# maxim2266/csvplus

Hardware: AMD Instinct MI355X
Metric: joined rows/sec (IndexOn build + chained Join, 1e8-row 3-col orders) (higher is better)
Workload: dtype u32; 1 GPU; BASELINE configs[3]: orders(1e8 x {cust_id,prod_id,qty}).Join(UniqueIndexOn customers.id 1e7).Join(UniqueIndexOn products.prod_id 1e5); rows=100000000, customers=10000000, products=100000, rows_this_rank=100000000, exchange=none (1 GPU), output=sorted positions

## Files before the change

csvplus_amd/csrc/capi.hip:

```cpp
#include <algorithm>
#include <map>
#include <mutex>
#include <new>

#include "cph_internal.hpp"
#include "codec_device.hpp"

namespace cph {

constexpr size_t kGuardBytes = 256;
constexpr uint8_t kGuardByte = 0xA5;

Status DevicePool::alloc(size_t bytes, void** out) {
    std::lock_guard<std::recursive_mutex> lk(mu_);
    const size_t want = (bytes + (guard ? kGuardBytes : 0) + 255) & ~(size_t)255;
    int best = -1;
    for (int i = 0; i < (int)free_.size(); i++) {
        if (free_[i].cap >= want && free_[i].cap <= want * 2 + (1u << 20)) {
            if (best < 0 || free_[i].cap < free_[best].cap) best = i;
        }
    }
    Block b;
    bool from_slab = false;
    for (size_t i = 0; i < slab_free_.size(); i++)
// ... 349 lines not shown
}

Status validate_cols(const cph_strcol* cols, int32_t ncols) {
    if (!cols || ncols <= 0) return {CPH_ERR_INVALID, "no key columns"};
    if (ncols > kMaxKeyCols) return {CPH_ERR_INVALID, "too many key columns"};
    for (int c = 0; c < ncols; c++) {
        if (cols[c].fixed_width == 0 && cols[c].offset_bits != 32 && cols[c].offset_bits != 64)
            return {CPH_ERR_INVALID, "offset_bits must be 32 or 64"};
        if (cols[c].mem != CPH_MEM_HOST && cols[c].mem != CPH_MEM_DEVICE) return {CPH_ERR_INVALID, "bad mem"};
        if (cols[c].nrows != cols[0].nrows) return {CPH_ERR_INVALID, "key columns differ in row count"};
        if (cols[c].nrows && !cols[c].offsets && cols[c].fixed_width == 0) return {CPH_ERR_INVALID, "offsets is NULL"};
        if (cols[c].nrows && cols[c].fixed_width && !cols[c].data) return {CPH_ERR_INVALID, "data is NULL"};
    }
    if (cols[0].nrows > 0xFFFFFFFFull) return {CPH_ERR_TOO_MANY_ROWS, "more than 2^32-1 rows"};
    return {};
}

Status stage_cols(cph_ctx* ctx, const cph_strcol* cols, int32_t ncols, std::vector<DevBuf>* storage,
                         DevCol* out) {
    for (int c = 0; c < ncols; c++) {
        DevCol d;
        d.nrows = cols[c].nrows;
        d.offset_bits = cols[c].offset_bits;
        d.fixed_width = cols[c].fixed_width;
        if (cols[c].mem == CPH_MEM_DEVICE || cols[c].nrows == 0) {
            d.data = cols[c].data;
            d.offsets = cols[c].offsets;
            if (!d.data) {
                if (!ctx->safe_words) {
                    CPH_TRY(ctx->safe_words.alloc(&ctx->pool, 64));
                    CPH_HIP_TRY(hipMemsetAsync(ctx->safe_words.get(), 0, 64, ctx->stream));
                }
                d.data = ctx->safe_words.as<uint8_t>();
            }
        } else if (cols[c].fixed_width) {
            const size_t bytes = (size_t)cols[c].nrows * cols[c].fixed_width;
            DevBuf bd;
            CPH_TRY(bd.alloc(&ctx->pool, bytes + 8));
            CPH_HIP_TRY(hipMemcpyAsync(bd.get(), cols[c].data, bytes, hipMemcpyHostToDevice, ctx->stream));
            d.data = bd.as<uint8_t>();
            d.offsets = nullptr;
            storage->push_back(std::move(bd));
        } else {
            const size_t obytes = (size_t)(cols[c].nrows + 1) * (size_t)(cols[c].offset_bits / 8);
            const uint64_t first = cols[c].offset_bits == 32 ? ((const uint32_t*)cols[c].offsets)[0]
                                                             : ((const uint64_t*)cols[c].offsets)[0];
            const uint64_t last = cols[c].offset_bits == 32 ? ((const uint32_t*)cols[c].offsets)[cols[c].nrows]
                                                            : ((const uint64_t*)cols[c].offsets)[cols[c].nrows];
            if (last < first) return {CPH_ERR_INVALID, "offsets are not monotonic"};
            DevBuf bo, bd;
            CPH_TRY(bo.alloc(&ctx->pool, obytes));
            CPH_TRY(bd.alloc(&ctx->pool, (size_t)last + 8));
            CPH_HIP_TRY(hipMemcpyAsync(bo.get(), cols[c].offsets, obytes, hipMemcpyHostToDevice, ctx->stream));
            if (last) CPH_HIP_TRY(hipMemcpyAsync(bd.get(), cols[c].data, (size_t)last, hipMemcpyHostToDevice, ctx->stream));
            d.data = bd.as<uint8_t>();
            d.offsets = bo.get();
            storage->push_back(std::move(bo));
            storage->push_back(std::move(bd));
        }
        out[c] = d;
    }
    return {};
}

Status check_row_sources(const cph_strcol* cols, const cph_rowsel* sel, int32_t ncols, uint64_t first_row, uint64_t nrows, bool exact) {
    for (int c = 0; c < ncols; c++) {
        CPH_TRY(validate_cols(cols + c, 1));
        const bool ident = !sel || !sel[c].ids;
        if (ident && nrows && (exact ? cols[c].nrows != nrows : cols[c].nrows < first_row + nrows))
            return {CPH_ERR_INVALID, exact ? "a column without row ids must have nrows rows"
                                           : "a column without row ids must have at least first_row + nrows rows"};
        if (!ident && sel[c].bits != 32 && sel[c].bits != 64) return {CPH_ERR_INVALID, "row id bits must be 32 or 64"};
    }
    return {};
}

Status stage_row_sources(cph_ctx* ctx, const cph_strcol* cols, const cph_rowsel* sel, const int* order, int32_t ncols, uint64_t first_row,
                         uint64_t n, std::vector<DevBuf>* staged, ColsArg* arg, ColIds* ids) {
    for (int k = 0; k < ncols; k++) {
        const int c = order ? order[k] : k;
        CPH_TRY(stage_cols(ctx, cols + c, 1, staged, &arg->c[k]));
        if (!sel || !sel[c].ids || !n) continue;
        RowIds& r = ids->ids[k];
        r.bits = sel[c].bits;
        r.base = sel[c].base;
        r.ptr = sel[c].ids;
        if (cols[c].mem == CPH_MEM_HOST) {
            const size_t w = (size_t)(sel[c].bits / 8);
            staged->emplace_back();
            CPH_TRY(staged->back().alloc(&ctx->pool, n * w));
            CPH_HIP_TRY(hipMemcpyAsync(staged->back().get(), static_cast<const uint8_t*>(sel[c].ids) + first_row * w, n * w,
                                       hipMemcpyHostToDevice, ctx->stream));
            r.ptr = reinterpret_cast<const void*>((uintptr_t)staged->back().get() - (uintptr_t)(first_row * w));
        }
    }
    return {};
}

Status deliver(cph_ctx* ctx, ResultOwner* owner, const ResultPart* parts, int nparts, int32_t out_mem) {
    auto show = [](const ResultPart& p, const void* v) { memcpy(p.pub, &v, sizeof v); };
    auto padded = [](const ResultPart& p) { return (p.bytes + 15) & ~(size_t)15; };
    uint8_t* h = nullptr;
    if (out_mem == CPH_MEM_HOST) {
        size_t need = 16;
        for (int i = 0; i < nparts; i++) need += padded(parts[i]);
        CPH_HIP_TRY(hipHostMalloc(&owner->h_block, need, hipHostMallocDefault));
        h = static_cast<uint8_t*>(owner->h_block);
    }
    for (int i = 0; i < nparts; i++) {
        const ResultPart& p = parts[i];
        const void* src = p.src ? p.src : p.dev->get();
        if (h && p.bytes) CPH_HIP_TRY(hipMemcpyAsync(h, src, p.bytes, hipMemcpyDeviceToHost, ctx->stream));
        show(p, h ? h : src);
        if (h) h += padded(p);
    }
    CPH_HIP_TRY(hipStreamSynchronize(ctx->stream));
    if (h)
        for (int i = 0; i < nparts; i++) parts[i].dev->reset();
    return {};
}

static int32_t fail(cph_ctx* ctx, const Status& s) {
    if (ctx) ctx->err = s.msg;
    return s.code;
}

static Status enter(cph_ctx* ctx) {
    if (!ctx) return {CPH_ERR_INVALID, "ctx is NULL"};
    CPH_HIP_TRY(hipSetDevice(ctx->device));
    return {};
}

struct BuildJob {
    cph_index* ix = nullptr;
    int32_t nkeycols = 0;
    std::vector<DevBuf> staged;
    DevCol dcols[kMaxKeyCols];
    DevBuf stats_dev;
    const void* sample_host = nullptr;
    size_t scratch_off = 0;
    GroupSpec spec;
    bool small = false;
    SmallBufs sbufs;
    bool presplit = false;
    bool sampled = false;
    bool no_sample = false;
    bool unique = false;
    bool no_direct = false;
    bool side = false;
    bool spec_split = false;
    bool exact_split = false;
    bool no_split = false;
    uint32_t* miss = nullptr;
    uint32_t* cs_over = nullptr;
    DevBuf cs_codes;
};

static Status build_phase1(cph_ctx* ctx, const cph_strcol* keycols, int32_t nkeycols, BuildJob* job) {
    CPH_TRY(validate_cols(keycols, nkeycols));
    cph_index* ix = job->ix;
    ix->ctx = ctx;
    ix->nrows = keycols[0].nrows;
    ix->table_rows = ix->nrows;
    ix->nkeycols = nkeycols;
    job->nkeycols = nkeycols;
    CPH_TRY(stage_cols(ctx, keycols, nkeycols, &job->staged, job->dcols));
    job->small = small_build_applies(ctx, job->dcols, nkeycols, ix->nrows);
    if (!job->small && !job->no_split && nkeycols == 1 && !job->dcols[0].fixed_width && ix->nrows >= (1ull << 22)) {
        CPH_TRY(codec_try_split(ctx, job->dcols, 1, ix->nrows, nullptr, &ix->codec, !job->exact_split, &job->spec_split));
        job->presplit = ix->codec.has_split();
    }
    job->sampled = !job->small && !job->presplit && !job->no_sample && codec_sample_applies(ctx, job->dcols, nkeycols, ix->nrows);
    if (job->sampled) CPH_TRY(codec_sample_launch(ctx, job->dcols[0], ix->nrows, &job->sample_host));
    else if (!job->small && !job->presplit) CPH_TRY(codec_stats_launch(ctx, job->dcols, nkeycols, &job->stats_dev));
    return {};
}

static Status build_phase2(cph_ctx* ctx, BuildJob* job, const void* stats_host);
static Status job_arm_miss(cph_ctx* ctx, BuildJob* job) {
    job->miss = host_word(ctx);
    return job->miss ? Status{} : Status{CPH_ERR_HIP, "no pinned host memory for the report words of a build"};
}
static Status build_encode_sort(cph_ctx* ctx, BuildJob* job);

static size_t job_readback_bytes(const BuildJob& j) {
    return j.small ? sizeof(SmallResult) : (j.presplit || j.sampled) ? 0 : sizeof(ColStats) * (size_t)j.nkeycols;
}

static void build_run(cph_ctx* ctx, std::vector<BuildJob>& jobs, std::vector<Status>& status) {
    const size_t nj = jobs.size();
    auto fail_all = [&](const Status& s) {
        for (size_t i = 0; i < nj; i++)
            if (status[i].ok()) status[i] = s;
    };
    size_t total = 0;
    bool any_general = false;
    for (size_t i = 0; i < nj; i++) {
        jobs[i].scratch_off = total;
        total += job_readback_bytes(jobs[i]);
        total = (total + 63) & ~(size_t)63;
        if (status[i].ok() && !jobs[i].small) any_general = true;
    }
    Status s = ensure_pinned_scratch(ctx, total > 64 ? total : 64);
    if (!s.ok()) return fail_all(s);
    uint8_t* h = static_cast<uint8_t*>(ctx->pinned_scratch);
    for (size_t i = 0; i < nj; i++) {
        if (!status[i].ok()) continue;
        if (jobs[i].small) {
            SideStream on_side(ctx, jobs[i].side);
            status[i] = small_build_launch(ctx, jobs[i].dcols, jobs[i].nkeycols, jobs[i].ix->nrows, &jobs[i].sbufs,
                                           reinterpret_cast<SmallResult*>(h + jobs[i].scratch_off));
            continue;
        }
        if (jobs[i].presplit || jobs[i].sampled) continue;
        hipError_t e = hipMemcpyAsync(h + jobs[i].scratch_off, jobs[i].stats_dev.get(), job_readback_bytes(jobs[i]),
                                      hipMemcpyDeviceToHost, jobs[i].side ? ctx->side_stream : ctx->stream);
        if (e != hipSuccess) status[i] = {CPH_ERR_HIP, std::string("statistics read-back: ") + hipGetErrorString(e)};
    }
    bool any_side = false;
    for (size_t i = 0; i < nj; i++) any_side = any_side || jobs[i].side;
    auto sync_streams = [&]() {
        return hipStreamSynchronize(ctx->stream) == hipSuccess && (!any_side || hipStreamSynchronize(ctx->side_stream) == hipSuccess);
    };
    if (!sync_streams()) return fail_all({CPH_ERR_HIP, "hipStreamSynchronize failed"});
    ctx->pool.flush_deferred();
    std::vector<std::vector<uint8_t>> stats_host(nj);
    std::vector<size_t> retry;
    for (size_t i = 0; i < nj; i++) {
        if (!status[i].ok()) continue;
        if (jobs[i].small) {
            const SmallResult res = *reinterpret_cast<const SmallResult*>(h + jobs[i].scratch_off);
            bool not_small = false;
            status[i] = small_build_finish(ctx, jobs[i].ix, jobs[i].nkeycols, &jobs[i].sbufs, &res, &not_small);
            jobs[i].sbufs = SmallBufs{};
            if (status[i].ok() && not_small) retry.push_back(i);
            else if (status[i].ok()) index_plan_table(jobs[i].ix);
            continue;
        }
        if (jobs[i].sampled) {
            const uint8_t* sh = static_cast<const uint8_t*>(jobs[i].sample_host);
            stats_host[i].assign(sh, sh + codec_sample_bytes());
        } else if (!jobs[i].presplit) {
            stats_host[i].assign(h + jobs[i].scratch_off, h + jobs[i].scratch_off + job_readback_bytes(jobs[i]));
        }
    }
    for (size_t i = 0; i < nj; i++)
        if (status[i].ok() && !jobs[i].small) {
            SideStream on_side(ctx, jobs[i].side);
            status[i] = build_phase2(ctx, &jobs[i], stats_host[i].data());
        }
    std::vector<size_t> resplit;
    std::vector<size_t> resort;
    if (any_general) {
        s = ensure_pinned_scratch(ctx, 2 * sizeof(uint32_t) * nj + 64);
        if (!s.ok()) return fail_all(s);
        uint32_t* fd = static_cast<uint32_t*>(ctx->pinned_scratch);
        uint32_t* sm = fd + nj;
        for (size_t i = 0; i < nj; i++) {
            if (!status[i].ok() || jobs[i].small) continue;
            hipStream_t js = jobs[i].side ? ctx->side_stream : ctx->stream;
            fd[i] = 0xFFFFFFFFu;
            sm[i] = 0;
            if (!jobs[i].ix->first_dup_dev) continue;
            hipError_t e = hipMemcpyAsync(&fd[i], jobs[i].ix->first_dup_dev.get(), sizeof(uint32_t), hipMemcpyDeviceToHost, js);
            if (e != hipSuccess) status[i] = {CPH_ERR_HIP, std::string("first-duplicate read-back: ") + hipGetErrorString(e)};
        }
        if (!sync_streams()) return fail_all({CPH_ERR_HIP, "hipStreamSynchronize failed"});
        ctx->pool.flush_deferred();
        for (size_t i = 0; i < nj; i++) {
            if (!status[i].ok() || jobs[i].small) continue;
            cph_index* ix = jobs[i].ix;
            if (jobs[i].miss) sm[i] = *(volatile uint32_t*)jobs[i].miss;
            if (sm[i]) { jobs[i].cs_codes.reset(); jobs[i].cs_over = nullptr; resplit.push_back(i); continue; }
            if (jobs[i].cs_over && *(volatile uint32_t*)jobs[i].cs_over) { resort.push_back(i); continue; }
            jobs[i].cs_codes.reset();
            ix->first_dup = fd[i] != 0xFFFFFFFFu ? (uint64_t)fd[i] : UINT64_MAX;
            ix->first_dup_dev.reset();
            index_plan_table(ix);
        }
    }
    for (size_t i : resort) {
        BuildJob& j = jobs[i];
        cph_index* ix = j.ix;
        const uint64_t n = ix->nrows;
        uint32_t* over = j.cs_over;
        j.cs_over = nullptr;
        ix->sorted_codes.reset(); ix->perm.reset(); ix->first_dup_dev.reset();
        DevBuf kb, va, vb;
        Status r = kb.alloc(&ctx->pool, n * sizeof(uint32_t));
        if (r.ok()) r = va.alloc(&ctx->pool, n * sizeof(uint32_t));
        bool sorted_now = false;
        {
            CountedSortPlan first;
            int wb = counted_sort_plan(ctx, n, ix->codec.word_states[0], &first) ? (int)first.wbits : 0;
            for (int attempt = 0; attempt < 2 && r.ok() && !sorted_now && wb > 0; attempt++) {
                wb -= 2;
                CountedSortPlan csp;
                if (!counted_sort_plan(ctx, n, ix->codec.word_states[0], &csp, wb) || (int)csp.wbits != wb) break;
                r = ix->first_dup_dev.alloc(&ctx->pool, sizeof(uint32_t));
                if (r.ok()) r = counted_sort(ctx, csp, j.cs_codes.as<uint32_t>(), n, ix->codec.word_states[0], va.as<uint32_t>(), kb.as<uint32_t>(),
                                             ix->first_dup_dev.as<uint32_t>(), over);
                if (r.ok() && hipStreamSynchronize(ctx->stream) != hipSuccess) r = {CPH_ERR_HIP, "hipStreamSynchronize failed"};
                if (r.ok() && *(volatile uint32_t*)over == 0) {
                    ix->sorted_codes = std::move(kb);
                    ix->perm = std::move(va);
                    ix->sort_passes = 0;
                    r = index_first_dup_read(ctx, ix);
                    sorted_now = true;
                } else {
                    ix->first_dup_dev.reset();
                }
            }
        }
        if (sorted_now) {
            j.cs_codes.reset();
            if (r.ok()) index_plan_table(ix);
            status[i] = r;
            continue;
        }
        if (r.ok()) r = vb.alloc(&ctx->pool, n * sizeof(uint32_t));
        uint32_t *kout = nullptr, *vout = nullptr;
        int passes = 0;
        if (r.ok()) r = radix_sort_pairs<uint32_t>(ctx, j.cs_codes.as<uint32_t>(), kb.as<uint32_t>(), va.as<uint32_t>(), vb.as<uint32_t>(), true, n,
                                                   ix->codec.word_bits[0], &kout, &vout, &passes);
        if (r.ok()) {
            ix->sorted_codes = std::move(kout == j.cs_codes.as<uint32_t>() ? j.cs_codes : kb);
            ix->perm = std::move(vout == va.as<uint32_t>() ? va : vb);
            ix->sort_passes = passes;
            r = index_first_dup_launch(ctx, ix);
        }
        if (r.ok()) r = index_first_dup_read(ctx, ix);
        j.cs_codes.reset();
        if (r.ok()) index_plan_table(ix);
        status[i] = r;
    }
    for (size_t i : resplit) {
        std::vector<BuildJob> one;
        one.push_back(std::move(jobs[i]));
        std::vector<Status> st1(1);
        BuildJob& j = one[0];
        j.side = false;
        const bool again_exact = j.spec_split;
        j.spec_split = false;
        j.exact_split = again_exact;
        j.no_split = !again_exact;
        j.no_sample = true;
        j.sampled = false;
        j.no_direct = true;
        j.presplit = false;
        j.miss = nullptr;
        cph_index* ix = j.ix;
        ix->codec = CodecHost{};
        ix->codec_dev.reset(); ix->sorted_codes.reset(); ix->perm.reset(); ix->first_dup_dev.reset(); ix->ranktab.reset();
        if (again_exact) {
            ctx->n_split_respec++;
            st1[0] = codec_try_split(ctx, j.dcols, 1, ix->nrows, nullptr, &ix->codec, false, nullptr);
            j.presplit = st1[0].ok() && ix->codec.has_split();
        }
        if (st1[0].ok() && !j.presplit) st1[0] = codec_stats_launch(ctx, j.dcols, j.nkeycols, &j.stats_dev);
        if (st1[0].ok()) build_run(ctx, one, st1);
        status[i] = st1[0];
        jobs[i] = std::move(one[0]);
    }
    for (size_t i : retry) {
        std::vector<BuildJob> one;
        one.push_back(std::move(jobs[i]));
        std::vector<Status> st1(1);
        one[0].small = false;
        one[0].side = false;
        st1[0] = codec_stats_launch(ctx, one[0].dcols, one[0].nkeycols, &one[0].stats_dev);
        if (st1[0].ok()) build_run(ctx, one, st1);
        status[i] = st1[0];
        jobs[i] = std::move(one[0]);
    }
}

static Status sort_words_lsd(cph_ctx* ctx, cph_index* ix, const uint64_t* all, int nw, const int* bits, uint64_t n, DevBuf& va,
                             DevBuf& vb) {
    DevBuf ka, kb;
    CPH_TRY(ka.alloc(&ctx->pool, n * sizeof(uint64_t)));
    CPH_TRY(kb.alloc(&ctx->pool, n * sizeof(uint64_t)));
    uint32_t* vcur = va.as<uint32_t>();
    uint32_t* vother = vb.as<uint32_t>();
    uint64_t* kout = ka.as<uint64_t>();
    bool first = true;
    int passes = 0;
    ix->sort_passes = 0;
    for (int w = nw - 1; w >= 0; w--) {
        const uint64_t* word = all + (uint64_t)w * n;
        if (first) {
            if (n) CPH_HIP_TRY(hipMemcpyAsync(ka.get(), word, n * sizeof(uint64_t), hipMemcpyDeviceToDevice, ctx->stream));
        } else {
            CPH_TRY(gather_u64(ctx, word, vcur, ka.as<uint64_t>(), n));
        }
        uint32_t* vout;
        CPH_TRY(radix_sort_pairs<uint64_t>(ctx, ka.as<uint64_t>(), kb.as<uint64_t>(), vcur, vother, first, n, bits[w], &kout, &vout,
                                           &passes));
        ix->sort_passes += passes;
        if (vout != vcur) { vother = vcur; vcur = vout; }
        first = false;
    }
    DevBuf sorted;
    CPH_TRY(sorted.alloc(&ctx->pool, (size_t)nw * n * sizeof(uint64_t)));
    if (n) CPH_HIP_TRY(hipMemcpyAsync(sorted.get(), kout, n * sizeof(uint64_t), hipMemcpyDeviceToDevice, ctx->stream));
    for (int w = 1; w < nw; w++) CPH_TRY(gather_u64(ctx, all + (uint64_t)w * n, vcur, sorted.as<uint64_t>() + (uint64_t)w * n, n));
    ix->sorted_codes = std::move(sorted);
    ix->perm = std::move(vcur == va.as<uint32_t>() ? va : vb);
    return {};
}

static DevCol window_col(const DevCol* cols, const cph_key_window& w, int s) {
    DevCol v = cols[w.seg_col[s]];
    v.skip = w.seg_skip[s];
    v.take = w.seg_take[s];
    return v;
}

static Status build_multi_window(cph_ctx* ctx, BuildJob* job, const std::vector<ColStats>& raw) {
    cph_index* ix = job->ix;
    const uint64_t n = ix->nrows;
    std::vector<cph_key_window>& W = ix->windows;
    W.clear();
    W.emplace_back();
    uint32_t room = kMaxKeyBytes;
    for (int c = 0; c < job->nkeycols; c++) {
        uint32_t left = raw[(size_t)c].maxlen, skip = 0;
        do {
            if (room == 0 || W.back().nseg == kMaxKeyCols) {
                W.emplace_back();
                room = kMaxKeyBytes;
            }
            cph_key_window& w = W.back();
            const uint32_t t = left < room ? left : room;
            w.seg_col[w.nseg] = c;
            w.seg_skip[w.nseg] = skip;
            w.seg_take[w.nseg] = t == left ? 0xFFFFFFFFu : t;
            w.nseg++;
            skip += t;
            left -= t;
            room -= t;
        } while (left > 0);
    }
    int total_words = 0;
    for (auto& w : W) {
        DevCol v[kMaxKeyCols];
        for (int s = 0; s < w.nseg; s++) v[s] = window_col(job->dcols, w, s);
        std::vector<ColStats> st;
        CPH_TRY(codec_collect_stats(ctx, v, w.nseg, &st));
        CPH_TRY(codec_build(st, &w.codec));
        w.codec.key32 = false;
        CPH_TRY(codec_upload(ctx, w.codec, &w.codec_dev));
        w.word_base = total_words;
        total_words += w.codec.nwords;
    }
    ix->codec = W[0].codec;
    DevBuf all, va, vb;
    CPH_TRY(all.alloc(&ctx->pool, (size_t)total_words * n * sizeof(uint64_t)));
    CPH_TRY(va.alloc(&ctx->pool, n * sizeof(uint32_t)));
    CPH_TRY(vb.alloc(&ctx->pool, n * sizeof(uint32_t)));
    std::vector<int> bits((size_t)total_words);
    for (auto& w : W) {
        DevCol v[kMaxKeyCols];
        for (int s = 0; s < w.nseg; s++) v[s] = window_col(job->dcols, w, s);
        CPH_TRY(codec_encode_build(ctx, w.codec, w.codec_dev, v, n, all.as<uint64_t>() + (uint64_t)w.word_base * n));
        for (int k = 0; k < w.codec.nwords; k++) bits[(size_t)(w.word_base + k)] = w.codec.word_bits[k];
    }
    CPH_TRY(sort_words_lsd(ctx, ix, all.as<uint64_t>(), total_words, bits.data(), n, va, vb));
    return index_first_dup_launch(ctx, ix);
}

static Status build_phase2(cph_ctx* ctx, BuildJob* job, const void* stats_host) {
    cph_index* ix = job->ix;
    const uint64_t n = ix->nrows;
    const int32_t nkeycols = job->nkeycols;
    const DevCol* dcols = job->dcols;
    if (job->presplit) {
        CPH_TRY(job_arm_miss(ctx, job));
        CPH_TRY(codec_upload(ctx, ix->codec, &ix->codec_dev));
        return build_encode_sort(ctx, job);
    }
    std::vector<ColStats> stats;
    if (job->sampled) {
        codec_sample_finish(dcols[0], stats_host, &stats);
        CPH_TRY(codec_build(stats, &ix->codec));
        if (codec_sample_checked(ix->codec, dcols)) {
            CPH_TRY(job_arm_miss(ctx, job));
            CPH_TRY(codec_upload(ctx, ix->codec, &ix->codec_dev));
            return build_encode_sort(ctx, job);
        }
        job->sampled = false;
        ix->codec = CodecHost{};
        CPH_TRY(codec_collect_stats(ctx, dcols, nkeycols, &stats));
    } else {
        codec_stats_finish(dcols, nkeycols, stats_host, &stats);
    }
    uint64_t positions = 0;
    for (const auto& s : stats) positions += s.maxlen;
    if (positions > (uint64_t)kMaxKeyBytes) return build_multi_window(ctx, job, stats);
    CPH_TRY(codec_build(stats, &ix->codec));
    if (!job->no_split) CPH_TRY(codec_try_split(ctx, dcols, nkeycols, n, &stats, &ix->codec));
// ... 97 lines not shown
                    return build_encode_sort(ctx, job);
                }
                CPH_TRY(codec_encode_build(ctx, cd, ix->codec_dev, dcols, n, ka.get(), &eh, nullptr));
            }
        }
        uint32_t* vout;
        if (cd.key32) {
            uint32_t* kout;
            CPH_TRY(radix_sort_pairs<uint32_t>(ctx, ka.as<uint32_t>(), kb.as<uint32_t>(), va.as<uint32_t>(), vb.as<uint32_t>(),
                                               true, n, cd.word_bits[0], &kout, &vout, &passes, eh.counts, eh.done));
            ix->sorted_codes = std::move(kout == ka.as<uint32_t>() ? ka : kb);
        } else {
            uint64_t* kout;
            CPH_TRY(radix_sort_pairs<uint64_t>(ctx, ka.as<uint64_t>(), kb.as<uint64_t>(), va.as<uint32_t>(), vb.as<uint32_t>(),
                                               true, n, cd.word_bits[0], &kout, &vout, &passes, eh.counts, eh.done));
            ix->sorted_codes = std::move(kout == ka.as<uint64_t>() ? ka : kb);
        }
        ix->sort_passes = passes;
        ix->perm = std::move(vout == va.as<uint32_t>() ? va : vb);
    } else {
        DevBuf all;
        CPH_TRY(all.alloc(&ctx->pool, (size_t)cd.nwords * n * sizeof(uint64_t)));
        CPH_TRY(codec_encode_build(ctx, cd, ix->codec_dev, dcols, n, all.get(), nullptr, nullptr, job->miss));
        CPH_TRY(sort_words_lsd(ctx, ix, all.as<uint64_t>(), cd.nwords, cd.word_bits, n, va, vb));
    }

    CPH_TRY(index_first_dup_launch(ctx, ix));
    return {};
}

static Status index_build_impl(cph_ctx* ctx, const cph_strcol* keycols, int32_t nkeycols, cph_index* ix, bool unique) {
    if (nkeycols == 1 && keycols && keycols[0].mem == CPH_MEM_HOST && validate_cols(keycols, nkeycols).ok()) {
        bool taken = false;
        CPH_TRY(build_from_host_codes(ctx, keycols, nkeycols, ix, unique, &taken));
        if (taken) return {};
    }
    std::vector<BuildJob> jobs(1);
    std::vector<Status> st(1);
    jobs[0].ix = ix;
    jobs[0].unique = unique;
    st[0] = build_phase1(ctx, keycols, nkeycols, &jobs[0]);
    if (st[0].ok()) build_run(ctx, jobs, st);
    return st[0];
}

}

using namespace cph;

extern "C" {

CPH_API const char* cph_version(void) { return "csvplus_hip 0.1 (gfx950)"; }

CPH_API int32_t cph_ctx_create(int32_t device_id, cph_ctx** out) {
    if (!out) return CPH_ERR_INVALID;
    *out = nullptr;
    int count = 0;
    hipError_t e = hipGetDeviceCount(&count);
    if (e != hipSuccess || count <= 0) {
        (void)hipGetLastError();
        return CPH_ERR_NO_DEVICE;
    }
    if (device_id < 0 || device_id >= count) return CPH_ERR_NO_DEVICE;
    if (hipSetDevice(device_id) != hipSuccess) return CPH_ERR_NO_DEVICE;
    cph_ctx* ctx = new (std::nothrow) cph_ctx();
    if (!ctx) return CPH_ERR_NOMEM;
    ctx->device = device_id;
    if (hipStreamCreateWithFlags(&ctx->stream, hipStreamNonBlocking) != hipSuccess) {
        delete ctx;
        return CPH_ERR_HIP;
    }
    ctx->own_stream = true;
    warm_keycodec();
    warm_radix_sort();
    warm_probe();
    warm_chain();
    warm_materialize();
    warm_csv_ingest();
    warm_index_ops();
    warm_resolve();
    warm_small_build();
    warm_window_sort();
    warm_counted_sort();
    (void)ensure_pinned_scratch(ctx, 1 << 16);
    void* ring = nullptr;
    (void)pinned_upload(ctx, 64, &ring);
    (void)host_word(ctx);
    *out = ctx;
    return CPH_OK;
}

CPH_API void cph_ctx_destroy(cph_ctx* ctx) {
    if (!ctx) return;
    (void)hipSetDevice(ctx->device);
    (void)hipStreamSynchronize(ctx->stream);
    if (ctx->pinned_scratch) (void)hipHostFree(ctx->pinned_scratch);
    if (ctx->upload_ring) (void)hipHostFree(ctx->upload_ring);
    if (ctx->host_words) (void)hipHostFree(ctx->host_words);
    for (void* p : ctx->pinned_user) (void)hipHostFree(p);
    for (auto& b : ctx->pinned_user_free) (void)hipHostFree(b.first);
    for (auto& b : ctx->pinned_cache) (void)hipHostFree(b.first);
    for (auto& p : ctx->prof_pending) { (void)hipEventDestroy(p.start); (void)hipEventDestroy(p.stop); }
    for (hipEvent_t e : ctx->prof_free_events) (void)hipEventDestroy(e);
    hipStream_t own = ctx->own_stream ? ctx->stream : nullptr;
    if (ctx->side_stream) {
        (void)hipStreamSynchronize(ctx->side_stream);
        (void)hipStreamDestroy(ctx->side_stream);
    }
    if (ctx->side_fork) (void)hipEventDestroy(ctx->side_fork);
    for (auto& sc : ctx->scan) sc.words.reset();
    for (auto& sc : ctx->self_clean) { sc.sum.reset(); sc.sample.reset(); sc.win.reset(); }
    host_pool_destroy(ctx);
    ctx->pool.trim();
    if (own) (void)hipStreamDestroy(own);
    delete ctx;
}

CPH_API int32_t cph_ctx_set_option(cph_ctx* ctx, const char* name, int64_t value) {
    if (!ctx || !name) return CPH_ERR_INVALID;
    const std::string k(name);
    if (k == "chain_debug") ctx->chain_debug = (int)value;
    else if (k == "sort_threads") ctx->sort_threads = (int)value;
    else if (k == "sort_rbits") ctx->sort_rbits = (int)value;
    else if (k == "sort_digit_stream") ctx->sort_digit_stream = value != 0;
    else if (k == "sort_xcd_tiles") ctx->sort_xcd_tiles = value != 0;
    else if (k == "codec_debug") ctx->codec_debug = (int)value;
    else if (k == "join_hash") ctx->join_hash = value != 0;
    else if (k == "chain_nt_streams") ctx->chain_nt_streams = value < 0 || value > 2 ? 0 : (int)value;
    else if (k == "chain_rank_lds") ctx->chain_rank_lds = value != 0;
    else if (k == "chain_rows4") ctx->chain_rows4 = value < 0 || value > 2 ? 1 : (int)value;
    else if (k == "codec_split") ctx->codec_split = value != 0;
    else if (k == "split_speculative") ctx->split_speculative = value != 0;
    else if (k == "scan_lookback") ctx->scan_lookback = value != 0;
    else if (k == "build_side_stream") ctx->build_side_stream = value != 0;
    else if (k == "stats_sample") ctx->stats_sample = value != 0;
    else if (k == "host_build") ctx->host_build = value != 0;
    else if (k == "host_threads") { ctx->host_threads = value < 0 || value > 256 ? 0 : (int)value; host_pool_destroy(ctx); }
    else if (k == "host_split") ctx->host_split = value < 0 || value > 2 ? 1 : (int)value;
    else if (k == "host_numa") ctx->host_numa = value != 0;
    else if (k == "hash_partitioned") ctx->hash_partitioned = value < 0 || value > 2 ? 1 : (int)value;
    else if (k == "host_split_threads") { ctx->host_split_threads = value < 0 || value > 256 ? 0 : (int)value; host_pool_destroy(ctx); }
    else if (k == "counted_sort") ctx->counted_sort = value != 0;
    else if (k == "csv_fast") ctx->csv_fast = value != 0;
    else if (k == "csv_onepass_debug") ctx->csv_onepass_debug = (int)value;
    else if (k == "csv_onepass") ctx->csv_onepass = value < 0 ? 0 : value > (1 << 20) ? (1 << 20) : (int)value;
    else if (k == "direct_sort") {
        if (value != 0 && value != 1) return fail_with(ctx, {CPH_ERR_INVALID, "direct_sort must be 0 or 1"});
        ctx->direct_sort = (int)value;
    }
    else if (k == "chain_arith") ctx->chain_arith = value != 0;
    else if (k == "chain_identity") ctx->chain_identity = value != 0;
    else if (k == "chain_prejoin") ctx->chain_prejoin = value != 0;
    else if (k == "direct_fused_encode") ctx->direct_fused_encode = value != 0;
    else if (k == "direct_ranktab") ctx->direct_ranktab = value != 0;
    else if (k == "hash_load_pct") ctx->hash_load_pct = value < 25 ? 25 : value > 90 ? 90 : (int)value;
    else if (k == "small_build_rows") ctx->small_build_rows = value < 0 ? 0 : value > (1 << 20) ? (1 << 20) : (int)value;
    else if (k == "plan_threads") ctx->plan_threads = (int)value;
    else if (k == "gstats_threads") ctx->gstats_threads = (int)value;
    else if (k == "speculative_groups") ctx->speculative_groups = value < 0 || value > 2 ? 1 : (int)value;
    else if (k == "pool_guard") ctx->pool.guard = value != 0;
    else if (k == "pool_reserve_mb") {
        if (value <= 0) return fail_with(ctx, {CPH_ERR_INVALID, "pool_reserve_mb must be positive"});
        if (hipSetDevice(ctx->device) != hipSuccess) return fail_with(ctx, {CPH_ERR_HIP, "hipSetDevice failed"});
        Status rs = ctx->pool.reserve((size_t)value << 20);
        if (!rs.ok()) return fail_with(ctx, rs);
    }
    else if (k == "pool_guard_check") {
        ctx->pool.check_live();
        if (ctx->pool.guard_violations) {
            char b[64];
            snprintf(b, sizeof b, " (%llu blocks)", (unsigned long long)ctx->pool.guard_violations);
            return fail_with(ctx, {CPH_ERR_INVALID, ctx->pool.first_violation + b});
        }
    }
    else return fail_with(ctx, {CPH_ERR_INVALID, "unknown option: " + k});
    return CPH_OK;
}

CPH_API const char* cph_last_error(const cph_ctx* ctx) { return ctx ? ctx->err.c_str() : "ctx is NULL"; }

CPH_API int32_t cph_ctx_set_stream(cph_ctx* ctx, void* hip_stream) {
    Status s = enter(ctx);
    if (!s.ok()) return fail(ctx, s);
    (void)hipStreamSynchronize(ctx->stream);
    if (ctx->side_stream) (void)hipStreamSynchronize(ctx->side_stream);
    for (auto& sc : ctx->scan) { sc.words.reset(); sc.tiles = 0; sc.tickets = 0; sc.epoch = 0; }
    if (hip_stream) {
        if (ctx->own_stream) (void)hipStreamDestroy(ctx->stream);
        ctx->stream = reinterpret_cast<hipStream_t>(hip_stream);
        ctx->own_stream = false;
    } else if (!ctx->own_stream) {
        if (hipStreamCreateWithFlags(&ctx->stream, hipStreamNonBlocking) != hipSuccess)
            return fail(ctx, {CPH_ERR_HIP, "hipStreamCreate failed"});
        ctx->own_stream = true;
    }
    return CPH_OK;
}

CPH_API int32_t cph_ctx_synchronize(cph_ctx* ctx) {
    Status s = enter(ctx);
    if (!s.ok()) return fail(ctx, s);
    hipError_t e = hipStreamSynchronize(ctx->stream);
    if (e != hipSuccess) return fail(ctx, {CPH_ERR_HIP, std::string("hipStreamSynchronize: ") + hipGetErrorString(e)});
    return CPH_OK;
}

CPH_API int32_t cph_ctx_profile(cph_ctx* ctx, int32_t enable) {
    Status s = enter(ctx);
    if (!s.ok()) return fail(ctx, s);
    ctx->profiling = enable != 0;
    ctx->prof_only.clear();
    return CPH_OK;
}

CPH_API int32_t cph_ctx_profile_only(cph_ctx* ctx, const char* kernel_name) {
    Status s = enter(ctx);
    if (!s.ok()) return fail(ctx, s);
    ctx->profiling = kernel_name != nullptr;
    ctx->prof_only = kernel_name ? kernel_name : "";
    return CPH_OK;
}

CPH_API int32_t cph_ctx_profile_read(cph_ctx* ctx, cph_kernel_stat* out, int32_t cap, int32_t* n, int32_t reset) {
    Status s = enter(ctx);
    if (!s.ok()) return fail(ctx, s);
    if (!n || (cap > 0 && !out)) return fail(ctx, {CPH_ERR_INVALID, "bad argument"});
    hipError_t e = hipStreamSynchronize(ctx->stream);
    if (e != hipSuccess) return fail(ctx, {CPH_ERR_HIP, std::string("hipStreamSynchronize: ") + hipGetErrorString(e)});
    for (auto& p : ctx->prof_pending) {
        float ms = 0;
        if (hipEventElapsedTime(&ms, p.start, p.stop) == hipSuccess) {
            ProfStat& st = ctx->prof_stats[(size_t)p.name_idx];
            st.launches++;
            st.total_ms += ms;
            st.bytes += p.bytes;
        } else {
            (void)hipGetLastError();
        }
        ctx->prof_free_events.push_back(p.start);
        ctx->prof_free_events.push_back(p.stop);
    }
    ctx->prof_pending.clear();
    const int32_t total = (int32_t)ctx->prof_stats.size();
    *n = total;
    for (int32_t i = 0; i < total && i < cap; i++) {
        const ProfStat& st = ctx->prof_stats[(size_t)i];
        memset(&out[i], 0, sizeof out[i]);
        snprintf(out[i].name, sizeof out[i].name, "%s", st.name.c_str());
        out[i].launches = st.launches;
        out[i].total_ms = st.total_ms;
        out[i].algo_bytes = st.bytes;
    }
    if (reset) ctx->prof_stats.clear();
    return CPH_OK;
}

CPH_API int32_t cph_pinned_alloc(cph_ctx* ctx, size_t bytes, void** out) {
    Status s = enter(ctx);
    if (!s.ok()) return fail(ctx, s);
    if (!out) return fail(ctx, {CPH_ERR_INVALID, "out is NULL"});
    void* p = nullptr;
    constexpr size_t kRecycleMax = 4u << 20;
    size_t cap = bytes ? bytes : 1;
    if (cap <= kRecycleMax) {
        size_t c2 = 4096;
        while (c2 < cap) c2 <<= 1;
        cap = c2;
        for (size_t i = 0; i < ctx->pinned_user_free.size(); i++)
            if (ctx->pinned_user_free[i].second == cap) {
                p = ctx->pinned_user_free[i].first;
                ctx->pinned_user_free.erase(ctx->pinned_user_free.begin() + (long)i);
                break;
            }
    }
    if (!p) {
        hipError_t e = hipHostMalloc(&p, cap, hipHostMallocDefault);
        if (e != hipSuccess) {
            (void)hipGetLastError();
            for (auto& b : ctx->pinned_user_free) (void)hipHostFree(b.first);
            ctx->pinned_user_free.clear();
            e = hipHostMalloc(&p, cap, hipHostMallocDefault);
        }
        if (e != hipSuccess) return fail(ctx, {CPH_ERR_NOMEM, std::string("hipHostMalloc: ") + hipGetErrorString(e)});
    }
    ctx->pinned_user.push_back(p);
    if (cap <= kRecycleMax) ctx->pinned_user_cap.push_back({p, cap});
    *out = p;
    return CPH_OK;
}

CPH_API int32_t cph_pinned_free(cph_ctx* ctx, void* p) {
    Status s = enter(ctx);
    if (!s.ok()) return fail(ctx, s);
    auto it = std::find(ctx->pinned_user.begin(), ctx->pinned_user.end(), p);
    if (it == ctx->pinned_user.end()) return fail(ctx, {CPH_ERR_INVALID, "not a cph_pinned_alloc block"});
    ctx->pinned_user.erase(it);
    for (size_t i = 0; i < ctx->pinned_user_cap.size(); i++)
        if (ctx->pinned_user_cap[i].first == p) {
            const size_t cap = ctx->pinned_user_cap[i].second;
            ctx->pinned_user_cap.erase(ctx->pinned_user_cap.begin() + (long)i);
            if (ctx->pinned_user_free.size() < 32) {
                ctx->pinned_user_free.push_back({p, cap});
                return CPH_OK;
            }
            break;
        }
    (void)hipHostFree(p);
    return CPH_OK;
}

CPH_API int32_t cph_index_build(cph_ctx* ctx, const cph_strcol* keycols, int32_t nkeycols, int32_t unique,
                                cph_index** out, uint64_t* first_dup_pos) {
    Status s = enter(ctx);
    if (!s.ok()) return fail(ctx, s);
    if (!out) return fail(ctx, {CPH_ERR_INVALID, "out is NULL"});
    *out = nullptr;
    if (first_dup_pos) *first_dup_pos = UINT64_MAX;
    cph_index* ix = new (std::nothrow) cph_index();
    if (!ix) return fail(ctx, {CPH_ERR_NOMEM, "out of host memory"});
    s = index_build_impl(ctx, keycols, nkeycols, ix, unique != 0);
    if (!s.ok()) {
        delete ix;
        return fail(ctx, s);
    }
    if (first_dup_pos) *first_dup_pos = ix->first_dup;
    *out = ix;
    if (unique && ix->first_dup != UINT64_MAX) {
        char b[128];
        snprintf(b, sizeof b, "duplicate value while creating unique index (sorted position %llu)",
                 (unsigned long long)ix->first_dup);
        return fail(ctx, {CPH_ERR_DUPLICATE, b});
    }
    return CPH_OK;
}

CPH_API int32_t cph_index_build_many(cph_ctx* ctx, const cph_index_spec* specs, int32_t nspecs, cph_index** out,
                                     uint64_t* first_dup_pos, int32_t* status) {
    Status s = enter(ctx);
    if (!s.ok()) return fail(ctx, s);
    if (!specs || !out || nspecs < 1 || nspecs > 64) return fail(ctx, {CPH_ERR_INVALID, "bad cph_index_build_many arguments"});
    std::vector<BuildJob> jobs((size_t)nspecs);
    std::vector<Status> st((size_t)nspecs);
    if (!host_words_reserve(ctx, (uint32_t)nspecs * (uint32_t)(codec_sample_bytes() / 4 + 16)))
        return fail(ctx, {CPH_ERR_INVALID, "cph_index_build_many: the batch needs more report words than the ctx holds"});
    bool two_streams = nspecs >= 2 && ctx->build_side_stream != 0;
    if (two_streams && !ctx->side_stream && hipStreamCreateWithFlags(&ctx->side_stream, hipStreamNonBlocking) != hipSuccess) {
        (void)hipGetLastError();
        ctx->side_stream = nullptr;
        two_streams = false;
    }
    struct DeferGuard {
        cph_ctx* c;
        ~DeferGuard() {
            if (!c) return;
            (void)hipStreamSynchronize(c->stream);
            (void)hipStreamSynchronize(c->side_stream);
            c->pool.end_defer();
        }
    } defer{two_streams ? ctx : nullptr};
    if (two_streams) {
        hipError_t fe = ctx->side_fork ? hipSuccess : hipEventCreateWithFlags(&ctx->side_fork, hipEventDisableTiming);
        if (fe == hipSuccess) fe = hipEventRecord(ctx->side_fork, ctx->stream);
        if (fe == hipSuccess) fe = hipStreamWaitEvent(ctx->side_stream, ctx->side_fork, 0);
        if (fe != hipSuccess) {
            (void)hipGetLastError();
            two_streams = false;
            defer.c = nullptr;
        }
    }
    if (two_streams) ctx->pool.begin_defer();
    for (int i = 0; i < nspecs; i++) {
        out[i] = nullptr;
        if (first_dup_pos) first_dup_pos[i] = UINT64_MAX;
        jobs[i].ix = new (std::nothrow) cph_index();
        jobs[i].side = two_streams && (i & 1);
        jobs[i].unique = specs[i].unique != 0;
        SideStream on_side(ctx, jobs[i].side);
        if (!jobs[i].ix) st[i] = {CPH_ERR_NOMEM, "out of host memory"};
        else st[i] = build_phase1(ctx, specs[i].keycols, specs[i].nkeycols, &jobs[i]);
    }
    build_run(ctx, jobs, st);
    int32_t rc = CPH_OK;
    std::string msg;
    for (int i = 0; i < nspecs; i++) {
        cph_index* ix = jobs[i].ix;
        if (st[i].ok() && specs[i].unique && ix->first_dup != UINT64_MAX) {
            char b[160];
            snprintf(b, sizeof b, "index %d: duplicate value while creating unique index (sorted position %llu)", i,
                     (unsigned long long)ix->first_dup);
            st[i] = {CPH_ERR_DUPLICATE, b};
        }
        const bool keep = st[i].ok() || st[i].code == CPH_ERR_DUPLICATE;
        if (keep) {
            out[i] = ix;
            if (first_dup_pos) first_dup_pos[i] = ix->first_dup;
        } else {
            delete ix;
        }
        if (status) status[i] = st[i].code;
        if (!st[i].ok() && rc == CPH_OK) { rc = st[i].code; msg = st[i].msg; }
    }
    if (rc != CPH_OK) return fail(ctx, {rc, msg});
    return CPH_OK;
}

CPH_API void cph_index_destroy(cph_index* ix) {
    if (!ix) return;
    if (ix->ctx) (void)hipSetDevice(ix->ctx->device);
    if (ix->perm_host) {
        if (ix->ctx) pinned_cache_put(ix->ctx, ix->perm_host, ix->perm_host_cap);
        else (void)hipHostFree(ix->perm_host);
    }
    delete ix;
}

CPH_API uint64_t cph_index_nrows(const cph_index* ix) { return ix ? ix->nrows : 0; }
CPH_API int32_t cph_index_nkeycols(const cph_index* ix) { return ix ? ix->nkeycols : 0; }

CPH_API int32_t cph_index_perm(cph_index* ix, int32_t mem, const uint32_t** perm, uint64_t* n) {
    if (!ix || !perm) return CPH_ERR_INVALID;
    cph_ctx* ctx = ix->ctx;
    Status s = enter(ctx);
    if (!s.ok()) return fail(ctx, s);
    if (n) *n = ix->nrows;
    if (mem == CPH_MEM_DEVICE) {
        *perm = ix->perm.as<uint32_t>();
        return CPH_OK;
    }
    if (!ix->perm_host) {
        const size_t bytes = (size_t)ix->nrows * sizeof(uint32_t);
        void* p = nullptr;
        size_t cap = 0;
        s = pinned_cache_get(ctx, bytes, &p, &cap);
        if (!s.ok()) return fail(ctx, s);
        if (bytes) {
            hipError_t e = hipMemcpyAsync(p, ix->perm.get(), bytes, hipMemcpyDeviceToHost, ctx->stream);
            if (e == hipSuccess) e = hipStreamSynchronize(ctx->stream);
            if (e != hipSuccess) {
                (void)hipHostFree(p);
                return fail(ctx, {CPH_ERR_HIP, std::string("perm read-back: ") + hipGetErrorString(e)});
            }
        }
        ix->perm_host = static_cast<uint32_t*>(p);
        ix->perm_host_cap = cap;
    }
    *perm = ix->perm_host;
    return CPH_OK;
}

CPH_API int32_t cph_join_probe(cph_ctx* ctx, const cph_index* ix, const cph_strcol* probecols, int32_t nprobecols,
                               const void* row_sel, int32_t sel_bits, uint64_t sel_base, uint64_t nsel,
                               uint64_t probe_base, int32_t want_pairs, int32_t out_mem, cph_matches** out) {
    Status s = enter(ctx);
    if (!s.ok()) return fail(ctx, s);
    if (!ix || !out) return fail(ctx, {CPH_ERR_INVALID, "index/out is NULL"});
    *out = nullptr;
    if (nprobecols > ix->nkeycols) return fail(ctx, {CPH_ERR_TOO_MANY_COLS, "too many source columns in Join()"});
    s = validate_cols(probecols, nprobecols);
    if (!s.ok()) return fail(ctx, s);
    if (out_mem != CPH_MEM_HOST && out_mem != CPH_MEM_DEVICE) return fail(ctx, {CPH_ERR_INVALID, "bad out_mem"});
    if (row_sel && sel_bits != 32 && sel_bits != 64) return fail(ctx, {CPH_ERR_INVALID, "sel_bits must be 32 or 64"});
    if (row_sel && nsel > 0xFFFFFFFFull) return fail(ctx, {CPH_ERR_TOO_MANY_ROWS, "more than 2^32-1 selected rows"});

    cph_matches_impl* m = new (std::nothrow) cph_matches_impl();
    if (!m) return fail(ctx, {CPH_ERR_NOMEM, "out of host memory"});
    m->ctx = ctx;
    auto run = [&]() -> Status {
        std::vector<DevBuf> staged;
        DevCol dcols[kMaxKeyCols];
        CPH_TRY(stage_cols(ctx, probecols, nprobecols, &staged, dcols));
        RowSel dsel;
        dsel.ptr = row_sel;
        dsel.bits = sel_bits;
        dsel.base = sel_base;
        DevBuf selbuf;
        const bool cols_on_host = probecols[0].mem == CPH_MEM_HOST;
        if (row_sel && cols_on_host && nsel) {
            const size_t sb = nsel * (size_t)(sel_bits / 8);
            CPH_TRY(selbuf.alloc(&ctx->pool, sb));
            CPH_HIP_TRY(hipMemcpyAsync(selbuf.get(), row_sel, sb, hipMemcpyHostToDevice, ctx->stream));
            dsel.ptr = selbuf.get();
        }
        const uint64_t nprobe = row_sel ? nsel : probecols[0].nrows;
        ProbeOut po;
        CPH_TRY(probe_run(ctx, ix, dcols, nprobecols, dsel, nprobe, probe_base, want_pairs != 0, &po));
        m->pub.nprobe = nprobe;
        m->pub.nmatches = po.nmatches;
        m->pub.mem = out_mem;
        const bool pairs = want_pairs && po.nmatches;
        if (out_mem == CPH_MEM_DEVICE) {
            m->d_lo = std::move(po.lo);
            m->d_cnt = std::move(po.cnt);
            m->d_pidx = std::move(po.pidx);
            m->d_brow = std::move(po.brow);
            m->pub.lo = m->d_lo.as<uint32_t>();
            m->pub.cnt = m->d_cnt.as<uint32_t>();
// ... 306 lines not shown
```

csvplus_amd/csrc/codec_device.hpp:

```cpp
#pragma once

#include "cph_internal.hpp"
#include "device_utils.hpp"

namespace cph {

__device__ __forceinline__ uint64_t find_first_byte(const uint8_t* data, uint64_t begin, uint64_t len, uint32_t d) {
    const uint64_t dv = 0x0101010101010101ull * (uint64_t)(d & 0xFFu);
    for (uint64_t j = 0; 8 * j < len; j++) {
        const uint64_t x = load_value_chunk(data, begin, len, (int)j) ^ dv;
        const uint64_t t = (x - 0x0101010101010101ull) & ~x & 0x8080808080808080ull;
        if (t) {
            const uint64_t pos = 8 * j + (uint64_t)((__ffsll((long long)t) - 1) >> 3);
            return pos < len ? pos : len;
        }
    }
    return len;
}

__device__ __forceinline__ void value_span_whole(const DevCol& col, uint64_t row, uint64_t* begin, uint64_t* len);
__device__ __forceinline__ void value_span(const DevCol& col, uint64_t row, uint64_t* begin, uint64_t* len) {
    value_span_whole(col, row, begin, len);
    if (col.split) {
        const uint64_t b = *begin, l = *len;
// ... 218 lines not shown
        uint32_t b[R], e[R];
#pragma unroll
        for (int k = 0; k < R; k++) {
            b[k] = NT ? __builtin_nontemporal_load(&off[wr.rel[k]]) : off[wr.rel[k]];
            e[k] = NT ? __builtin_nontemporal_load(&off[wr.rel[k] + 1]) : off[wr.rel[k] + 1];
        }
#pragma unroll
        for (int k = 0; k < R; k++) {
            sp->x[k] = b[k];
            sp->len[k] = e[k] - b[k];
        }
    } else if constexpr (sizeof(B) == 8) {
        const uint64_t* off = reinterpret_cast<const uint64_t*>(c.offsets) + wr.rbase;
        uint64_t b[R], e[R];
#pragma unroll
        for (int k = 0; k < R; k++) {
            b[k] = off[wr.rel[k]];
            e[k] = off[wr.rel[k] + 1];
        }
#pragma unroll
        for (int k = 0; k < R; k++) {
            sp->x[k] = b[k];
            const uint64_t l = e[k] - b[k];
            sp->len[k] = l > 0xFFFFFFFFull ? 0xFFFFFFFFu : (uint32_t)l;
        }
    } else {
#pragma unroll
        for (int k = 0; k < R; k++) { sp->x[k] = 0; sp->len[k] = 0; }
    }
}
template <int R, class B>
__device__ __forceinline__ void gather_spans(const DevCol& c, const uint32_t (&row)[R], WaveSpans<R, B>* sp) {
    const uint64_t p = (uint64_t)(uintptr_t)c.data;
    sp->base8 = (const uint8_t*)(uintptr_t)(p & ~7ull);
    sp->delta = (uint32_t)(p & 7ull);
    if (c.fixed_width) {
#pragma unroll
        for (int k = 0; k < R; k++) {
            sp->x[k] = (B)row[k] * (B)c.fixed_width;
            sp->len[k] = c.fixed_width;
        }
        return;
    }
    if (c.offset_bits == 32) {
        const uint32_t* off = reinterpret_cast<const uint32_t*>(c.offsets);
        uint32_t b[R], e[R];
#pragma unroll
        for (int k = 0; k < R; k++) {
            b[k] = off[row[k]];
            e[k] = off[(uint64_t)row[k] + 1];
        }
#pragma unroll
        for (int k = 0; k < R; k++) {
            sp->x[k] = b[k];
            sp->len[k] = e[k] - b[k];
        }
    } else if constexpr (sizeof(B) == 8) {
        const uint64_t* off = reinterpret_cast<const uint64_t*>(c.offsets);
        uint64_t b[R], e[R];
#pragma unroll
        for (int k = 0; k < R; k++) {
            b[k] = off[row[k]];
            e[k] = off[(uint64_t)row[k] + 1];
        }
#pragma unroll
        for (int k = 0; k < R; k++) {
            sp->x[k] = b[k];
            const uint64_t l = e[k] - b[k];
            sp->len[k] = l > 0xFFFFFFFFull ? 0xFFFFFFFFu : (uint32_t)l;
        }
    } else {
#pragma unroll
        for (int k = 0; k < R; k++) { sp->x[k] = 0; sp->len[k] = 0; }
    }
}
inline bool col_is_narrow(const DevCol& c) { return c.fixed_width ? c.fixed_width <= 0xFFFFu : c.offset_bits == 32; }

template <int R, class W, class B, bool FIXED>
__device__ __forceinline__ void encode_position(const CPH_LDS W* lp, int b, uint32_t pos, const WaveSpans<R, B>& sp, const uint64_t (&cur)[R],
                                                W (&acc)[R], W (&bad)[R]) {
#pragma unroll
    for (int k = 0; k < R; k++) {
        const uint32_t half = b < 4 ? (uint32_t)cur[k] : (uint32_t)(cur[k] >> 32);
        const uint32_t byte = (half >> (8 * (b & 3))) & 0xFFu;
        const uint32_t sym = FIXED ? byte + 1u : (pos < sp.len[k] ? byte + 1u : 0u);
        const W v = lp[b * kLutStride + sym];
        if constexpr (sizeof(W) == 4) {
            acc[k] = __builtin_elementwise_add_sat(acc[k], v);
        } else {
            bad[k] |= v;
            acc[k] += v;
        }
    }
}

template <int R, class W, class B, class CW, bool LONG>
__device__ __forceinline__ void encode_rows(const CodecView& cv, const WaveSpans<R, B>& sp, const uint64_t (&c0)[R],
                                            const uint64_t (&c1)[R], CW (&code)[R], uint32_t* okmask, bool fixed = false) {
    const int maxlen = cv.hdr->col_maxlen[0];
    const CPH_LDS W* lutw = (const CPH_LDS W*)cv.lutw;
    W acc[R], bad[R];
#pragma unroll
    for (int k = 0; k < R; k++) { acc[k] = 0; bad[k] = 0; }
    const int nchunks = (maxlen + 7) >> 3;
#pragma unroll 1
    for (int j = 0; j < nchunks; j++) {
        uint64_t cur[R];
        if (j == 0) {
#pragma unroll
            for (int k = 0; k < R; k++) cur[k] = c0[k];
        } else if (LONG && j == 1) {
#pragma unroll
            for (int k = 0; k < R; k++) cur[k] = c1[k];
        } else {
#pragma unroll
            for (int k = 0; k < R; k++) cur[k] = sp.chunk(k, (uint32_t)j);
        }
        const int qn = maxlen - 8 * j < 8 ? maxlen - 8 * j : 8;
        const CPH_LDS W* lp = lutw + (8 * j) * kLutStride;
        if (fixed) {
#pragma unroll
            for (int b = 0; b < 8; b++)
                if (b < qn) encode_position<R, W, B, true>(lp, b, (uint32_t)(8 * j + b), sp, cur, acc, bad);
        } else {
#pragma unroll
            for (int b = 0; b < 8; b++)
                if (b < qn) encode_position<R, W, B, false>(lp, b, (uint32_t)(8 * j + b), sp, cur, acc, bad);
        }
    }
    uint32_t m = *okmask;
#pragma unroll
    for (int k = 0; k < R; k++) {
        code[k] = (CW)acc[k];
        const W flag = sizeof(W) == 4 ? acc[k] : bad[k];
        const bool good = sp.len[k] <= (uint32_t)maxlen && !(flag >> (sizeof(W) * 8 - 1));
        if (!good) m &= ~(1u << k);
    }
    *okmask = m;
}

struct ArithPlan {
    uint32_t enabled;
    uint32_t mul24;
    uint32_t keylen;
    uint32_t keep[2];
    uint32_t lo[2];
    uint32_t rngc[2];
    uint32_t wa[2], wb[2];
    uint32_t ma[2];
    uint32_t s1;
};

void codec_arith_plan(const CodecHost& codec, ArithPlan* ap);

template <int R, class CW>
__device__ __forceinline__ void encode_rows_arith(const ArithPlan& ap, const uint64_t (&c0)[R], CW (&code)[R], uint32_t* okmask) {
    uint32_t m = *okmask;
    uint32_t zl[R], zh[R];
#pragma unroll
    for (int k = 0; k < R; k++) {
        const uint32_t xl = (uint32_t)c0[k], xh = (uint32_t)(c0[k] >> 32);
        zl[k] = xl - ap.lo[0];
        zh[k] = xh - ap.lo[1];
        const uint32_t tl = zl[k] + ap.rngc[0], th = zh[k] + ap.rngc[1];
        const uint32_t bad = ((xl | zl[k] | tl) | (xh | zh[k] | th)) & 0x80808080u;
        if (bad) m &= ~(1u << k);
    }
    if (ap.mul24) {
#pragma unroll
        for (int k = 0; k < R; k++) {
            const uint32_t pa0 = __builtin_amdgcn_udot4(zl[k], ap.wa[0], 0u, false);
            const uint32_t pa1 = __builtin_amdgcn_udot4(zh[k], ap.wa[1], 0u, false);
            const uint32_t w0 = __builtin_amdgcn_udot4(zl[k], ap.wb[0], __umul24(pa0, ap.ma[0]), false);
            code[k] = (CW)__builtin_amdgcn_udot4(zh[k], ap.wb[1], __umul24(pa1, ap.ma[1]) + __umul24(w0, ap.s1), false);
        }
    } else {
#pragma unroll
        for (int k = 0; k < R; k++) {
            const uint32_t pa0 = __builtin_amdgcn_udot4(zl[k], ap.wa[0], 0u, false);
            const uint32_t pa1 = __builtin_amdgcn_udot4(zh[k], ap.wa[1], 0u, false);
            const uint32_t w0 = __builtin_amdgcn_udot4(zl[k], ap.wb[0], pa0 * ap.ma[0], false);
            code[k] = (CW)__builtin_amdgcn_udot4(zh[k], ap.wb[1], pa1 * ap.ma[1] + w0 * ap.s1, false);
        }
    }
    *okmask = m;
}

template <bool LONGV = true>
struct ValueHeadT {
    uint64_t begin = 0, len = 0, c0 = 0, c1 = 0, c2 = 0;
    __device__ __forceinline__ void span(const DevCol& col, uint64_t row) { value_span(col, row, &begin, &len); }
    __device__ __forceinline__ void chunks(const DevCol& col) {
        c0 = len > 0 ? load_value_chunk(col.data, begin, len, 0) : 0;
        c1 = len > 8 ? load_value_chunk(col.data, begin, len, 1) : 0;
        c2 = len > 16 ? load_value_chunk(col.data, begin, len, 2) : 0;
    }
    __device__ __forceinline__ void chunks_nobranch(const DevCol& col) {
        const uint64_t p = (uint64_t)(uintptr_t)col.data;
        const uint8_t* base8 = (const uint8_t*)(uintptr_t)(p & ~7ull);
        const uint32_t delta = (uint32_t)(p & 7ull);
        const uint32_t l32 = len > 0xFFFFFFFFull ? 0xFFFFFFFFu : (uint32_t)len;
        const uint64_t a = load_chunk_nobranch<uint64_t>(base8, delta, begin, l32, 0);
        const uint64_t b = load_chunk_nobranch<uint64_t>(base8, delta, begin, l32, 1);
        const uint64_t c = load_chunk_nobranch<uint64_t>(base8, delta, begin, l32, 2);
        c0 = l32 > 0 ? a : 0;
        c1 = l32 > 8 ? b : 0;
        c2 = l32 > 16 ? c : 0;
    }
    __device__ __forceinline__ void load(const DevCol& col, uint64_t row) {
        span(col, row);
        chunks(col);
    }
    __device__ __forceinline__ uint64_t chunk(const DevCol& col, int j) const {
        if constexpr (LONGV) {
            if (8ull * (uint64_t)j >= len) return 0;
            return j == 0 ? c0 : j == 1 ? c1 : j == 2 ? c2 : load_value_chunk(col.data, begin, len, j);
        } else {
            return j == 0 ? c0 : j == 1 ? c1 : j == 2 ? c2 : 0;
        }
    }
    __device__ __forceinline__ uint32_t sym(const DevCol& col, int q) const {
        const uint32_t b = ((uint32_t)(chunk(col, q >> 3) >> (8 * (q & 7))) & 0xFFu) + 1u;
        return (uint64_t)q < len ? b : 0u;
    }
    __device__ __forceinline__ uint64_t window(const DevCol& col, int q) const {
        const int sh = (q & 7) * 8;
        const uint64_t lo = chunk(col, q >> 3);
        if (sh == 0) return lo;
        return (lo >> sh) | (chunk(col, (q >> 3) + 1) << (64 - sh));
    }
    __device__ __forceinline__ uint64_t raw(const DevCol& col, int q, int span) const {
        const uint64_t nvalid = len > (uint64_t)q ? (len - (uint64_t)q < (uint64_t)span ? len - (uint64_t)q : (uint64_t)span) : 0;
        return group_raw(window(col, q), nvalid);
    }
    template <int J>
    __device__ __forceinline__ uint64_t ck() const {
        if constexpr (J == 0) return c0;
        else if constexpr (J == 1) return c1;
        else if constexpr (J == 2) return c2;
        else return 0;
    }
    template <int J>
    __device__ __forceinline__ uint32_t sym_j(int q) const {
        const uint32_t b = ((uint32_t)(ck<J>() >> (8 * (q & 7))) & 0xFFu) + 1u;
        return (uint64_t)q < len ? b : 0u;
    }
    template <int J>
    __device__ __forceinline__ uint64_t window_j(int q) const {
        const int sh = (q & 7) * 8;
        return sh == 0 ? ck<J>() : (ck<J>() >> sh) | (ck<J + 1>() << (64 - sh));
    }
    template <int J>
    __device__ __forceinline__ uint64_t raw_j(int q, int span) const {
        const uint32_t l32 = len > 0xFFFFFFFFull ? 0xFFFFFFFFu : (uint32_t)len;
        const uint32_t left = l32 > (uint32_t)q ? l32 - (uint32_t)q : 0u;
        return group_raw(window_j<J>(q), (uint64_t)(left < (uint32_t)span ? left : (uint32_t)span));
    }
};
using ValueHead = ValueHeadT<true>;

template <class Emit>
__device__ __forceinline__ bool encode_key_groups(const CodecView& cv, const ColsArg& cols, int ncols_used, uint64_t row,
                                                  Emit&& emit) {
    const int p_end = cv.hdr->col_start[ncols_used];
    uint64_t acc = 0;
    bool valid = true;
    for (int c = 0; c < ncols_used; c++) {
        const DevCol& col = cols.c[c];
        uint64_t begin, len;
        value_span(col, row, &begin, &len);
        const int maxlen = cv.hdr->col_maxlen[c];
        const int p0 = cv.hdr->col_start[c];
        if (len > (uint64_t)maxlen) valid = false;
        ValueHead v;
        v.begin = begin;
        v.len = len;
        v.chunks(col);
        for (int q = 0; q < maxlen; q++) {
            const int p = p0 + q;
            const uint32_t kind = cv.unit[p];
            uint64_t r = 0;
            if (kind == kUnitWide) {
                int rank = -1;
                if (len <= (uint64_t)kWideBytes) {
                    uint64_t w[4];
                    wide_words(col.data, begin, len, w);
                    rank = wide_lookup(cv, w[0], w[1], w[2], w[3], (uint32_t)len);
                }
                if (rank < 0) valid = false;
                r = rank < 0 ? 0ull : (uint64_t)rank;
            } else if (kind == kUnitHead) {
                int span = 1;
                while (span < kGroupSpan && q + span < maxlen && cv.unit[p + span] == kUnitAbsorbed) span++;
                const uint64_t joint = v.raw(col, q, span);
                const CPH_LDS uint64_t* d = cv.dict + cv.dict_off[p];
                const CPH_LDS uint16_t* ht = cv.hash + cv.hash_off[p];
                const int bits = cv.hash_bits[p];
                const uint32_t mask = (1u << bits) - 1u;
                uint32_t sl = bits ? group_slot(joint, bits) : 0u;
                bool found = false;
                for (;;) {
                    const uint32_t e = ht[sl];
                    if (e == 0) break;
                    if (d[e - 1] == joint) { r = (uint64_t)(e - 1); found = true; break; }
                    sl = (sl + 1) & mask;
                }
// ... 56 lines not shown
```

csvplus_amd/csrc/cph_internal.hpp:

```cpp
#pragma once

#include <hip/hip_runtime.h>

#include <cstdint>
#include <cstdio>
#include <cstring>
#include <mutex>
#include <string>
#include <utility>
#include <vector>

#include "../../include/csvplus_hip.h"

namespace cph {

constexpr int kMaxKeyBytes = 128;
constexpr int kMaxKeyCols  = CPH_MAX_KEY_COLS;
constexpr int kLutStride   = 257;
constexpr uint16_t kLutInvalid = 0xFFFF;
constexpr int kMaxWords    = 20;

struct Status {
    int32_t code = CPH_OK;
    std::string msg;
// ... 99 lines not shown
#else
#define CPH_HD2
#endif
CPH_HD2 inline uint32_t wide_rotl(uint32_t v, int r) { return (v << r) | (v >> (32 - r)); }
CPH_HD2 inline void wide_fold(uint64_t w0, uint64_t w1, uint64_t w2, uint64_t w3, uint32_t len, uint32_t* x, uint32_t* y) {
    *x = (uint32_t)w0 ^ wide_rotl((uint32_t)w1, 9) ^ wide_rotl((uint32_t)w2, 18) ^ wide_rotl((uint32_t)w3, 27) ^ (len * 0x01000193u);
    *y = (uint32_t)(w0 >> 32) ^ wide_rotl((uint32_t)(w1 >> 32), 7) ^ wide_rotl((uint32_t)(w2 >> 32), 14) ^ wide_rotl((uint32_t)(w3 >> 32), 21);
}
CPH_HD2 inline uint32_t wide_hash_lo(uint64_t w0, uint64_t w1, uint64_t w2, uint64_t w3, uint32_t len) {
    uint32_t x, y;
    wide_fold(w0, w1, w2, w3, len, &x, &y);
    uint32_t h1 = (x * 0x9E3779B1u) ^ (y * 0x85EBCA6Bu);
    h1 ^= h1 >> 15;
    return h1;
}
CPH_HD2 inline uint64_t wide_hash(uint64_t w0, uint64_t w1, uint64_t w2, uint64_t w3, uint32_t len) {
    uint32_t x, y;
    wide_fold(w0, w1, w2, w3, len, &x, &y);
    const uint32_t h1 = wide_hash_lo(w0, w1, w2, w3, len);
    uint32_t h2 = (x * 0xCC9E2D51u + wide_rotl(y, 13)) * 0x1B873593u;
    h2 ^= h2 >> 16;
    h2 *= 0xC2B2AE35u;
    h2 ^= h2 >> 13;
    const uint64_t h = (uint64_t)h1 | ((uint64_t)h2 << 32);
    return h ? h : 1ull;
}

struct CodecHost {
    int32_t ncols = 0;
    int32_t npos = 0;
    int32_t nwords = 1;
    bool    key32 = false;
    int32_t col_start[kMaxKeyCols + 1] = {0};
    int32_t col_maxlen[kMaxKeyCols] = {0};
    int32_t col_minlen[kMaxKeyCols] = {0};
    int32_t word_bits[kMaxWords] = {0};
    uint64_t word_states[kMaxWords] = {0};
    std::vector<uint16_t> radix;
    std::vector<uint64_t> mult;
    std::vector<int32_t>  word_of;
    std::vector<uint16_t> lut;
    std::vector<uint8_t>  unit;
    std::vector<int32_t>  dict_off;
    std::vector<int32_t>  dict_len;
    std::vector<uint64_t> dict;
    bool has_groups() const { return !unit.empty(); }
    int32_t split_col = -1;
    uint8_t split_byte = 0;
    bool spec_checked = false;
    int32_t split_maxlen = 0;
    std::vector<WideKey> wdict;
    std::vector<uint16_t> wide_disp, wide_slots;
    bool has_split() const { return split_col >= 0; }
    int32_t virtual_cols(int32_t real_cols) const { return real_cols + (has_split() && split_col < real_cols ? 1 : 0); }
};
constexpr int kGroupSpan = 7;
constexpr int kGroupDictMax = 4096;
enum : uint8_t { kUnitPos = 0, kUnitHead = 1, kUnitAbsorbed = 2, kUnitWide = 3 };

struct CodecDevHeader {
    int32_t ncols;
    int32_t npos;
    int32_t nwords;
    int32_t key32;
    int32_t col_start[kMaxKeyCols + 1];
    int32_t col_maxlen[kMaxKeyCols];
    int32_t mult_off;
    int32_t wordof_off;
    int32_t lut_off;
    int32_t total_bytes;
    int32_t lutw_off;
    int32_t lutw_bits;
    int32_t ngroups;
    int32_t unit_off;
    int32_t dictoff_off;
    int32_t dictlen_off;
    int32_t dict_off;
    int32_t hashoff_off;
    int32_t hashbits_off;
    int32_t hash_off;
    int32_t wide_pos;
    int32_t wide_n;
    int32_t wide_off;
    int32_t wide_hash_off;
    int32_t wide_hash_bits;
    int32_t split_vcol;
    int32_t split_byte;
    int32_t wide_disp_off;
    int32_t wide_disp_bits;
    int32_t pad_[3];
};
#if defined(__HIPCC__)
#define CPH_HD __host__ __device__
#else
#define CPH_HD
#endif
CPH_HD inline uint32_t group_slot(uint64_t raw, int bits) { return (uint32_t)((raw * 0x9E3779B97F4A7C15ull) >> (64 - bits)); }
CPH_HD inline uint64_t group_raw(uint64_t window, uint64_t nvalid) {
    return (window & ((1ull << (8 * nvalid)) - 1ull)) | (nvalid << 56);
}
CPH_HD inline uint64_t group_order_key(uint64_t raw, int span) {
    const int nvalid = (int)(raw >> 56);
    uint64_t k = 0;
    for (int i = 0; i < span && i < nvalid; i++) k |= (((raw >> (8 * i)) & 0xFFull) + 1ull) << (9 * (kGroupSpan - 1 - i));
    return k;
}

}

namespace cph {
struct ProfPending { int name_idx; hipEvent_t start, stop; double bytes; };
struct ProfStat { std::string name; uint64_t launches = 0; double total_ms = 0, bytes = 0; };
}

struct cph_ctx {
    int device = 0;
    hipStream_t stream = nullptr;
    bool own_stream = false;
    std::string err;
    cph::DevicePool pool;
    void* pinned_scratch = nullptr;
    size_t pinned_scratch_bytes = 0;
    void* upload_ring = nullptr;
    size_t upload_cap = 0, upload_pos = 0;
    std::vector<void*> pinned_user;
    std::vector<std::pair<void*, size_t>> pinned_user_free;
    std::vector<std::pair<void*, size_t>> pinned_user_cap;
    std::vector<std::pair<void*, size_t>> pinned_cache;
    uint32_t* host_words = nullptr;
    uint32_t host_words_pos = 0;
    struct SelfClean {
        cph::DevBuf sum;
        cph::DevBuf sample;
        cph::DevBuf win;
        uint64_t win_words = 0;
    } self_clean[2];
    cph::DevBuf safe_words;
    int cus = 0;
    int chain_debug = 0;
    int sort_threads = 0, sort_rbits = 0;
    int sort_digit_stream = 1;
    int sort_xcd_tiles = 1;
    int small_build_rows = 8192;
    int chain_nt_streams = 0;
    int chain_arith = 1;
    int chain_identity = 1;
    int chain_rows4 = 1;
    int chain_rank_lds = 1;
    int join_hash = 1;
    int codec_debug = 0;
    uint64_t n_split_respec = 0;
    int hash_load_pct = 50;
    int direct_fused_encode = 1;
    int direct_ranktab = 1;
    int chain_prejoin = 1;
    int split_speculative = 1;
    int codec_split = 1;
    int scan_lookback = 1;
    struct ScanState {
        cph::DevBuf words;
        uint64_t tiles = 0, epoch = 0;
        uint32_t tickets = 0;
    } scan[2];
    int csv_fast = 1;
    int csv_onepass = 1;
    int csv_onepass_debug = 0;
    int hash_partitioned = 1;
    int counted_sort = 1;
    int direct_sort = 1;
    int stats_sample = 1;
    int host_build = 1;
    int host_threads = 0;
    void* host_pool = nullptr;
    int host_split = 1;
    int host_split_threads = 0;
    void* host_pool_wide = nullptr;
    int host_numa = 0;
    int build_side_stream = 1;
    hipStream_t side_stream = nullptr;
    hipEvent_t side_fork = nullptr;
    int stream_slot = 0;
    hipStream_t swapped_main = nullptr;
    hipStream_t other_stream() const { return stream_slot ? swapped_main : side_stream; }
    int plan_threads = 0, gstats_threads = 0;
    int speculative_groups = 1;
    struct KernelCfg { const void* fn; size_t lds; int blocks_per_cu; };
    std::vector<KernelCfg> kernel_cfg;
    bool profiling = false;
    std::string prof_only;
    std::vector<cph::ProfPending> prof_pending;
    std::vector<cph::ProfStat> prof_stats;
    std::vector<hipEvent_t> prof_free_events;
};

namespace cph {
constexpr uint32_t kHostWords = 65536;
uint32_t* host_word(cph_ctx* ctx, uint32_t n = 1);
bool host_words_reserve(cph_ctx* ctx, uint32_t n);
Status self_clean_block(cph_ctx* ctx, cph::DevBuf* b, size_t bytes);
struct SideStream {
    cph_ctx* ctx;
    hipStream_t saved;
    SideStream(cph_ctx* c, bool on) : ctx(on ? c : nullptr), saved(c->stream) {
        if (ctx) {
            ctx->swapped_main = saved;
            ctx->stream = ctx->side_stream;
            ctx->stream_slot = 1;
        }
    }
    ~SideStream() {
        if (ctx) {
            ctx->stream = saved;
            ctx->stream_slot = 0;
            ctx->swapped_main = nullptr;
        }
    }
    SideStream(const SideStream&) = delete;
    SideStream& operator=(const SideStream&) = delete;
};
}

struct cph_key_window {
    cph::CodecHost codec;
    cph::DevBuf codec_dev;
    int32_t nseg = 0;
    int32_t seg_col[CPH_MAX_KEY_COLS] = {0};
    uint32_t seg_skip[CPH_MAX_KEY_COLS] = {0}, seg_take[CPH_MAX_KEY_COLS] = {0};
    int32_t word_base = 0;
};

struct cph_index {
    cph_ctx* ctx = nullptr;
    uint64_t nrows = 0;
    uint64_t table_rows = 0;
    int32_t nkeycols = 0;
    cph::CodecHost codec;
    cph::DevBuf codec_dev;
    std::vector<cph_key_window> windows;
    int32_t total_words() const {
        if (windows.empty()) return codec.nwords;
        int32_t t = 0;
        for (const auto& w : windows) t += w.codec.nwords;
        return t;
    }
    cph::DevBuf sorted_codes;
    cph::DevBuf perm;
    cph::DevBuf table;
    cph::DevBuf rowtab;
    cph::DevBuf ranktab;
    uint64_t table_entries = 0;
    cph::DevBuf hash;
    uint32_t hash_sectors = 0;
    uint32_t hash_slice_mask = 0;
    int32_t hash_mode = 0;
    bool accel_failed = false;
    std::mutex accel_mu;
    hipEvent_t accel_ready = nullptr;
    ~cph_index() {
        if (accel_ready) (void)hipEventDestroy(accel_ready);
    }
    int32_t sort_passes = 0;
    bool small_built = false;
    bool host_coded = false;
    uint64_t first_dup = UINT64_MAX;
    uint32_t* perm_host = nullptr;
    size_t perm_host_cap = 0;
    cph::DevBuf first_dup_dev;
};

struct cph_chain_impl {
    cph_chain pub;
    cph_ctx* ctx = nullptr;
    cph::DevBuf d_stream;
    cph::DevBuf d_rows[CPH_MAX_CHAIN];
    void* h_block = nullptr;
    size_t h_cap = 0;
};

struct cph_matches_impl {
    cph_matches pub;
    cph_ctx* ctx = nullptr;
    cph::DevBuf d_lo, d_cnt, d_pidx, d_brow;
    void* h_block = nullptr;
    size_t h_cap = 0;
};

namespace cph {

struct DevCol {
    const uint8_t* data = nullptr;
    const void* offsets = nullptr;
    uint64_t nrows = 0;
    int32_t offset_bits = 32;
    uint32_t fixed_width = 0;
    uint32_t skip = 0, take = 0xFFFFFFFFu;
    bool segmented() const { return skip != 0 || take != 0xFFFFFFFFu; }
    uint16_t split = 0;
    uint16_t part = 0;
};
struct ColsArg {
    DevCol c[kMaxKeyCols];
};
struct RowIds {
    const void* ptr = nullptr;
    int32_t bits = 32;
    uint64_t base = 0;
    uint64_t* stash = nullptr;
};
struct ColIds {
    RowIds ids[kMaxKeyCols];
};
int codec_virtual_cols(const CodecHost& codec, const DevCol* real, int nreal, DevCol* out);
bool codec_wide_perfect_hash(CodecHost* codec);

struct ColStats {
    uint32_t minlen, maxlen;
    uint32_t mask[kMaxKeyBytes][8];
};
Status codec_collect_stats(cph_ctx* ctx, const DevCol* cols, int32_t ncols, std::vector<ColStats>* out);
Status codec_stats_launch(cph_ctx* ctx, const DevCol* cols, int32_t ncols, DevBuf* dev_stats);
void codec_stats_finish(const DevCol* cols, int32_t ncols, const void* host_copy, std::vector<ColStats>* out);
Status codec_build(const std::vector<ColStats>& stats, CodecHost* codec);
bool codec_sample_applies(const cph_ctx* ctx, const DevCol* cols, int32_t ncols, uint64_t n);
size_t codec_sample_bytes();
Status codec_sample_launch(cph_ctx* ctx, const DevCol& col, uint64_t n, const void** host_copy);
void codec_sample_finish(const DevCol& col, const void* host_copy, std::vector<ColStats>* out);
bool codec_sample_checked(const CodecHost& codec, const DevCol* cols);
struct GroupChoice { int t, p0, span; double saved; uint32_t count; uint32_t tab; };
struct GroupSpec {
    bool active = false;
    DevBuf slots, counts, miss;
    std::vector<GroupChoice> chosen;
    CodecHost plain;
};
Status codec_try_groups(cph_ctx* ctx, const DevCol* cols, int32_t ncols, uint64_t n, CodecHost* codec, GroupSpec* spec = nullptr);
constexpr uint32_t kSpecGiveUp = 1u << 16;
Status codec_groups_complete(cph_ctx* ctx, const DevCol* cols, int32_t ncols, uint64_t n, uint32_t missed, GroupSpec* spec, CodecHost* codec);
Status codec_upload(cph_ctx* ctx, const CodecHost& codec, DevBuf* dev);
int codec_premultiplied_bits(const CodecHost& codec);
struct EncodeHist {
    uint32_t tile_rows = 0;
    uint32_t digit_mask = 0;
    uint32_t bins = 0;
    uint32_t* counts = nullptr;
    bool done = false;
};
Status codec_encode_build(cph_ctx* ctx, const CodecHost& codec, const DevBuf& codec_dev, const DevCol* cols,
                          uint64_t n, void* out_codes, const EncodeHist* hist = nullptr, const GroupSpec* spec = nullptr,
                          uint32_t* miss = nullptr);
Status codec_try_split(cph_ctx* ctx, const DevCol* cols, int32_t ncols, uint64_t n, const std::vector<ColStats>* stats, CodecHost* codec,
                       bool speculate = false, bool* speculated = nullptr);
Status codec_split_from_host(cph_ctx* ctx, const cph_host::HostCol& hc, uint64_t n, cph_host::BlockPool& pool, CodecHost* codec);
bool codec_encode_values_host(const CodecHost& codec, const cph_strval* values, int32_t nvalues,
                              uint64_t* q_exact, int32_t* nq, uint64_t* qlo, uint64_t* qhi);

struct RadixPlan {
    int npass = 0, threads = 256, rbits = 8;
    uint32_t tile = 4096, ntiles = 0;
    int nb0 = 0;
    size_t count_words() const { return ((size_t)1 << rbits) * ntiles; }
};
RadixPlan radix_plan(const cph_ctx* ctx, uint64_t n, int bits);
template <class K>
Status radix_sort_pairs(cph_ctx* ctx, K* keys_a, K* keys_b, uint32_t* vals_a, uint32_t* vals_b, bool vals_iota,
                        uint64_t n, int bits, K** keys_out, uint32_t** vals_out, int* passes,
                        uint32_t* counts = nullptr, bool first_hist_done = false);
struct CountedSortPlan {
    uint32_t wbits = 0, k2 = 0, nb1 = 0, nwt = 0;
    bool two = false;
};
bool counted_sort_plan(const cph_ctx* ctx, uint64_t n, uint64_t states, CountedSortPlan* p, int max_wbits = 31, uint64_t min_rows = 1ull << 21);
struct CountedSort {
    CountedSortPlan p;
    DevBuf words, ent1, ent2;
    uint32_t* counts = nullptr;
    Status begin(cph_ctx* ctx, const CountedSortPlan& plan, uint64_t n);
    Status partition(cph_ctx* ctx, const uint32_t* codes, uint64_t n, uint64_t states, uint32_t* over_host, bool hist_done);
    const uint64_t* entries() const { return p.two ? ent2.as<uint64_t>() : ent1.as<uint64_t>(); }
    const uint32_t* flag() const { return counts + p.nwt; }
    const uint32_t* wbase() const { return counts + p.nwt + 1; }
    Status run(cph_ctx* ctx, const uint32_t* codes, uint64_t n, uint64_t states, uint32_t* perm_out, uint32_t* sorted_out, uint32_t* first_dup_dev,
               uint32_t* over_host, bool hist_done);
};
Status counted_sort(cph_ctx* ctx, const CountedSortPlan& p, const uint32_t* codes, uint64_t n, uint64_t states, uint32_t* perm_out,
                    uint32_t* sorted_out, uint32_t* first_dup_dev, uint32_t* over_host);
void warm_counted_sort();
struct ArithPlan;
Status direct_sort_windows_keys(cph_ctx* ctx, const uint64_t* keys, const ArithPlan& ap, uint64_t n, uint64_t states, uint32_t* perm_out,
                                uint32_t* sorted_out, uint32_t* flag, void* ranktab = nullptr, uint64_t rank_blocks = 0);
Status direct_sort_windows(cph_ctx* ctx, const uint32_t* codes, uint64_t n, uint64_t states, uint32_t* perm_out, uint32_t* sorted_out,
                           uint32_t* flag, void* ranktab = nullptr, uint64_t rank_blocks = 0);
struct WindowSort {
    Status begin(cph_ctx* ctx, uint64_t n, uint64_t states);
    Status add(cph_ctx* ctx, const uint32_t* codes, uint64_t row0, uint64_t m, uint32_t* flag, const uint64_t* keys = nullptr, const ArithPlan* ap = nullptr);
    Status finish(cph_ctx* ctx, uint32_t* perm_out, uint32_t* sorted_out, uint32_t* flag, void* ranktab = nullptr, uint64_t rank_blocks = 0);
    ~WindowSort();
    WindowSort() = default;
    WindowSort(const WindowSort&) = delete;
    WindowSort& operator=(const WindowSort&) = delete;
    uint64_t n = 0, states = 0, nb1 = 0, nwin_total = 0;
    uint32_t nb2 = 1, shift1 = 0;
    bool two = false, started = false, finished = false;
    DevBuf ent1, ent2;
    DevBuf* words = nullptr;
    uint32_t *cur1 = nullptr, *cur2 = nullptr;
};
Status exclusive_scan_u32(cph_ctx* ctx, uint32_t* data, uint64_t n);
Status exclusive_scan_u32_total(cph_ctx* ctx, uint32_t* data, uint64_t n, uint32_t* total_out);
Status exclusive_scan_u64(cph_ctx* ctx, uint64_t* data, uint64_t n, uint64_t* total_out);
Status gather_u64(cph_ctx* ctx, const uint64_t* src, const uint32_t* idx, uint64_t* dst, uint64_t n);
Status fill_iota_u32(cph_ctx* ctx, uint32_t* dst, uint64_t n);

Status index_first_dup_launch(cph_ctx* ctx, cph_index* ix);
Status index_first_dup_read(cph_ctx* ctx, cph_index* ix);
void index_plan_table(cph_index* ix);
Status index_ensure_table(cph_ctx* ctx, const cph_index* ix);
Status index_ensure_rowtab(cph_ctx* ctx, const cph_index* ix);
Status index_ensure_ranktab(cph_ctx* ctx, const cph_index* ix);
inline uint64_t ranktab_blocks(uint64_t table_entries) { return ((table_entries + 31) / 32 + 1) & ~1ull; }
Status index_ensure_hash(cph_ctx* ctx, const cph_index* ix);
bool index_wants_hash(const cph_index* ix);
struct ProbeOut {
    DevBuf lo, cnt, pidx, brow;
    uint64_t nprobe = 0, nmatches = 0;
};
struct RowSel {
    const void* ptr = nullptr;
    int32_t bits = 32;
    uint64_t base = 0;
};
Status probe_run(cph_ctx* ctx, const cph_index* ix, const DevCol* cols, int32_t ncols, RowSel sel,
                 uint64_t nprobe, uint64_t probe_base, bool want_pairs, ProbeOut* out, bool positions = false);
Status index_find_device(cph_ctx* ctx, const cph_index* ix, const uint64_t* q_exact, int32_t nq, uint64_t qlo,
                         uint64_t qhi, uint64_t* lower, uint64_t* upper);
Status index_find_many_device(cph_ctx* ctx, const cph_index* ix, const uint64_t* queries, size_t stride, uint64_t nkeys,
                              uint64_t* lower, uint64_t* upper);

void index_desc_serialize(const cph_index* ix, std::vector<uint8_t>* out);
size_t index_desc_header_bytes();
bool index_desc_size(const uint8_t* p, size_t n, size_t* need);
bool index_desc_parse(const uint8_t* p, size_t n, cph_index* ix);
Status index_adopt_payload(cph_ctx* ctx, cph_index* ix);
size_t index_code_bytes(const cph_index* ix);
Status index_select_device(cph_ctx* ctx, const cph_index* ix, const uint64_t* d_pos, uint64_t n, cph_index* nx);

struct ChainStep {
    const cph_index* index = nullptr;
    DevCol cols[kMaxKeyCols];
    int32_t ncols = 0;
    int32_t source = 0;
};
struct ChainOut {
    DevBuf stream_row;
    DevBuf build_row[CPH_MAX_CHAIN];
    uint64_t nrows = 0;
    int32_t nsteps = 0;
    bool identity = false;
};
Status chain_run(cph_ctx* ctx, const ChainStep* steps, int nsteps, uint64_t probe_base, ChainOut* out, bool positions = false);
bool chain_fast_path_ok(const ChainStep* steps, int nsteps);
Status chain_enqueue_dense(cph_ctx* ctx, const ChainStep* steps, int nsteps, uint64_t nprobe, uint64_t probe_base,
                           uint32_t* const* d_rows, uint64_t* d_masks, uint32_t* d_counts, uint64_t* d_total, bool positions = false);
Status chain_enqueue_codes(cph_ctx* ctx, const cph_index* const* idx, const uint32_t* const* d_codes, int nsteps, uint64_t nprobe,
                           uint32_t* const* d_rows, uint64_t* d_masks, uint32_t* d_counts, uint64_t* d_total, bool positions);
uint64_t chain_dense_mask_words(uint64_t nprobe);
uint64_t chain_dense_count_words(uint64_t nprobe);

void warm_keycodec();
void warm_radix_sort();
void warm_probe();
void warm_chain();
void warm_materialize();
void warm_csv_ingest();
void warm_index_ops();
void warm_resolve();
void warm_small_build();
void warm_window_sort();
Status build_from_host_codes(cph_ctx* ctx, const cph_strcol* keycols, int32_t nkeycols, cph_index* ix, bool unique, bool* taken);
void host_pool_destroy(cph_ctx* ctx);

constexpr int kSmallMaxPos = 64;
enum : uint32_t { kSmallBuilt = 0, kSmallNotSmall = 1, kSmallPending = 0xFFFFFFFFu };
struct SmallResult {
    uint32_t status;
    uint32_t first_dup;
    uint32_t bits, key32, passes;
    uint32_t minlen[kMaxKeyCols], maxlen[kMaxKeyCols];
    uint32_t mask[kSmallMaxPos][8];
    uint64_t t[10];
    uint64_t codec_check;
};
CPH_HD inline uint64_t small_codec_check(uint64_t h, uint64_t radix, uint64_t mult) {
    h = (h ^ radix) * 0x9E3779B97F4A7C15ull;
    return (h ^ mult) * 0xC2B2AE3D27D4EB4Full + 1;
}
struct SmallBufs {
    DevBuf ka, kb, va, vb, sorted, perm;
};
bool small_build_applies(const cph_ctx* ctx, const DevCol* cols, int32_t ncols, uint64_t n);
Status small_build_launch(cph_ctx* ctx, const DevCol* cols, int32_t ncols, uint64_t n, SmallBufs* bufs, SmallResult* res);
Status small_build_finish(cph_ctx* ctx, cph_index* ix, int32_t ncols, SmallBufs* bufs, const SmallResult* res, bool* not_small);

Status ensure_pinned_scratch(cph_ctx* ctx, size_t bytes);
Status pinned_cache_get(cph_ctx* ctx, size_t bytes, void** out, size_t* cap);
void pinned_cache_put(cph_ctx* ctx, void* p, size_t cap);
Status pinned_upload(cph_ctx* ctx, size_t bytes, void** out);
Status validate_cols(const cph_strcol* cols, int32_t ncols);
Status stage_cols(cph_ctx* ctx, const cph_strcol* cols, int32_t ncols, std::vector<DevBuf>* storage, DevCol* out);
Status check_row_sources(const cph_strcol* cols, const cph_rowsel* sel, int32_t ncols, uint64_t first_row, uint64_t nrows, bool exact);
Status stage_row_sources(cph_ctx* ctx, const cph_strcol* cols, const cph_rowsel* sel, const int* order, int32_t ncols, uint64_t first_row,
                         uint64_t n, std::vector<DevBuf>* staged, ColsArg* arg, ColIds* ids);

inline int32_t fail_with(cph_ctx* ctx, const Status& s) {
    if (ctx) ctx->err = s.msg;
    return s.code;
}

struct ResultOwner {
    cph_ctx* ctx = nullptr;
    void* h_block = nullptr;
    ResultOwner() = default;
    ResultOwner(const ResultOwner&) = delete;
    ResultOwner& operator=(const ResultOwner&) = delete;
    ~ResultOwner() {
        if (h_block) (void)hipHostFree(h_block);
    }
};
struct ResultPart {
    DevBuf* dev;
    size_t bytes;
    void* pub;
    const void* src = nullptr;
};
Status deliver(cph_ctx* ctx, ResultOwner* owner, const ResultPart* parts, int nparts, int32_t out_mem);

template <class Impl, class Pub>
int32_t finish_call(cph_ctx* ctx, Impl* r, const Status& s, Pub** out) {
    if (!s.ok()) {
        (void)hipStreamSynchronize(ctx->stream);
        delete r;
        return fail_with(ctx, s);
    }
    *out = &r->pub;
    return CPH_OK;
// ... 49 lines not shown
```

csvplus_amd/csrc/keycodec.hip:

```cpp
#include <algorithm>
#include <cmath>
#include <mutex>

#include "codec_device.hpp"
#include "host_encode_kernels.hpp"

namespace cph {

constexpr int kStatsThreads = 256;
constexpr int kStatsRows = 8;

template <class B, bool SEG>
__global__ __launch_bounds__(kStatsThreads) void k_col_stats(DevCol col, uint32_t* __restrict__ g_minmax,
                                                            uint32_t* __restrict__ g_mask) {
    __shared__ __attribute__((aligned(16))) uint8_t s_flag[kMaxKeyBytes * 256];
    __shared__ uint32_t s_min, s_max;
    {
        uint4* z = reinterpret_cast<uint4*>(s_flag);
        for (int i = threadIdx.x; i < kMaxKeyBytes * 256 / 16; i += kStatsThreads) z[i] = make_uint4(0, 0, 0, 0);
    }
    if (threadIdx.x == 0) { s_min = 0xFFFFFFFFu; s_max = 0; }
    __syncthreads();

    uint32_t mn = 0xFFFFFFFFu, mx = 0;
// ... 898 lines not shown
    }
    mx = wave_max(mx);
    mn = wave_min(mn);
    if (lane_id() == 0) { atomicMax(&s_max, mx); atomicMin(&s_min, mn); }
    lds_atomics_barrier();
    for (int i = threadIdx.x; i < 256; i += kSplitThreads)
        if (s_cnt[i]) atomicAdd(&out->cnt[i], s_cnt[i]);
    for (int i = threadIdx.x; i < kSplitMaxValue * 8; i += kSplitThreads) {
        const uint32_t* f = reinterpret_cast<const uint32_t*>(s_flag + 32 * i);
        uint32_t bits = 0;
#pragma unroll
        for (int x = 0; x < 8; x++) {
            const uint32_t q = f[x];
            bits |= ((q & 1u) | ((q >> 7) & 2u) | ((q >> 14) & 4u) | ((q >> 21) & 8u)) << (4 * x);
        }
        uint32_t* gm = &out->mask[0][0] + i;
        if (bits && (__hip_atomic_load(gm, __ATOMIC_RELAXED, __HIP_MEMORY_SCOPE_AGENT) & bits) != bits) atomicOr(gm, bits);
    }
    if (threadIdx.x == 0) { atomicMax(&out->maxlen, s_max); atomicMax(&out->minlen_inv, ~s_min); }
    if (host_out) {
        __shared__ uint32_t s_last;
        uint32_t* ticket = reinterpret_cast<uint32_t*>(out + 1);
        __threadfence();
        __syncthreads();
        if (threadIdx.x == 0) s_last = atomicAdd(ticket, 1u) == gridDim.x - 1u ? 1u : 0u;
        __syncthreads();
        if (s_last) {
            uint32_t* src = reinterpret_cast<uint32_t*>(out);
            uint32_t* dst = reinterpret_cast<uint32_t*>(host_out);
            for (uint32_t i = threadIdx.x; i < (uint32_t)(sizeof(SplitSample) / 4); i += kSplitThreads) dst[i] = atomicExch(&src[i], 0u);
            if (threadIdx.x == 0) atomicExch(ticket, 0u);
            __threadfence_system();
        }
    }
}

template <class OUT, int NCH, bool PLAIN32 = false>
__global__ __launch_bounds__(kSplitThreads) void k_encode_split(DevCol col, const uint8_t* __restrict__ g_codec, uint64_t n,
                                                               OUT* __restrict__ out, uint32_t tile_rows, uint32_t ntiles,
                                                               uint32_t* __restrict__ counts, uint32_t digit_mask, uint32_t bins,
                                                               int codec_bytes, uint32_t* __restrict__ miss, OUT inv, uint32_t vmax) {
    extern __shared__ __attribute__((aligned(16))) uint8_t smem[];
    const CodecView cv = codec_load_to_lds(g_codec, smem);
    const uint64_t dv = 0x0101010101010101ull * (uint64_t)((uint32_t)cv.hdr->split_byte & 0xFFu);
    const int vp = cv.hdr->split_vcol;
    const int ps = cv.hdr->col_start[vp + 1];
    const uint32_t smaxlen = (uint32_t)cv.hdr->col_maxlen[vp + 1];
    const OUT pmult = (OUT)cv.mult[cv.hdr->wide_pos];
    CPH_LDS OUT* s_lutw = (CPH_LDS OUT*)(smem + codec_bytes);
    uint32_t* s_hist = reinterpret_cast<uint32_t*>(smem + codec_bytes + (size_t)smaxlen * kLutStride * sizeof(OUT));
    for (uint32_t i = threadIdx.x; i < smaxlen * (uint32_t)kLutStride; i += kSplitThreads) {
        const uint32_t r = cv.lut[(uint32_t)ps * kLutStride + i];
        s_lutw[i] = r == kLutInvalid ? inv : (OUT)r * (OUT)cv.mult[ps + (int)(i / kLutStride)];
    }
    __syncthreads();
    const uint32_t hmask = (1u << cv.hdr->wide_hash_bits) - 1u, dmask = (1u << cv.hdr->wide_disp_bits) - 1u;
    const uint32_t per_xcd = (ntiles + 7) / 8, xcd = blockIdx.x & 7u;
    const uint32_t t_end = (xcd + 1) * per_xcd < ntiles ? (xcd + 1) * per_xcd : ntiles;
    uint32_t missed = 0;
    for (uint32_t tile = xcd * per_xcd + (blockIdx.x >> 3); tile < t_end; tile += gridDim.x >> 3) {
        if (counts) {
            for (uint32_t x = threadIdx.x; x < bins; x += kSplitThreads) s_hist[x] = 0;
            __syncthreads();
        }
        const uint64_t tile_end = (uint64_t)(tile + 1) * tile_rows < n ? (uint64_t)(tile + 1) * tile_rows : n;
        for (uint64_t base = (uint64_t)tile * tile_rows; base < tile_end; base += (uint64_t)kSplitThreads * kSplitRows) {
            ValueRegs<NCH> v[kSplitRows];
            {
                uint64_t b[kSplitRows], l[kSplitRows];
                if constexpr (PLAIN32) {
                    const uint32_t* __restrict__ offs = reinterpret_cast<const uint32_t*>(col.offsets);
                    uint32_t o0[kSplitRows], o1[kSplitRows];
#pragma unroll
                    for (int k = 0; k < kSplitRows; k++) {
                        const uint64_t i = base + (uint64_t)k * kSplitThreads + threadIdx.x;
                        const uint64_t r = i < n ? i : n - 1;
                        o0[k] = offs[r];
                        o1[k] = offs[r + 1];
                    }
#pragma unroll
                    for (int k = 0; k < kSplitRows; k++) v[k].load32(col, o0[k], o1[k] - o0[k]);
                } else {
#pragma unroll
                    for (int k = 0; k < kSplitRows; k++) {
                        const uint64_t i = base + (uint64_t)k * kSplitThreads + threadIdx.x;
                        value_span_whole(col, i < n ? i : n - 1, &b[k], &l[k]);
                    }
#pragma unroll
                    for (int k = 0; k < kSplitRows; k++) v[k].load(col, b[k], l[k]);
                }
            }
            uint32_t plen[kSplitRows], slen[kSplitRows], hh[kSplitRows], disp[kSplitRows], e[kSplitRows];
            uint64_t w[kSplitRows][4];
#pragma unroll
            for (int k = 0; k < kSplitRows; k++) {
                split_lengths(v[k], dv, &plen[k], &slen[k]);
                v[k].head_words(plen[k] < (uint32_t)kWideBytes ? plen[k] : (uint32_t)kWideBytes, w[k]);
                hh[k] = wide_hash_lo(w[k][0], w[k][1], w[k][2], w[k][3], plen[k]);
            }
#pragma unroll
            for (int k = 0; k < kSplitRows; k++) disp[k] = cv.wide_disp[hh[k] & dmask];
#pragma unroll
            for (int k = 0; k < kSplitRows; k++) e[k] = cv.wide_hash[((hh[k] >> 16) + disp[k]) & hmask];
            bool hit[kSplitRows];
#pragma unroll
            for (int k = 0; k < kSplitRows; k++) {
                const CPH_LDS WideKey* key = cv.wide + (e[k] ? e[k] - 1 : 0);
                const uint32_t klen = key->len;
                const uint64_t k0 = key->w[0], k1 = key->w[1], k2 = key->w[2];
                uint64_t diff = (k0 ^ w[k][0]) | (k1 ^ w[k][1]) | (k2 ^ w[k][2]);
                if constexpr (NCH > 3) diff |= key->w[3] ^ w[k][3];
                hit[k] = (e[k] != 0) & (klen == plen[k]) & (diff == 0);
            }
            OUT acc[kSplitRows];
            uint64_t w0[kSplitRows], w1[kSplitRows];
#pragma unroll
            for (int k = 0; k < kSplitRows; k++) {
                const bool ok = hit[k] && v[k].len <= vmax && plen[k] <= (uint32_t)kWideBytes && slen[k] <= smaxlen;
                if (!ok && base + (uint64_t)k * kSplitThreads + threadIdx.x < tile_end) missed = 1;
                acc[k] = (OUT)(hit[k] ? e[k] - 1 : 0u) * pmult;
                v[k].window(plen[k], &w0[k], &w1[k]);
            }
            for (uint32_t q = 0; q < smaxlen; q++) {
                const CPH_LDS OUT* lp = s_lutw + q * (uint32_t)kLutStride;
#pragma unroll
                for (int k = 0; k < kSplitRows; k++) {
                    const uint64_t src = q < 8u ? w0[k] : w1[k];
                    const uint32_t sym = q < slen[k] ? ((uint32_t)(src >> (8u * (q & 7u))) & 0xFFu) + 1u : 0u;
                    acc[k] += lp[sym];
                }
            }
#pragma unroll
            for (int k = 0; k < kSplitRows; k++) {
                const uint64_t i = base + (uint64_t)k * kSplitThreads + threadIdx.x;
                if (i < tile_end) {
                    if (inv && acc[k] >= inv) missed = 1;
                    out[i] = acc[k];
                    if (counts) atomicAdd(&s_hist[(uint32_t)acc[k] & digit_mask], 1u);
                }
            }
        }
        if (counts) {
            lds_atomics_barrier();
            for (uint32_t x = threadIdx.x; x < bins; x += kSplitThreads) counts[(uint64_t)x * ntiles + tile] = s_hist[x];
            __syncthreads();
        }
    }
    if (__ballot(missed) && lane_id() == 0) *miss = 1u;
}

constexpr int kFixed8Rows = 8;
constexpr int kFixed8Blocks = 64;
__global__ __launch_bounds__(kSplitThreads) void k_sample_fixed8(DevCol col, uint64_t step, uint64_t n, SplitSample* __restrict__ out,
                                                                SplitSample* __restrict__ host_out) {
    __shared__ uint32_t s_mask[8 * 8];
    __shared__ uint32_t s_last;
    const uint32_t W = col.fixed_width;
    if (threadIdx.x < 64) s_mask[threadIdx.x] = 0;
    __syncthreads();
    const uint64_t stride = (uint64_t)gridDim.x * kSplitThreads;
    for (uint64_t i0 = (uint64_t)blockIdx.x * kSplitThreads + threadIdx.x; i0 < n; i0 += stride * kFixed8Rows) {
        uint64_t c[kFixed8Rows];
#pragma unroll
        for (int k = 0; k < kFixed8Rows; k++) {
            const uint64_t i = i0 + (uint64_t)k * stride;
            ValueRegs<1> v;
            v.load(col, (i < n ? i : i0) * step * W, W);
            c[k] = v.c[0];
        }
        for (uint32_t q = 0; q < W; q++) {
            uint32_t seen[kFixed8Rows];
#pragma unroll
            for (int k = 0; k < kFixed8Rows; k++) {
                const uint32_t byte = (uint32_t)(c[k] >> (8u * q)) & 0xFFu;
                seen[k] = *(volatile CPH_LDS uint32_t*)&s_mask[q * 8u + (byte >> 5)];
            }
#pragma unroll
            for (int k = 0; k < kFixed8Rows; k++) {
                const uint32_t byte = (uint32_t)(c[k] >> (8u * q)) & 0xFFu, bit = 1u << (byte & 31u);
                if (!(seen[k] & bit)) atomicOr(&s_mask[q * 8u + (byte >> 5)], bit);
            }
        }
    }
    lds_atomics_barrier();
    uint32_t* ticket = reinterpret_cast<uint32_t*>(out + 1);
    if (threadIdx.x < 64) {
        const uint32_t bits = s_mask[threadIdx.x];
        uint32_t* gm = &out->mask[0][0] + threadIdx.x;
        if (bits && (__hip_atomic_load(gm, __ATOMIC_RELAXED, __HIP_MEMORY_SCOPE_AGENT) & bits) != bits) atomicOr(gm, bits);
        __builtin_amdgcn_fence(__ATOMIC_RELEASE, "agent");
        asm volatile("s_waitcnt vmcnt(0)" ::: "memory");
        if (threadIdx.x == 0) s_last = atomicAdd(ticket, 1u) == gridDim.x - 1u ? 1u : 0u;
    }
    __syncthreads();
    if (s_last && threadIdx.x < 64) {
        __builtin_amdgcn_fence(__ATOMIC_ACQUIRE, "agent");
        (&host_out->mask[0][0])[threadIdx.x] = atomicExch(&out->mask[0][0] + threadIdx.x, 0u);
        if (threadIdx.x == 0) {
            host_out->maxlen = W;
            host_out->minlen_inv = ~W;
            atomicExch(ticket, 0u);
        }
        __threadfence_system();
    }
}

int codec_virtual_cols(const CodecHost& cd, const DevCol* real, int nreal, DevCol* out) {
    int nv = 0;
    for (int c = 0; c < nreal; c++) {
        if (cd.has_split() && c == cd.split_col) {
            DevCol a = real[c], b = real[c];
            a.split = b.split = (uint16_t)(0x100u | cd.split_byte);
            a.part = 0;
            b.part = 1;
            out[nv++] = a;
            out[nv++] = b;
        } else {
            out[nv++] = real[c];
        }
    }
    return nv;
}

bool codec_wide_perfect_hash(CodecHost* codec) {
    CodecHost& cd = *codec;
    const size_t n = cd.wdict.size();
    cd.wide_disp.clear();
    cd.wide_slots.clear();
    if (n == 0 || n > (size_t)kWideDictMax) return false;
    std::vector<uint32_t> h(n);
    for (size_t i = 0; i < n; i++) h[i] = wide_hash_lo(cd.wdict[i].w[0], cd.wdict[i].w[1], cd.wdict[i].w[2], cd.wdict[i].w[3], cd.wdict[i].len);
    size_t nslots = 4;
    while (nslots < 2 * n) nslots <<= 1;
    for (int attempt = 0; attempt < 3; attempt++, nslots <<= 1) {
        const size_t nbuckets = nslots / 4 > 0 ? nslots / 4 : 1;
        std::vector<std::vector<uint32_t>> bucket(nbuckets);
        for (size_t i = 0; i < n; i++) bucket[h[i] & (nbuckets - 1)].push_back((uint32_t)i);
        std::vector<size_t> order(nbuckets);
        for (size_t b = 0; b < nbuckets; b++) order[b] = b;
        std::sort(order.begin(), order.end(), [&](size_t a, size_t b) { return bucket[a].size() > bucket[b].size(); });
        std::vector<uint16_t> slots(nslots, 0), disp(nbuckets, 0);
        bool ok = true;
        for (size_t b : order) {
            if (bucket[b].empty()) break;
            bool placed = false;
            for (uint32_t d = 0; d < 65536u && !placed; d++) {
                std::vector<uint32_t> at;
                bool free_ = true;
                for (uint32_t i : bucket[b]) {
                    const uint32_t sl = ((h[i] >> 16) + d) & (uint32_t)(nslots - 1);
                    if (slots[sl] || std::find(at.begin(), at.end(), sl) != at.end()) { free_ = false; break; }
                    at.push_back(sl);
                }
                if (!free_) continue;
                for (size_t j = 0; j < at.size(); j++) slots[at[j]] = (uint16_t)(bucket[b][j] + 1);
                disp[b] = (uint16_t)d;
                placed = true;
            }
            if (!placed) { ok = false; break; }
        }
        if (ok) {
            cd.wide_disp = std::move(disp);
            cd.wide_slots = std::move(slots);
            return true;
        }
    }
    return false;
}

static bool wide_less(const WideKey& a, const WideKey& b) {
    const uint32_t m = a.len < b.len ? a.len : b.len;
    for (uint32_t i = 0; i < m; i++) {
        const uint8_t x = (uint8_t)(a.w[i >> 3] >> (8 * (i & 7))), y = (uint8_t)(b.w[i >> 3] >> (8 * (i & 7)));
        if (x != y) return x < y;
    }
    return a.len < b.len;
}

static double codec_sort_cost(const CodecHost& c) {
    if (c.nwords == 1) return (double)((c.word_bits[0] + 7) / 8) * (c.key32 ? 8.0 : 12.0);
    double cost = 0;
    for (int w = 0; w < c.nwords; w++) cost += (double)((c.word_bits[w] + 7) / 8) * 12.0 + 16.0;
    return cost;
}
static double radix_bits(const ColStats& st, uint32_t q) {
    int cnt = q >= st.minlen ? 1 : 0;
    for (int w = 0; w < 8; w++) cnt += __builtin_popcount(st.mask[q][w]);
    return std::log2((double)(cnt > 1 ? cnt : 1));
}

template <int NCH>
static void launch_split_stats(cph_ctx* ctx, const DevCol& col, const SplitCands& cands, uint64_t step, uint64_t rows, SplitSlot* slots, SplitStats* out) {
    uint64_t nblk = (rows + (uint64_t)kSplitThreads * kSplitRows - 1) / ((uint64_t)kSplitThreads * kSplitRows);
    if (nblk > 2048) nblk = 2048;
    if (nblk < 1) nblk = 1;
    hipLaunchKernelGGL((k_split_stats<NCH>), dim3((unsigned)nblk, cands.n), dim3(kSplitThreads), 0, ctx->stream, col, cands, step, rows, slots, out);
}
static double bits_sort_cost(double bits) {
    if (bits <= 32.0) return std::ceil(bits / 8.0) * 8.0;
    if (bits <= 63.0) return std::ceil(bits / 8.0) * 12.0;
    const double words = std::ceil(bits / 63.0);
    return std::ceil(bits / 8.0) * 12.0 + 16.0 * words;
}

static int split_pick(const cph_ctx* ctx, int c, const std::vector<int>& cand, const std::vector<SplitStats>& hs, uint64_t step, double most,
                      double plain_bits) {
    auto split_bits = [&](const SplitStats& st) {
        double bits = std::log2((double)(st.count > 1 ? st.count : 1));
        ColStats tmp{};
        tmp.minlen = ~st.smin_inv;
        memcpy(tmp.mask, st.mask, sizeof st.mask);
        for (uint32_t q = 0; q < st.smax && q < (uint32_t)kSplitMaxSuffix; q++) bits += radix_bits(tmp, q);
        return bits;
    };
    int best = -1;
    double best_bits = 1e30;
    for (size_t k = 0; k < cand.size(); k++) {
        const SplitStats& st = hs[k];
        if (st.flags || st.count == 0 || st.count > (uint32_t)kWideDictMax / (step > 1 ? 2 : 1) || st.smax > (uint32_t)kSplitMaxSuffix) continue;
        const double bits = split_bits(st);
        if (ctx->codec_debug) fprintf(stderr, "codec_try_split: column %d, byte 0x%02x: %u prefixes, suffix %u..%u bytes, %.1f bits (plain %.1f)\n", c, cand[k], st.count, ~st.smin_inv, st.smax, bits, most);
        if (bits < best_bits) { best_bits = bits; best = (int)k; }
    }
    if (best < 0 || bits_sort_cost(plain_bits - most + best_bits) >= bits_sort_cost(plain_bits)) return -1;
    return best;
}

static std::vector<int> split_candidates(const SplitSample& hsm, uint64_t nsel) {
    std::vector<int> cand;
    for (int b = 0; b < 256; b++)
        if ((double)hsm.cnt[b] >= 0.99 * (double)nsel) cand.push_back(b);
    auto alnum = [](int b) { return (b >= '0' && b <= '9') || (b >= 'a' && b <= 'z') || (b >= 'A' && b <= 'Z'); };
    std::sort(cand.begin(), cand.end(), [&](int a, int b) { return alnum(a) != alnum(b) ? !alnum(a) : hsm.cnt[a] > hsm.cnt[b]; });
    if (cand.size() > 8) cand.resize(8);
    return cand;
}

static Status split_assemble(const cph_ctx* ctx, int c, int ncols, const std::vector<ColStats>* stats, uint32_t d, const SplitStats& st,
                             std::vector<WideKey>* dict_io, double plain_bits, CodecHost* out, bool* usable) {
    *usable = false;
    std::vector<WideKey>& dict = *dict_io;
    const uint32_t pmin = ~st.pmin_inv, smin = ~st.smin_inv;
    std::sort(dict.begin(), dict.end(), wide_less);

    std::vector<ColStats> vstats;
    for (int k = 0; k < ncols; k++) {
        if (k != c) { vstats.push_back((*stats)[(size_t)k]); continue; }
        ColStats pre{}, suf{};
        pre.minlen = pmin;
        pre.maxlen = st.pmax;
        for (uint32_t q = 0; q < st.pmax; q++) pre.mask[q][0] = 1u;
        suf.minlen = smin;
        suf.maxlen = st.smax;
        memcpy(suf.mask, st.mask, sizeof st.mask);
        vstats.push_back(pre);
        vstats.push_back(suf);
    }
    uint64_t positions = 0;
    for (const auto& v : vstats) positions += v.maxlen;
    if (positions > (uint64_t)kMaxKeyBytes || st.pmax == 0) return {};
    CodecHost trial;
    CPH_TRY(codec_build(vstats, &trial));
    const int p0 = trial.col_start[c];
    trial.unit.assign((size_t)trial.npos, kUnitPos);
    trial.dict_off.assign((size_t)trial.npos, 0);
    trial.dict_len.assign((size_t)trial.npos, 0);
    trial.unit[(size_t)p0] = kUnitWide;
    trial.radix[(size_t)p0] = (uint16_t)dict.size();
    for (int sym = 0; sym < kLutStride; sym++) trial.lut[(size_t)p0 * kLutStride + (size_t)sym] = kLutInvalid;
    for (uint32_t i = 1; i < st.pmax; i++) {
        trial.unit[(size_t)p0 + i] = kUnitAbsorbed;
        trial.radix[(size_t)p0 + i] = 1;
        for (int sym = 0; sym < kLutStride; sym++) trial.lut[((size_t)p0 + i) * kLutStride + (size_t)sym] = 0;
    }
    trial.split_col = c;
    trial.split_byte = (uint8_t)d;
    trial.split_maxlen = (int32_t)st.vmax;
    trial.wdict = std::move(dict);
    if (!codec_wide_perfect_hash(&trial)) return {};
    CPH_TRY(codec_split_words(&trial));
    if (ctx->codec_debug)
        fprintf(stderr, "codec_try_split: column %d cut at 0x%02x: %zu prefixes (<= %u bytes), suffix %u..%u bytes: %d word(s), %d bits, sort cost %.0f (plain: %.1f bits%s)\n",
                c, d, trial.wdict.size(), st.pmax, smin, st.smax, trial.nwords, trial.word_bits[0], codec_sort_cost(trial), plain_bits,
                stats ? "" : " by the sample");
    *out = std::move(trial);
    *usable = true;
    return {};
}

bool codec_sample_applies(const cph_ctx* ctx, const DevCol* cols, int32_t ncols, uint64_t n) {
    return ctx->stats_sample != 0 && ncols == 1 && cols[0].fixed_width >= 1 && cols[0].fixed_width <= (uint32_t)kSplitMaxValue &&
           !cols[0].segmented() && n >= (1ull << 20);
}
size_t codec_sample_bytes() { return sizeof(SplitSample); }
Status codec_sample_launch(cph_ctx* ctx, const DevCol& col, uint64_t n, const void** host_copy) {
    const uint64_t step = n >> 16;
    const uint64_t nsel = (n + step - 1) / step;
    DevBuf& acc = ctx->self_clean[ctx->stream_slot].sample;
    CPH_TRY(self_clean_block(ctx, &acc, sizeof(SplitSample) + 16));
    uint32_t* hw = host_word(ctx, (uint32_t)(sizeof(SplitSample) / 4));
    if (!hw) return {CPH_ERR_HIP, "no pinned host memory for the sample's statistics"};
    ProfScope ps(ctx, "k_split_count", 0);
    uint64_t nblk = (nsel + kSplitThreads - 1) / kSplitThreads;
    if (nblk > 1024) nblk = 1024;
    if (col.fixed_width <= 8)
        hipLaunchKernelGGL(k_sample_fixed8, dim3((unsigned)std::min<uint64_t>(nblk, (uint64_t)kFixed8Blocks)), dim3(kSplitThreads), 0, ctx->stream, col, step, nsel, acc.as<SplitSample>(),
                           reinterpret_cast<SplitSample*>(hw));
    else
        hipLaunchKernelGGL(k_split_count, dim3((unsigned)nblk), dim3(kSplitThreads), 0, ctx->stream, col, step, nsel, acc.as<SplitSample>(),
                           reinterpret_cast<SplitSample*>(hw));
    if (hipGetLastError() != hipSuccess) {
        acc.reset();
        return {CPH_ERR_HIP, "k_split_count launch failed"};
    }
    *host_copy = hw;
    return {};
}
void codec_sample_finish(const DevCol& col, const void* host_copy, std::vector<ColStats>* out) {
    const SplitSample* sm = static_cast<const SplitSample*>(host_copy);
    out->assign(1, ColStats{});
    ColStats& st = (*out)[0];
    st.minlen = st.maxlen = col.fixed_width;
    static_assert(sizeof(sm->mask) <= sizeof(st.mask), "the sample's positions must fit ColStats");
    memcpy(st.mask, sm->mask, sizeof sm->mask);
}
bool codec_sample_checked(const CodecHost& cd, const DevCol* cols) {
    return !cd.has_split() && !cd.has_groups() && cd.ncols == 1 && cd.nwords == 1 && codec_premultiplied_bits(cd) != 0 && !cols[0].segmented();
}

Status codec_try_split(cph_ctx* ctx, const DevCol* cols, int32_t ncols, uint64_t n, const std::vector<ColStats>* stats, CodecHost* codec,
                       bool speculate, bool* speculated) {
    if (speculated) *speculated = false;
    if (!ctx->codec_split || n < (1ull << 16) || ncols >= kMaxKeyCols) return {};
    if (stats && (codec->key32 || codec->has_groups())) return {};
    if (!stats && ncols != 1) return {};
    int c = -1;
    double most = 0, plain_bits = 0;
    if (stats) {
        for (int k = 0; k < ncols; k++) {
            double bits = 0;
            for (uint32_t q = 0; q < (*stats)[(size_t)k].maxlen; q++) bits += radix_bits((*stats)[(size_t)k], q);
            plain_bits += bits;
            if (cols[k].fixed_width || cols[k].segmented() || (*stats)[(size_t)k].maxlen > (uint32_t)kSplitMaxValue || (*stats)[(size_t)k].maxlen < 4) continue;
            if (bits > most) { most = bits; c = k; }
        }
        if (c < 0 || most < 24.0) return {};
    } else {
        if (cols[0].fixed_width || cols[0].segmented()) return {};
        c = 0;
    }
    const DevCol& col = cols[c];
    const uint64_t step = n > (1ull << 19) ? n >> 18 : 1;
    const uint64_t nsel = (n + step - 1) / step;

    DevBuf sample;
    CPH_TRY(sample.alloc(&ctx->pool, sizeof(SplitSample)));
    CPH_HIP_TRY(hipMemsetAsync(sample.get(), 0, sizeof(SplitSample), ctx->stream));
    {
        ProfScope ps(ctx, "k_split_count", 0);
        uint64_t nblk = (nsel + kSplitThreads - 1) / kSplitThreads;
        if (nblk > 1024) nblk = 1024;
        hipLaunchKernelGGL(k_split_count, dim3((unsigned)nblk), dim3(kSplitThreads), 0, ctx->stream, col, step, nsel, sample.as<SplitSample>(), (SplitSample*)nullptr);
        CPH_HIP_TRY(hipGetLastError());
    }
    CPH_TRY(ensure_pinned_scratch(ctx, sizeof(SplitSample)));
    CPH_HIP_TRY(hipMemcpyAsync(ctx->pinned_scratch, sample.get(), sizeof(SplitSample), hipMemcpyDeviceToHost, ctx->stream));
    CPH_HIP_TRY(hipStreamSynchronize(ctx->stream));
    std::vector<SplitSample> hsv(1);
    SplitSample& hsm = hsv[0];
    memcpy(&hsm, ctx->pinned_scratch, sizeof hsm);
    if (hsm.maxlen > (uint32_t)kSplitMaxValue || hsm.maxlen < 4) return {};
    if (!stats) {
        ColStats tmp{};
        tmp.minlen = ~hsm.minlen_inv;
        memcpy(tmp.mask, hsm.mask, sizeof hsm.mask);
        for (uint32_t q = 0; q < hsm.maxlen; q++) most += radix_bits(tmp, q);
        plain_bits = most;
        if (most <= 32.0) return {};
    }
    const bool small_values = (stats ? (*stats)[(size_t)c].maxlen : hsm.maxlen) <= 24;
    const std::vector<int> cand = split_candidates(hsm, nsel);
    if (cand.empty()) return {};

    const size_t set_bytes = (size_t)kSplitSetSlots * sizeof(SplitSlot);
    DevBuf sets, sstats;
    CPH_TRY(sets.alloc(&ctx->pool, cand.size() * set_bytes));
    CPH_TRY(sstats.alloc(&ctx->pool, cand.size() * sizeof(SplitStats)));
    CPH_HIP_TRY(hipMemsetAsync(sets.get(), 0, cand.size() * set_bytes, ctx->stream));
    CPH_HIP_TRY(hipMemsetAsync(sstats.get(), 0, cand.size() * sizeof(SplitStats), ctx->stream));
    SplitCands all{};
    all.n = (uint32_t)cand.size();
    for (size_t k = 0; k < cand.size(); k++) all.d[k] = (uint8_t)cand[k];
    {
        ProfScope ps(ctx, "k_split_sample", 0);
        if (small_values) launch_split_stats<3>(ctx, col, all, step, nsel, sets.as<SplitSlot>(), sstats.as<SplitStats>());
        else launch_split_stats<5>(ctx, col, all, step, nsel, sets.as<SplitSlot>(), sstats.as<SplitStats>());
        CPH_HIP_TRY(hipGetLastError());
    }
    std::vector<SplitStats> hs(cand.size());
    CPH_TRY(ensure_pinned_scratch(ctx, cand.size() * sizeof(SplitStats)));
    CPH_HIP_TRY(hipMemcpyAsync(ctx->pinned_scratch, sstats.get(), cand.size() * sizeof(SplitStats), hipMemcpyDeviceToHost, ctx->stream));
    CPH_HIP_TRY(hipStreamSynchronize(ctx->stream));
    memcpy(hs.data(), ctx->pinned_scratch, cand.size() * sizeof(SplitStats));
    const int best = split_pick(ctx, c, cand, hs, step, most, plain_bits);
    if (best < 0) return {};

    SplitSlot* slots = sets.as<SplitSlot>() + (size_t)best * kSplitSetSlots;
    SplitStats* dstat = sstats.as<SplitStats>() + best;
    const uint32_t d = (uint32_t)cand[(size_t)best];
    const bool spec = speculate && step > 1 && ctx->split_speculative != 0;
    if (step > 1 && !spec) {
        ProfScope ps(ctx, "k_split_stats", 0);
        SplitCands one{};
        one.n = 1;
        one.d[0] = (uint8_t)d;
        if (small_values) launch_split_stats<3>(ctx, col, one, 1, n, slots, dstat);
        else launch_split_stats<5>(ctx, col, one, 1, n, slots, dstat);
        CPH_HIP_TRY(hipGetLastError());
    }
    CPH_TRY(ensure_pinned_scratch(ctx, sizeof(SplitStats) + set_bytes));
    uint8_t* hp = static_cast<uint8_t*>(ctx->pinned_scratch);
    CPH_HIP_TRY(hipMemcpyAsync(hp, dstat, sizeof(SplitStats), hipMemcpyDeviceToHost, ctx->stream));
    CPH_HIP_TRY(hipMemcpyAsync(hp + sizeof(SplitStats), slots, set_bytes, hipMemcpyDeviceToHost, ctx->stream));
    CPH_HIP_TRY(hipStreamSynchronize(ctx->stream));
    SplitStats st;
    memcpy(&st, hp, sizeof st);
    if (st.flags || st.count == 0 || st.count > (uint32_t)kWideDictMax || st.pmax > (uint32_t)kWideBytes || st.smax > (uint32_t)kSplitMaxSuffix ||
        st.vmax > (uint32_t)kSplitMaxValue)
        return {};
    std::vector<WideKey> dict;
    const SplitSlot* hsl = reinterpret_cast<const SplitSlot*>(hp + sizeof(SplitStats));
    for (int i = 0; i < kSplitSetSlots; i++)
        if (hsl[i].tag) {
            WideKey k{};
            for (int j = 0; j < 4; j++) k.w[j] = hsl[i].w[j];
            k.len = hsl[i].len;
            dict.push_back(k);
        }
    if (dict.size() != st.count) return {};
    CodecHost trial;
    bool usable = false;
    CPH_TRY(split_assemble(ctx, c, ncols, stats, d, st, &dict, plain_bits, &trial, &usable));
    if (!usable) return {};
    if (spec) {
        trial.spec_checked = true;
        if (trial.nwords != 1 || trial.word_states[0] > (trial.key32 ? (1ull << 27) : (1ull << 58)))
            return codec_try_split(ctx, cols, ncols, n, stats, codec, false, nullptr);
    }
    const double plain_cost = stats ? codec_sort_cost(*codec) : bits_sort_cost(plain_bits);
    if (codec_sort_cost(trial) < plain_cost) {
        *codec = std::move(trial);
        if (speculated) *speculated = spec;
    }
    return {};
}

Status codec_split_from_host(cph_ctx* ctx, const cph_host::HostCol& hc, uint64_t n, cph_host::BlockPool& pool, CodecHost* codec) {
    if (!ctx->codec_split || !ctx->split_speculative || hc.fixed_width || !hc.offsets || n < (1ull << 22)) return {};
    const uint64_t step = n >> 18;
    const uint64_t nsel = (n + step - 1) / step;
// ... 35 lines not shown
        }
        std::lock_guard<std::mutex> lk(mu);
        for (int b = 0; b < 256; b++) hsm.cnt[b] += loc.cnt[b];
        hsm.maxlen = loc.maxlen > hsm.maxlen ? loc.maxlen : hsm.maxlen;
        hsm.minlen_inv = loc.minlen_inv > hsm.minlen_inv ? loc.minlen_inv : hsm.minlen_inv;
        for (int q = 0; q < kSplitMaxValue; q++)
            for (int w = 0; w < 8; w++) hsm.mask[q][w] |= loc.mask[q][w];
    }, 2048);
    if (hsm.maxlen > (uint32_t)kSplitMaxValue || hsm.maxlen < 4) return {};
    double most = 0;
    {
        ColStats tmp{};
        tmp.minlen = ~hsm.minlen_inv;
        memcpy(tmp.mask, hsm.mask, sizeof hsm.mask);
        for (uint32_t q = 0; q < hsm.maxlen; q++) most += radix_bits(tmp, q);
    }
    const double plain_bits = most;
    if (most <= 32.0) return {};
    const std::vector<int> cand = split_candidates(hsm, nsel);
    if (cand.empty()) return {};

    std::vector<SplitStats> hs(cand.size());
    std::vector<std::vector<WideKey>> dicts(cand.size());
    std::vector<std::vector<uint64_t>> dtags(cand.size());
    for (auto& x : hs) memset(&x, 0, sizeof x);
    pool.run(nsel, [&](uint64_t i0, uint64_t i1) {
        const size_t nc = cand.size();
        std::vector<SplitStats> loc(nc);
        for (auto& x : loc) memset(&x, 0, sizeof x);
        constexpr size_t kSlots = 4096;
        std::vector<uint64_t> tags(nc * kSlots, 0ull);
        std::vector<WideKey> keys(nc * kSlots);
        std::vector<uint32_t> nkeys(nc, 0);
        constexpr uint64_t kBatch = 32;
        uint64_t bb[kBatch], ll[kBatch];
        for (uint64_t i = i0; i < i1; i++) {
            if ((i - i0) % kBatch == 0) {
                const uint64_t m2 = i1 - i < kBatch ? i1 - i : kBatch;
                for (uint64_t k = 0; k < m2; k++) __builtin_prefetch(static_cast<const uint8_t*>(hc.offsets) + (i + k) * step * (uint64_t)(hc.offset_bits / 8));
                for (uint64_t k = 0; k < m2; k++) {
                    span((i + k) * step, &bb[k], &ll[k]);
                    __builtin_prefetch(hc.data + bb[k]);
                }
            }
            const uint64_t b = bb[(i - i0) % kBatch], l = ll[(i - i0) % kBatch];
            const uint8_t* p = hc.data + b;
            for (size_t k = 0; k < nc; k++) {
                SplitStats& st = loc[k];
                const void* f = l ? memchr(p, cand[k], (size_t)l) : nullptr;
                const uint64_t plen = f ? (uint64_t)((const uint8_t*)f - p) + 1 : l, slen = l - plen;
                const bool usable = l <= (uint64_t)kSplitMaxValue && plen <= (uint64_t)kWideBytes;
                if (!usable) st.flags |= 1u;
                if (slen > (uint64_t)kSplitMaxSuffix) st.flags |= 2u;
                st.rows_with += f ? 1u : 0u;
                const uint32_t pl = plen > 0xFFFFFFFFull ? 0xFFFFFFFFu : (uint32_t)plen, sl = slen > 0xFFFFFFFFull ? 0xFFFFFFFFu : (uint32_t)slen;
                const uint32_t vl = l > 0xFFFFFFFFull ? 0xFFFFFFFFu : (uint32_t)l;
                st.pmin_inv = ~pl > st.pmin_inv ? ~pl : st.pmin_inv;
                st.pmax = pl > st.pmax ? pl : st.pmax;
                st.smin_inv = ~sl > st.smin_inv ? ~sl : st.smin_inv;
                st.smax = sl > st.smax ? sl : st.smax;
                st.vmax = vl > st.vmax ? vl : st.vmax;
                if (usable && !(st.flags & 4u)) {
                    WideKey key{};
                    memcpy(key.w, p, (size_t)plen);
                    key.len = pl;
                    const uint64_t tag = wide_hash(key.w[0], key.w[1], key.w[2], key.w[3], pl);
                    uint64_t* tg = &tags[k * kSlots];
                    WideKey* ky = &keys[k * kSlots];
                    size_t h = (size_t)(tag >> 32) & (kSlots - 1);
                    while (tg[h] != 0ull && !(tg[h] == tag && ky[h].len == pl && memcmp(ky[h].w, key.w, sizeof key.w) == 0)) h = (h + 1) & (kSlots - 1);
                    if (tg[h] == 0ull) {
                        if (nkeys[k] >= (uint32_t)kWideDictMax) st.flags |= 4u;
                        else { tg[h] = tag; ky[h] = key; nkeys[k]++; }
                    }
                }
                const uint64_t lim = slen < (uint64_t)kSplitMaxSuffix ? slen : (uint64_t)kSplitMaxSuffix;
                for (uint64_t q = 0; q < lim; q++) {
                    const uint8_t v = p[plen + q];
                    st.mask[q][v >> 5] |= 1u << (v & 31);
                }
            }
        }
        std::lock_guard<std::mutex> lk(mu);
        for (size_t k = 0; k < nc; k++) {
            SplitStats& g = hs[k];
            const SplitStats& st = loc[k];
            g.flags |= st.flags;
            g.rows_with += st.rows_with;
            g.pmin_inv = st.pmin_inv > g.pmin_inv ? st.pmin_inv : g.pmin_inv;
            g.pmax = st.pmax > g.pmax ? st.pmax : g.pmax;
            g.smin_inv = st.smin_inv > g.smin_inv ? st.smin_inv : g.smin_inv;
            g.smax = st.smax > g.smax ? st.smax : g.smax;
            g.vmax = st.vmax > g.vmax ? st.vmax : g.vmax;
            for (int q = 0; q < kSplitMaxSuffix; q++)
                for (int w = 0; w < 8; w++) g.mask[q][w] |= st.mask[q][w];
            if (dtags[k].empty()) { dtags[k].assign(kSlots, 0ull); dicts[k].assign(kSlots, WideKey{}); }
            for (size_t s2 = 0; s2 < kSlots && !(g.flags & 4u); s2++) {
                const uint64_t tag = tags[k * kSlots + s2];
                if (!tag) continue;
                const WideKey& key = keys[k * kSlots + s2];
                size_t h = (size_t)(tag >> 32) & (kSlots - 1);
                while (dtags[k][h] != 0ull && !(dtags[k][h] == tag && dicts[k][h].len == key.len && memcmp(dicts[k][h].w, key.w, sizeof key.w) == 0)) h = (h + 1) & (kSlots - 1);
                if (dtags[k][h] == 0ull) {
                    if (g.count >= (uint32_t)kWideDictMax) g.flags |= 4u;
                    else { dtags[k][h] = tag; dicts[k][h] = key; g.count++; }
                }
            }
        }
    }, 2048);
    const int best = split_pick(ctx, 0, cand, hs, step, most, plain_bits);
    if (best < 0) return {};
    const SplitStats& st = hs[(size_t)best];
    if (st.flags || st.count == 0 || st.count > (uint32_t)kWideDictMax || st.pmax > (uint32_t)kWideBytes || st.smax > (uint32_t)kSplitMaxSuffix ||
        st.vmax > (uint32_t)kSplitMaxValue)
        return {};
    std::vector<WideKey> dict;
    for (size_t s2 = 0; s2 < dtags[(size_t)best].size(); s2++)
        if (dtags[(size_t)best][s2]) dict.push_back(dicts[(size_t)best][s2]);
    if (dict.size() != st.count) return {};
    CodecHost trial;
    bool usable = false;
    CPH_TRY(split_assemble(ctx, 0, 1, nullptr, (uint32_t)cand[(size_t)best], st, &dict, plain_bits, &trial, &usable));
    if (!usable) return {};
    trial.spec_checked = true;
    if (trial.nwords != 1 || !trial.key32 || trial.word_states[0] > (1ull << 27)) return {};
    if (codec_sort_cost(trial) < bits_sort_cost(plain_bits)) *codec = std::move(trial);
    return {};
}

int codec_premultiplied_bits(const CodecHost& cd) {
    if (cd.nwords != 1 || cd.npos <= 0 || cd.has_groups()) return 0;
    const int bits = cd.word_states[0] <= (1ull << 31) ? 32 : 64;
    return (size_t)cd.npos * kLutStride * (size_t)(bits / 8) <= 48 * 1024 ? bits : 0;
}

void codec_arith_plan(const CodecHost& cd, ArithPlan* ap) {
    *ap = ArithPlan{};
    if (cd.ncols != 1 || cd.nwords != 1 || cd.has_groups() || cd.npos < 1 || cd.npos > 8) return;
    if (cd.col_minlen[0] != cd.col_maxlen[0] || cd.word_states[0] > (1ull << 31)) return;
    uint32_t lo[8] = {0}, rng[8] = {0}, radix[8] = {1, 1, 1, 1, 1, 1, 1, 1};
    for (int p = 0; p < cd.npos; p++) {
        const uint16_t* lut = &cd.lut[(size_t)p * kLutStride];
        if (lut[0] != kLutInvalid) return;
        int first = -1, last = -1, count = 0;
        for (int b = 0; b < 256; b++)
            if (lut[1 + b] != kLutInvalid) { if (first < 0) first = b; last = b; count++; }
        if (first < 0 || last >= 0x80 || last - first + 1 != count || count > 255 || count != (int)cd.radix[(size_t)p]) return;
        for (int b = first; b <= last; b++)
            if (lut[1 + b] != (uint16_t)(b - first)) return;
        lo[p] = (uint32_t)first;
        rng[p] = (uint32_t)(last - first);
        radix[p] = (uint32_t)count;
    }
    ap->keylen = (uint32_t)cd.npos;
    for (int w = 0; w < 2; w++) {
        for (int i = 0; i < 4; i++) {
            const int p = 4 * w + i;
            if (p < cd.npos) ap->keep[w] |= 0xFFu << (8 * i);
            ap->lo[w] |= lo[p] << (8 * i);
            ap->rngc[w] |= (0x7Fu - rng[p]) << (8 * i);
        }
        ap->wa[w] = radix[4 * w + 1] | 1u << 8;
        ap->wb[w] = radix[4 * w + 3] << 16 | 1u << 24;
        ap->ma[w] = radix[4 * w + 2] * radix[4 * w + 3];
    }
    const uint64_t s0 = (uint64_t)radix[0] * radix[1] * radix[2] * radix[3];
    const uint64_t s1 = (uint64_t)radix[4] * radix[5] * radix[6] * radix[7];
    ap->s1 = (uint32_t)s1;
    ap->mul24 = s0 <= (1ull << 24) && s1 < (1ull << 24) ? 1u : 0u;
    ap->enabled = 1;
}

Status codec_upload(cph_ctx* ctx, const CodecHost& cd, DevBuf* dev) {
    CodecDevHeader h{};
    h.ncols = cd.ncols;
    h.npos = cd.npos;
    h.nwords = cd.nwords;
    h.key32 = cd.key32 ? 1 : 0;
    for (int c = 0; c <= cd.ncols; c++) h.col_start[c] = cd.col_start[c];
    for (int c = cd.ncols + 1; c <= kMaxKeyCols; c++) h.col_start[c] = cd.npos;
    for (int c = 0; c < cd.ncols; c++) h.col_maxlen[c] = cd.col_maxlen[c];
    auto align16 = [](size_t x) { return (x + 15) & ~(size_t)15; };
    size_t off = align16(sizeof(CodecDevHeader));
    h.mult_off = (int32_t)off;
    off = align16(off + sizeof(uint64_t) * (size_t)cd.npos);
    h.wordof_off = (int32_t)off;
    off = align16(off + (size_t)cd.npos + 1);
    const int lutw_bits = codec_premultiplied_bits(cd);
    h.lutw_bits = lutw_bits;
    if (lutw_bits) {
        h.lut_off = 0;
        h.lutw_off = (int32_t)off;
        off = align16(off + (size_t)(lutw_bits / 8) * (size_t)cd.npos * kLutStride);
    } else {
        h.lutw_off = 0;
        h.lut_off = (int32_t)off;
        off = align16(off + sizeof(uint16_t) * (size_t)cd.npos * kLutStride);
    }
    if (cd.has_groups()) {
        h.ngroups = 0;
        for (int p = 0; p < cd.npos; p++) h.ngroups += cd.unit[(size_t)p] == kUnitHead || cd.unit[(size_t)p] == kUnitWide;
        h.unit_off = (int32_t)off;
        off = align16(off + (size_t)cd.npos);
        h.dictoff_off = (int32_t)off;
        off = align16(off + sizeof(int32_t) * (size_t)cd.npos);
        h.dictlen_off = (int32_t)off;
        off = align16(off + sizeof(int32_t) * (size_t)cd.npos);
        h.dict_off = (int32_t)off;
        off = align16(off + sizeof(uint64_t) * cd.dict.size());
        h.hashoff_off = (int32_t)off;
        off = align16(off + sizeof(int32_t) * (size_t)cd.npos);
        h.hashbits_off = (int32_t)off;
        off = align16(off + sizeof(int32_t) * (size_t)cd.npos);
        h.hash_off = (int32_t)off;
        size_t slots = 0;
        for (int p = 0; p < cd.npos; p++)
            if (cd.unit[(size_t)p] == kUnitHead) slots += (size_t)1 << (bits_needed((uint64_t)cd.dict_len[(size_t)p] * 2) + 0);
        off = align16(off + sizeof(uint16_t) * slots);
    }
    h.wide_pos = -1;
    h.split_vcol = -1;
    int wide_bits = 0;
    if (cd.has_split()) {
        h.split_vcol = cd.split_col;
        h.split_byte = cd.split_byte;
        h.wide_pos = cd.col_start[cd.split_col];
        h.wide_n = (int32_t)cd.wdict.size();
        h.wide_off = (int32_t)off;
        off = align16(off + sizeof(WideKey) * cd.wdict.size());
        if (cd.wide_slots.empty() || cd.wide_disp.empty()) return {CPH_ERR_INVALID, "internal: split codec without its perfect hash"};
        wide_bits = bits_needed((uint64_t)cd.wide_slots.size());
        h.wide_hash_bits = wide_bits;
        h.wide_hash_off = (int32_t)off;
        off = align16(off + sizeof(uint16_t) * cd.wide_slots.size());
        h.wide_disp_bits = bits_needed((uint64_t)cd.wide_disp.size());
        h.wide_disp_off = (int32_t)off;
        off = align16(off + sizeof(uint16_t) * cd.wide_disp.size());
    }
    h.total_bytes = (int32_t)off;

    std::vector<uint8_t> blob(off, 0);
    memcpy(blob.data(), &h, sizeof h);
    if (cd.has_split()) {
        memcpy(blob.data() + h.wide_off, cd.wdict.data(), sizeof(WideKey) * cd.wdict.size());
        memcpy(blob.data() + h.wide_hash_off, cd.wide_slots.data(), sizeof(uint16_t) * cd.wide_slots.size());
        memcpy(blob.data() + h.wide_disp_off, cd.wide_disp.data(), sizeof(uint16_t) * cd.wide_disp.size());
    }
    if (cd.has_groups()) {
        memcpy(blob.data() + h.unit_off, cd.unit.data(), (size_t)cd.npos);
        memcpy(blob.data() + h.dictoff_off, cd.dict_off.data(), sizeof(int32_t) * (size_t)cd.npos);
        memcpy(blob.data() + h.dictlen_off, cd.dict_len.data(), sizeof(int32_t) * (size_t)cd.npos);
        memcpy(blob.data() + h.dict_off, cd.dict.data(), sizeof(uint64_t) * cd.dict.size());
        int32_t* hoff = reinterpret_cast<int32_t*>(blob.data() + h.hashoff_off);
        int32_t* hbits = reinterpret_cast<int32_t*>(blob.data() + h.hashbits_off);
        uint16_t* hash = reinterpret_cast<uint16_t*>(blob.data() + h.hash_off);
        size_t base = 0;
        for (int p = 0; p < cd.npos; p++) {
            if (cd.unit[(size_t)p] != kUnitHead) continue;
            const int bits = bits_needed((uint64_t)cd.dict_len[(size_t)p] * 2);
            const uint32_t mask = (1u << bits) - 1u;
            hoff[p] = (int32_t)base;
            hbits[p] = bits;
            for (int32_t r = 0; r < cd.dict_len[(size_t)p]; r++) {
                uint32_t sl = bits ? group_slot(cd.dict[(size_t)(cd.dict_off[(size_t)p] + r)], bits) : 0u;
                while (hash[base + sl]) sl = (sl + 1) & mask;
                hash[base + sl] = (uint16_t)(r + 1);
            }
            base += (size_t)1 << bits;
        }
    }
    if (cd.npos) {
        memcpy(blob.data() + h.mult_off, cd.mult.data(), sizeof(uint64_t) * (size_t)cd.npos);
        for (int p = 0; p < cd.npos; p++) blob[(size_t)h.wordof_off + (size_t)p] = (uint8_t)cd.word_of[(size_t)p];
        blob[(size_t)h.wordof_off + (size_t)cd.npos] = 0xFF;
        if (lutw_bits == 32) {
            uint32_t* w = reinterpret_cast<uint32_t*>(blob.data() + h.lutw_off);
            for (size_t i = 0; i < (size_t)cd.npos * kLutStride; i++) {
                const uint16_t r = cd.lut[i];
                w[i] = r == kLutInvalid ? 0x80000000u : (uint32_t)((uint64_t)r * cd.mult[i / kLutStride]);
            }
        } else if (lutw_bits == 64) {
            uint64_t* w = reinterpret_cast<uint64_t*>(blob.data() + h.lutw_off);
            for (size_t i = 0; i < (size_t)cd.npos * kLutStride; i++) {
                const uint16_t r = cd.lut[i];
                w[i] = r == kLutInvalid ? 0x8000000000000000ull : (uint64_t)r * cd.mult[i / kLutStride];
            }
        } else {
            memcpy(blob.data() + h.lut_off, cd.lut.data(), sizeof(uint16_t) * (size_t)cd.npos * kLutStride);
        }
    }
    CPH_TRY(dev->alloc(&ctx->pool, off));
    void* slot = nullptr;
    CPH_TRY(pinned_upload(ctx, off, &slot));
    memcpy(slot, blob.data(), off);
    CPH_HIP_TRY(hipMemcpyAsync(dev->get(), slot, off, hipMemcpyHostToDevice, ctx->stream));
    return {};
}

constexpr int kEncodeThreads = 256;

template <bool KEY32>
__global__ __launch_bounds__(kEncodeThreads) void k_encode_build(ColsArg cols, const uint8_t* __restrict__ g_codec,
                                                                uint64_t n, void* __restrict__ out, uint32_t* __restrict__ miss) {
    extern __shared__ __attribute__((aligned(16))) uint8_t smem[];
    const CodecView cv = codec_load_to_lds(g_codec, smem);
    const int ncols = cv.hdr->ncols;
    const uint64_t stride = (uint64_t)gridDim.x * kEncodeThreads;
    bool all_valid = true;
    for (uint64_t row = (uint64_t)blockIdx.x * kEncodeThreads + threadIdx.x; row < n; row += stride) {
        if constexpr (KEY32) {
            uint32_t code = 0;
            all_valid &= encode_key(cv, cols, ncols, row, [&](int, uint64_t v, int) { code = (uint32_t)v; });
            reinterpret_cast<uint32_t*>(out)[row] = code;
        } else {
            uint64_t* o = reinterpret_cast<uint64_t*>(out);
            if (cv.hdr->npos == 0) o[row] = 0;
            all_valid &= encode_key(cv, cols, ncols, row, [&](int word, uint64_t v, int) { o[(uint64_t)word * n + row] = v; });
        }
    }
    if (miss && !all_valid) *miss = 1u;
}

constexpr int kEncodeRows = 4;
// ... 464 lines not shown
```

csvplus_amd/csrc/window_sort.hip:

```cpp
#include "cph_internal.hpp"
#include "codec_device.hpp"
#include "device_utils.hpp"

namespace cph {

constexpr int kWpThreads = 512;
constexpr int kWpItems = 16;
constexpr int kWpThreadsOneLevel = 1024;
constexpr int kWpItemsOneLevel = 8;
constexpr int kWpTile = kWpThreads * kWpItems;
static_assert(kWpThreadsOneLevel * kWpItemsOneLevel == kWpTile, "one tile size");
constexpr int kWpMaxBuckets = 2048;
constexpr int kWinBits = 14;
constexpr uint32_t kWinSlots = 1u << kWinBits;
constexpr uint32_t kWinEmpty = 0xFFFFFFFFu;
constexpr int kPlaceThreads = 512;

struct WpArgs {
    const uint64_t* keys;
    ArithPlan ap;
    const uint32_t* codes;
    const uint64_t* entries;
    const uint32_t* src_count;
    uint64_t n;
    uint32_t src_cap;
    uint32_t tiles_per_src;
    uint32_t shift;
    uint32_t nb;
    uint64_t* dst;
    uint32_t* dst_count;
    uint32_t states;
    uint32_t row_base;
    uint32_t* flag;
};

template <int SRC, int THREADS, int ITEMS>
__global__ __launch_bounds__(THREADS) void k_win_partition(WpArgs a) {
    constexpr bool FROM_CODES = SRC != 0;
    constexpr int TILE = THREADS * ITEMS;
    extern __shared__ __attribute__((aligned(16))) uint8_t smem[];
    __shared__ uint32_t s_tmp[THREADS / kWave + 1];
    const uint32_t nbp = (a.nb + (uint32_t)THREADS - 1u) & ~((uint32_t)THREADS - 1u);
    uint64_t* s_ent = reinterpret_cast<uint64_t*>(smem);
    uint32_t* s_hist = reinterpret_cast<uint32_t*>(s_ent + TILE);
    uint32_t* s_start = s_hist + nbp;
    uint32_t* s_delta = s_start + nbp;
    const uint32_t sb = blockIdx.x / a.tiles_per_src, tl = blockIdx.x % a.tiles_per_src;
    uint64_t cnt = a.n;
    if constexpr (!FROM_CODES) {
        const uint32_t c = a.src_count[sb];
        cnt = c < a.src_cap ? c : a.src_cap;
    }
    const uint64_t t0 = (uint64_t)tl * TILE;
    if (t0 >= cnt) return;
    const uint32_t m = cnt - t0 < (uint64_t)TILE ? (uint32_t)(cnt - t0) : (uint32_t)TILE;
    const uint64_t src0 = FROM_CODES ? t0 : (uint64_t)sb * a.src_cap + t0;
    const uint32_t t = threadIdx.x;
    for (uint32_t i = t; i < nbp; i += THREADS) s_hist[i] = 0;
    __syncthreads();
    typedef unsigned int u32x4 __attribute__((ext_vector_type(4)));
    uint32_t code[ITEMS], row[ITEMS], rank[ITEMS];
    if constexpr (SRC == 2) {
        uint64_t c0[ITEMS];
        uint32_t okm = 0;
#pragma unroll
        for (int j = 0; j < ITEMS / 4; j++) {
            const uint32_t i4 = 4u * ((uint32_t)j * THREADS + t);
            if (i4 + 3 < m) {
                const u32x4 v0 = reinterpret_cast<const u32x4*>(a.keys + src0 + i4)[0], v1 = reinterpret_cast<const u32x4*>(a.keys + src0 + i4)[1];
                c0[4 * j] = (uint64_t)v0.x | ((uint64_t)v0.y << 32);
                c0[4 * j + 1] = (uint64_t)v0.z | ((uint64_t)v0.w << 32);
                c0[4 * j + 2] = (uint64_t)v1.x | ((uint64_t)v1.y << 32);
                c0[4 * j + 3] = (uint64_t)v1.z | ((uint64_t)v1.w << 32);
                okm |= 0xFu << (4 * j);
            } else {
#pragma unroll
                for (int c = 0; c < 4; c++) {
                    c0[4 * j + c] = i4 + c < m ? a.keys[src0 + i4 + c] : 0ull;
                    okm |= (i4 + c < m ? 1u : 0u) << (4 * j + c);
                }
            }
#pragma unroll
            for (int c = 0; c < 4; c++) row[4 * j + c] = a.row_base + (uint32_t)(t0 + i4 + c);
        }
        const uint32_t have = okm;
        encode_rows_arith<ITEMS, uint32_t>(a.ap, c0, code, &okm);
        bool bad = false;
#pragma unroll
        for (int k = 0; k < ITEMS; k++) {
            const bool ok = ((okm >> k) & 1u) && code[k] < a.states;
            bad |= ((have >> k) & 1u) && !ok;
            code[k] = ok ? code[k] : kWinEmpty;
        }
        if (__ballot(bad) && lane_id() == 0) *a.flag = 1u;
    } else if constexpr (SRC == 1) {
        const bool vec = m == (uint32_t)TILE && (((uintptr_t)(a.codes + src0)) & 15) == 0;
#pragma unroll
        for (int j = 0; j < ITEMS / 4; j++) {
            const uint32_t i4 = 4u * ((uint32_t)j * THREADS + t);
            uint32_t w[4];
            if (vec) {
                const u32x4 v = reinterpret_cast<const u32x4*>(a.codes + src0)[i4 >> 2];
                w[0] = v.x; w[1] = v.y; w[2] = v.z; w[3] = v.w;
            } else {
#pragma unroll
                for (int c = 0; c < 4; c++) w[c] = i4 + c < m ? a.codes[src0 + i4 + c] : kWinEmpty;
            }
#pragma unroll
            for (int c = 0; c < 4; c++) {
                const bool ok = i4 + c < m && w[c] < a.states;
                code[4 * j + c] = ok ? w[c] : kWinEmpty;
                row[4 * j + c] = a.row_base + (uint32_t)(t0 + i4 + c);
            }
        }
    } else {
        const bool vec = m == (uint32_t)TILE;
#pragma unroll
        for (int j = 0; j < ITEMS / 2; j++) {
            const uint32_t i2 = 2u * ((uint32_t)j * THREADS + t);
            if (vec) {
                const u32x4 v = reinterpret_cast<const u32x4*>(a.entries + src0)[i2 >> 1];
                row[2 * j] = v.x; code[2 * j] = v.y; row[2 * j + 1] = v.z; code[2 * j + 1] = v.w;
            } else {
#pragma unroll
                for (int c = 0; c < 2; c++) {
                    const uint64_t e = i2 + c < m ? a.entries[src0 + i2 + c] : ~0ull;
                    row[2 * j + c] = (uint32_t)e;
                    code[2 * j + c] = i2 + c < m ? (uint32_t)(e >> 32) : kWinEmpty;
                }
            }
        }
    }
#pragma unroll
    for (int k = 0; k < ITEMS; k++) rank[k] = code[k] != kWinEmpty ? atomicAdd(&s_hist[code[k] >> a.shift], 1u) : 0u;
    lds_atomics_barrier();
    uint32_t tot;
    {
        const uint32_t per = nbp / THREADS;
        uint32_t h[kWpMaxBuckets / THREADS], sum = 0;
#pragma unroll
        for (int k = 0; k < kWpMaxBuckets / THREADS; k++) {
            h[k] = (uint32_t)k < per ? s_hist[t * per + k] : 0u;
            sum += h[k];
        }
        uint32_t run = block_exclusive_sum<uint32_t, THREADS>(sum, s_tmp, &tot);
#pragma unroll
        for (int k = 0; k < kWpMaxBuckets / THREADS; k++) {
            if ((uint32_t)k < per) {
                const uint32_t b = t * per + k;
                s_start[b] = run;
                if (h[k]) s_delta[b] = atomicAdd(&a.dst_count[(uint64_t)sb * a.nb + b], h[k]) - run;
                run += h[k];
            }
        }
    }
    __syncthreads();
#pragma unroll
    for (int k = 0; k < ITEMS; k++)
        if (code[k] != kWinEmpty) s_ent[s_start[code[k] >> a.shift] + rank[k]] = ((uint64_t)code[k] << 32) | row[k];
    __syncthreads();
    const uint32_t cap = 1u << a.shift, mask = cap - 1u;
    bool over = false;
    uint64_t e[ITEMS];
    uint32_t pos[ITEMS];
#pragma unroll
    for (int k = 0; k < ITEMS; k++) {
        const uint32_t i = (uint32_t)k * THREADS + t;
        e[k] = s_ent[i < tot ? i : 0u];
    }
#pragma unroll
    for (int k = 0; k < ITEMS; k++) {
        const uint32_t i = (uint32_t)k * THREADS + t;
        pos[k] = s_delta[i < tot ? (uint32_t)(e[k] >> 32) >> a.shift : 0u] + i;
    }
#pragma unroll
    for (int k = 0; k < ITEMS; k++) {
        const uint32_t i = (uint32_t)k * THREADS + t;
        if (i < tot) {
            const uint32_t w = (uint32_t)(e[k] >> 32), b = w >> a.shift;
            if (pos[k] < cap) a.dst[(((uint64_t)sb * a.nb + b) << a.shift) + pos[k]] = ((uint64_t)(w & mask) << 32) | (uint32_t)e[k];
            else over = true;
        }
    }
    if (__ballot(over) && lane_id() == 0) *a.flag = 1u;
}

__global__ __launch_bounds__(1024) void k_win_offsets(const uint32_t* __restrict__ counts, uint32_t nwin, uint32_t* __restrict__ off) {
    __shared__ uint32_t s_tmp[1024 / kWave + 1];
    uint32_t carry = 0;
    for (uint32_t base = 0; base < nwin; base += 1024) {
        const uint32_t i = base + threadIdx.x;
        uint32_t v = i < nwin ? counts[i] : 0u;
        v = v < kWinSlots ? v : kWinSlots;
        uint32_t total;
        const uint32_t ex = block_exclusive_sum<uint32_t, 1024>(v, s_tmp, &total);
        if (i < nwin) off[i] = carry + ex;
        carry += total;
    }
}

__global__ __launch_bounds__(kPlaceThreads) void k_win_place(const uint64_t* __restrict__ entries, uint32_t* __restrict__ counts,
                                                            const uint32_t* __restrict__ off, uint64_t n, uint32_t* __restrict__ perm,
                                                            uint32_t* __restrict__ sorted, uint32_t* __restrict__ flag,
                                                            uint32_t* __restrict__ clear_also, uint32_t nclear, uint2* __restrict__ ranktab,
                                                            uint32_t rank_blocks) {
    extern __shared__ __attribute__((aligned(16))) uint8_t smem[];
    __shared__ uint32_t s_wcount[kPlaceThreads / kWave];
    typedef unsigned int u32x4 __attribute__((ext_vector_type(4)));
    uint32_t* win = reinterpret_cast<uint32_t*>(smem);
    const uint32_t g = blockIdx.x, t = threadIdx.x;
    const uint32_t craw = counts[g], cnt = craw < kWinSlots ? craw : kWinSlots;
    {
        u32x4 e;
        e.x = e.y = e.z = e.w = kWinEmpty;
        for (uint32_t i = t; i < kWinSlots / 4; i += kPlaceThreads) reinterpret_cast<u32x4*>(win)[i] = e;
    }
    __syncthreads();
    if (t == 0) {
        counts[g] = 0u;
        if (g < nclear) clear_also[g] = 0u;
    }
    const uint64_t* src = entries + ((uint64_t)g << kWinBits);
    for (uint32_t i = t; i < cnt; i += kPlaceThreads) {
        const uint64_t e = src[i];
        win[(uint32_t)(e >> 32) & (kWinSlots - 1u)] = (uint32_t)e;
    }
    __syncthreads();
    constexpr uint32_t kWaves = kPlaceThreads / kWave, kPerWave = kWinSlots / kWaves, kIters = kPerWave / kWave;
    const uint32_t wave = (uint32_t)wave_id(), lane = (uint32_t)lane_id();
    const uint32_t s0 = wave * kPerWave;
    uint32_t c = 0;
#pragma unroll 4
    for (uint32_t it = 0; it < kIters; it++) c += (uint32_t)__popcll(__ballot(win[s0 + it * kWave + lane] != kWinEmpty));
    if (lane == 0) s_wcount[wave] = c;
    __syncthreads();
    uint32_t before = 0, filled = 0;
#pragma unroll
    for (uint32_t w = 0; w < kWaves; w++) {
        const uint32_t x = s_wcount[w];
        before += w < wave ? x : 0u;
        filled += x;
    }
    if (t == 0 && (filled != craw)) *flag = 1u;
    uint64_t pos = (off ? (uint64_t)off[g] : ((uint64_t)g << kWinBits)) + before;
    const uint64_t lt = lanemask_lt();
    const uint32_t code0 = (g << kWinBits) + s0;
    for (uint32_t it = 0; it < kIters; it++) {
        const uint32_t v = win[s0 + it * kWave + lane];
        const uint64_t bal = __ballot(v != kWinEmpty);
        if (ranktab && lane < 2) {
            const uint32_t blk = ((code0 + it * kWave) >> 5) + lane;
            if (blk < rank_blocks)
                ranktab[blk] = make_uint2(lane ? (uint32_t)(bal >> 32) : (uint32_t)bal, (uint32_t)pos + (lane ? (uint32_t)__popc((uint32_t)bal) : 0u));
        }
        if (v != kWinEmpty) {
            const uint64_t p = pos + (uint64_t)__popcll(bal & lt);
            if (p < n) {
                perm[p] = v;
                sorted[p] = code0 + it * kWave + lane;
            }
        }
        pos += (uint64_t)__popcll(bal);
    }
}

Status WindowSort::begin(cph_ctx* ctx, uint64_t n_, uint64_t states_) {
    n = n_;
    states = states_;
    const uint64_t nwin = (states + kWinSlots - 1) >> kWinBits;
    two = nwin > (uint64_t)kWpMaxBuckets;
    int k2 = 0;
    if (two) {
        int wb = 0;
        while ((1ull << wb) < nwin) wb++;
        k2 = (wb + 1) / 2;
    }
    nb2 = 1u << k2;
    shift1 = (uint32_t)kWinBits + (uint32_t)k2;
    nb1 = two ? (states + (1ull << shift1) - 1) >> shift1 : nwin;
    if (nb1 > (uint64_t)kWpMaxBuckets) return {CPH_ERR_INVALID, "direct_sort_windows: code space too large"};
    nwin_total = two ? nb1 * nb2 : nwin;
    CPH_TRY(ent1.alloc(&ctx->pool, (nb1 << shift1) * sizeof(uint64_t)));
    if (two) CPH_TRY(ent2.alloc(&ctx->pool, (nwin_total << kWinBits) * sizeof(uint64_t)));
    const uint64_t nwords = nb1 + (two ? nwin_total : 0);
    words = &ctx->self_clean[ctx->stream_slot].win;
    CPH_TRY(self_clean_block(ctx, words, nwords * sizeof(uint32_t)));
    cur1 = words->as<uint32_t>();
    cur2 = two ? cur1 + nb1 : cur1;
    started = true;
    return {};
}
WindowSort::~WindowSort() {
    if (started && !finished && words) words->reset();
}

template <int SRC, int THREADS, int ITEMS>
static Status win_partition_launch(cph_ctx* ctx, const WpArgs& a, unsigned grid, double bytes) {
    const uint32_t nbp = (a.nb + (uint32_t)THREADS - 1u) & ~((uint32_t)THREADS - 1u);
    const size_t lds = (size_t)THREADS * ITEMS * 8 + (size_t)nbp * 12;
    CPH_TRY(kernel_setup(ctx, reinterpret_cast<const void*>(&k_win_partition<SRC, THREADS, ITEMS>), THREADS, lds, nullptr));
    ProfScope ps(ctx, "k_win_partition", bytes);
    hipLaunchKernelGGL((k_win_partition<SRC, THREADS, ITEMS>), dim3(grid), dim3(THREADS), lds, ctx->stream, a);
    return {};
}

Status WindowSort::add(cph_ctx* ctx, const uint32_t* codes, uint64_t row0, uint64_t m, uint32_t* flag, const uint64_t* keys, const ArithPlan* ap) {
    if (m == 0) return {};
    WpArgs a{};
    a.codes = codes;
    a.keys = keys;
    if (keys) a.ap = *ap;
    a.n = m;
    a.tiles_per_src = (uint32_t)((m + kWpTile - 1) / kWpTile);
    a.shift = shift1;
    a.nb = (uint32_t)nb1;
    a.dst = ent1.as<uint64_t>();
    a.dst_count = cur1;
    a.states = (uint32_t)states;
    a.row_base = (uint32_t)row0;
    a.flag = flag;
    if (keys) {
        if (two) CPH_TRY((win_partition_launch<2, kWpThreads, kWpItems>(ctx, a, a.tiles_per_src, 16.0 * (double)m)));
        else CPH_TRY((win_partition_launch<2, kWpThreadsOneLevel, kWpItemsOneLevel>(ctx, a, a.tiles_per_src, 16.0 * (double)m)));
    } else {
        if (two) CPH_TRY((win_partition_launch<1, kWpThreads, kWpItems>(ctx, a, a.tiles_per_src, 12.0 * (double)m)));
        else CPH_TRY((win_partition_launch<1, kWpThreadsOneLevel, kWpItemsOneLevel>(ctx, a, a.tiles_per_src, 12.0 * (double)m)));
    }
    CPH_HIP_TRY(hipGetLastError());
    return {};
}

Status WindowSort::finish(cph_ctx* ctx, uint32_t* perm_out, uint32_t* sorted_out, uint32_t* flag, void* ranktab, uint64_t rank_blocks) {
    const bool need_off = states != n;
    DevBuf offsets;
    if (need_off) CPH_TRY(offsets.alloc(&ctx->pool, nwin_total * sizeof(uint32_t)));
    uint32_t* off = offsets.as<uint32_t>();
    if (two) {
        WpArgs a{};
        a.entries = ent1.as<uint64_t>();
        a.src_count = cur1;
        a.src_cap = 1u << shift1;
        a.tiles_per_src = (a.src_cap + kWpTile - 1) / kWpTile;
        a.shift = (uint32_t)kWinBits;
        a.nb = nb2;
        a.dst = ent2.as<uint64_t>();
        a.dst_count = cur2;
        a.flag = flag;
        CPH_TRY((win_partition_launch<0, kWpThreads, kWpItems>(ctx, a, (unsigned)(nb1 * a.tiles_per_src), 16.0 * (double)n)));
        CPH_HIP_TRY(hipGetLastError());
    }
    uint32_t* counts = two ? cur2 : cur1;
    if (need_off) {
        ProfScope ps(ctx, "k_win_place", 0);
        hipLaunchKernelGGL(k_win_offsets, dim3(1), dim3(1024), 0, ctx->stream, counts, (uint32_t)nwin_total, off);
    }
    {
        const size_t lds = (size_t)kWinSlots * sizeof(uint32_t);
        CPH_TRY(kernel_setup(ctx, reinterpret_cast<const void*>(&k_win_place), kPlaceThreads, lds, nullptr));
        ProfScope ps(ctx, "k_win_place", 16.0 * (double)n);
        hipLaunchKernelGGL(k_win_place, dim3((unsigned)nwin_total), dim3(kPlaceThreads), lds, ctx->stream, two ? ent2.as<uint64_t>() : ent1.as<uint64_t>(),
                           counts, need_off ? off : nullptr, n, perm_out, sorted_out, flag, cur1, two ? (uint32_t)nb1 : 0u,
                           static_cast<uint2*>(ranktab), (uint32_t)rank_blocks);
    }
    CPH_HIP_TRY(hipGetLastError());
    finished = true;
    return {};
}

Status direct_sort_windows(cph_ctx* ctx, const uint32_t* codes, uint64_t n, uint64_t states, uint32_t* perm_out, uint32_t* sorted_out,
                           uint32_t* flag, void* ranktab, uint64_t rank_blocks) {
    if (n == 0) return {};
    WindowSort ws;
    CPH_TRY(ws.begin(ctx, n, states));
    CPH_TRY(ws.add(ctx, codes, 0, n, flag));
    return ws.finish(ctx, perm_out, sorted_out, flag, ranktab, rank_blocks);
}
Status direct_sort_windows_keys(cph_ctx* ctx, const uint64_t* keys, const ArithPlan& ap, uint64_t n, uint64_t states, uint32_t* perm_out,
                                uint32_t* sorted_out, uint32_t* flag, void* ranktab, uint64_t rank_blocks) {
    if (n == 0) return {};
    WindowSort ws;
    CPH_TRY(ws.begin(ctx, n, states));
    CPH_TRY(ws.add(ctx, nullptr, 0, n, flag, keys, &ap));
    return ws.finish(ctx, perm_out, sorted_out, flag, ranktab, rank_blocks);
}

}

namespace cph {
void warm_window_sort() {
    hipFuncAttributes a;
    (void)hipFuncGetAttributes(&a, reinterpret_cast<const void*>(&k_win_offsets));
    (void)hipGetLastError();
}
}
```

Baseline: 149.0 billion rows/s.

## Speculatively launch direct window sort from device-computed plan before host stats sync

The sampling kernel now derives an arithmetic codec plan and a state count on the device and writes a DirectPlan to device memory and to pinned host memory. For unique fixed-width-8 key builds, the partition, offsets and place kernels are launched right away, reading the plan from device memory, so no host round-trip is needed before the sort. The host later checks the device plan against its own codec and adopts the sorted output, or discards it and reruns the normal path. This removes a stream synchronize and host planning gap from the build's critical path. The cost is extra kernel variants, wasted work when the plan is declined, and a new fallback recursion.

New measurement: 147.3 billion rows/s. 1.1% lower.

```diff
diff --git a/csvplus_amd/csrc/capi.hip b/csvplus_amd/csrc/capi.hip
--- a/csvplus_amd/csrc/capi.hip
+++ b/csvplus_amd/csrc/capi.hip
@@ -525,6 +525,14 @@
     bool exact_split = false;
     bool no_split = false;
     uint32_t* miss = nullptr;
+    bool planned = false;
+    bool have_sample = false;
+    DirectPlan* plan_host = nullptr;
+    DevBuf plan_dev, sp_ent, sp_off, sp_perm, sp_sorted, sp_rt;
+    void drop_planned() {
+        planned = false;
+        plan_dev.reset(); sp_ent.reset(); sp_off.reset(); sp_perm.reset(); sp_sorted.reset(); sp_rt.reset();
+    }
     uint32_t* cs_over = nullptr;
     DevBuf cs_codes;
 };
@@ -544,8 +552,18 @@
         job->presplit = ix->codec.has_split();
     }
     job->sampled = !job->small && !job->presplit && !job->no_sample && codec_sample_applies(ctx, job->dcols, nkeycols, ix->nrows);
-    if (job->sampled) CPH_TRY(codec_sample_launch(ctx, job->dcols[0], ix->nrows, &job->sample_host));
-    else if (!job->small && !job->presplit) CPH_TRY(codec_stats_launch(ctx, job->dcols, nkeycols, &job->stats_dev));
+    if (job->sampled) {
+        const DevCol& kc = job->dcols[0];
+        const uint64_t n = ix->nrows;
+        job->planned = ctx->direct_spec && job->unique && !job->no_direct && ctx->direct_sort == 1 && ctx->direct_fused_encode && nkeycols == 1 &&
+                       kc.fixed_width == 8 && !kc.segmented() && ((uintptr_t)kc.data & 15) == 0 && n >= (1ull << 20) && n <= (1ull << 25);
+        if (job->planned) {
+            CPH_TRY(job->plan_dev.alloc(&ctx->pool, sizeof(DirectPlan)));
+            job->plan_host = reinterpret_cast<DirectPlan*>(host_word(ctx, (uint32_t)(sizeof(DirectPlan) / 4)));
+            if (!job->plan_host) return {CPH_ERR_HIP, "no pinned host memory for the report words of a build"};
+        }
+        CPH_TRY(codec_sample_launch(ctx, kc, n, &job->sample_host, job->plan_dev.as<DirectPlan>(), job->plan_host));
+    } else if (!job->small && !job->presplit) CPH_TRY(codec_stats_launch(ctx, job->dcols, nkeycols, &job->stats_dev));
     return {};
 }
 
@@ -555,6 +573,50 @@
     return job->miss ? Status{} : Status{CPH_ERR_HIP, "no pinned host memory for the report words of a build"};
 }
 static Status build_encode_sort(cph_ctx* ctx, BuildJob* job);
+
+static Status planned_launch(cph_ctx* ctx, BuildJob* job) {
+    const uint64_t n = job->ix->nrows;
+    CPH_TRY(job_arm_miss(ctx, job));
+    CPH_TRY(job->sp_perm.alloc(&ctx->pool, n * sizeof(uint32_t)));
+    CPH_TRY(job->sp_sorted.alloc(&ctx->pool, n * sizeof(uint32_t)));
+    if (ctx->direct_ranktab && !job->sp_rt.alloc(&ctx->pool, ranktab_blocks(planned_max_states(n)) * 8).ok()) job->sp_rt.reset();
+    return direct_sort_windows_planned(ctx, reinterpret_cast<const uint64_t*>(job->dcols[0].data), n, job->plan_dev.as<DirectPlan>(),
+                                       job->sp_perm.as<uint32_t>(), job->sp_sorted.as<uint32_t>(), job->miss, job->sp_rt.get(), &job->sp_ent, &job->sp_off);
+}
+static Status planned_finish(cph_ctx* ctx, BuildJob* job, bool* adopt) {
+    *adopt = false;
+    cph_index* ix = job->ix;
+    const uint64_t n = ix->nrows;
+    DirectPlan dp;
+    memcpy(&dp, job->plan_host, sizeof dp);
+    std::vector<ColStats> stats;
+    codec_sample_finish(job->dcols[0], job->sample_host, &stats);
+    CPH_TRY(codec_build(stats, &ix->codec));
+    const CodecHost& cd = ix->codec;
+    ArithPlan ap{};
+    bool host_ok = false;
+    uint64_t states = 0;
+    if (codec_sample_checked(cd, job->dcols) && cd.nwords == 1) {
+        states = cd.word_states[0];
+        const bool direct = cd.key32 && !job->spec.active && n >= (1ull << 16) && states >= n && states <= 2 * n && states < 0xFFFFFFFFull;
+        codec_arith_plan(cd, &ap);
+        host_ok = direct && ap.enabled && ap.keylen == 8 && ((states + (1ull << kWinBits) - 1) >> kWinBits) <= (uint64_t)kWpMaxBuckets;
+    }
+    *adopt = host_ok && dp.accept == 1u && (uint64_t)dp.states == states && memcmp(&dp.ap, &ap, sizeof ap) == 0;
+    if (!*adopt) {
+        if (dp.accept == 1u) ctx->n_plan_disagree++;
+        ix->codec = CodecHost{};
+        job->drop_planned();
+        job->miss = nullptr;
+        return {};
+    }
+    ix->sorted_codes = std::move(job->sp_sorted);
+    ix->perm = std::move(job->sp_perm);
+    ix->sort_passes = 0;
+    if (states != n && job->sp_rt) ix->ranktab = std::move(job->sp_rt);
+    job->drop_planned();
+    return codec_upload(ctx, cd, &ix->codec_dev);
+}
 
 static size_t job_readback_bytes(const BuildJob& j) {
     return j.small ? sizeof(SmallResult) : (j.presplit || j.sampled) ? 0 : sizeof(ColStats) * (size_t)j.nkeycols;
@@ -590,13 +652,23 @@
                                       hipMemcpyDeviceToHost, jobs[i].side ? ctx->side_stream : ctx->stream);
         if (e != hipSuccess) status[i] = {CPH_ERR_HIP, std::string("statistics read-back: ") + hipGetErrorString(e)};
     }
+    for (size_t i = 0; i < nj; i++)
+        if (status[i].ok() && jobs[i].planned) {
+            SideStream on_side(ctx, jobs[i].side);
+            status[i] = planned_launch(ctx, &jobs[i]);
+        }
     bool any_side = false;
     for (size_t i = 0; i < nj; i++) any_side = any_side || jobs[i].side;
     auto sync_streams = [&]() {
         return hipStreamSynchronize(ctx->stream) == hipSuccess && (!any_side || hipStreamSynchronize(ctx->side_stream) == hipSuccess);
     };
-    if (!sync_streams()) return fail_all({CPH_ERR_HIP, "hipStreamSynchronize failed"});
-    ctx->pool.flush_deferred();
+    bool need_main = false, need_side = false;
+    for (size_t i = 0; i < nj; i++)
+        if (status[i].ok() && !jobs[i].planned && !jobs[i].have_sample) (jobs[i].side ? need_side : need_main) = true;
+    if ((need_main && hipStreamSynchronize(ctx->stream) != hipSuccess) || (need_side && hipStreamSynchronize(ctx->side_stream) != hipSuccess))
+        return fail_all({CPH_ERR_HIP, "hipStreamSynchronize failed"});
+    if (need_main && (need_side || !any_side))
+        ctx->pool.flush_deferred();
     std::vector<std::vector<uint8_t>> stats_host(nj);
     std::vector<size_t> retry;
     for (size_t i = 0; i < nj; i++) {
@@ -610,6 +682,7 @@
             else if (status[i].ok()) index_plan_table(jobs[i].ix);
             continue;
         }
+        if (jobs[i].planned) continue;
         if (jobs[i].sampled) {
             const uint8_t* sh = static_cast<const uint8_t*>(jobs[i].sample_host);
             stats_host[i].assign(sh, sh + codec_sample_bytes());
@@ -618,12 +691,13 @@
         }
     }
     for (size_t i = 0; i < nj; i++)
-        if (status[i].ok() && !jobs[i].small) {
+        if (status[i].ok() && !jobs[i].small && !jobs[i].planned) {
             SideStream on_side(ctx, jobs[i].side);
             status[i] = build_phase2(ctx, &jobs[i], stats_host[i].data());
         }
     std::vector<size_t> resplit;
     std::vector<size_t> resort;
+    std::vector<size_t> declined;
     if (any_general) {
         s = ensure_pinned_scratch(ctx, 2 * sizeof(uint32_t) * nj + 64);
         if (!s.ok()) return fail_all(s);
@@ -643,6 +717,12 @@
         for (size_t i = 0; i < nj; i++) {
             if (!status[i].ok() || jobs[i].small) continue;
             cph_index* ix = jobs[i].ix;
+            if (jobs[i].planned) {
+                bool adopt = false;
+                status[i] = planned_finish(ctx, &jobs[i], &adopt);
+                if (!status[i].ok()) continue;
+                if (!adopt) { declined.push_back(i); continue; }
+            }
             if (jobs[i].miss) sm[i] = *(volatile uint32_t*)jobs[i].miss;
             if (sm[i]) { jobs[i].cs_codes.reset(); jobs[i].cs_over = nullptr; resplit.push_back(i); continue; }
             if (jobs[i].cs_over && *(volatile uint32_t*)jobs[i].cs_over) { resort.push_back(i); continue; }
@@ -707,6 +787,16 @@
         if (r.ok()) index_plan_table(ix);
         status[i] = r;
     }
+    for (size_t i : declined) {
+        std::vector<BuildJob> one;
+        one.push_back(std::move(jobs[i]));
+        std::vector<Status> st1(1);
+        one[0].side = false;
+        one[0].have_sample = true;
+        build_run(ctx, one, st1);
+        status[i] = st1[0];
+        jobs[i] = std::move(one[0]);
+    }
     for (size_t i : resplit) {
         std::vector<BuildJob> one;
         one.push_back(std::move(jobs[i]));
@@ -719,6 +809,7 @@
         j.no_split = !again_exact;
         j.no_sample = true;
         j.sampled = false;
+        j.have_sample = false;
         j.no_direct = true;
         j.presplit = false;
         j.miss = nullptr;
@@ -1122,6 +1213,7 @@
     else if (k == "chain_identity") ctx->chain_identity = value != 0;
     else if (k == "chain_prejoin") ctx->chain_prejoin = value != 0;
     else if (k == "direct_fused_encode") ctx->direct_fused_encode = value != 0;
+    else if (k == "direct_spec") ctx->direct_spec = value != 0;
     else if (k == "direct_ranktab") ctx->direct_ranktab = value != 0;
     else if (k == "hash_load_pct") ctx->hash_load_pct = value < 25 ? 25 : value > 90 ? 90 : (int)value;
     else if (k == "small_build_rows") ctx->small_build_rows = value < 0 ? 0 : value > (1 << 20) ? (1 << 20) : (int)value;
@@ -1311,7 +1403,7 @@
     if (!specs || !out || nspecs < 1 || nspecs > 64) return fail(ctx, {CPH_ERR_INVALID, "bad cph_index_build_many arguments"});
     std::vector<BuildJob> jobs((size_t)nspecs);
     std::vector<Status> st((size_t)nspecs);
-    if (!host_words_reserve(ctx, (uint32_t)nspecs * (uint32_t)(codec_sample_bytes() / 4 + 16)))
+    if (!host_words_reserve(ctx, (uint32_t)nspecs * (uint32_t)(codec_sample_bytes() / 4 + 16 + (sizeof(DirectPlan) + 7) / 4)))
         return fail(ctx, {CPH_ERR_INVALID, "cph_index_build_many: the batch needs more report words than the ctx holds"});
     bool two_streams = nspecs >= 2 && ctx->build_side_stream != 0;
     if (two_streams && !ctx->side_stream && hipStreamCreateWithFlags(&ctx->side_stream, hipStreamNonBlocking) != hipSuccess) {
diff --git a/csvplus_amd/csrc/codec_device.hpp b/csvplus_amd/csrc/codec_device.hpp
--- a/csvplus_amd/csrc/codec_device.hpp
+++ b/csvplus_amd/csrc/codec_device.hpp
@@ -394,6 +394,44 @@
 };
 
 void codec_arith_plan(const CodecHost& codec, ArithPlan* ap);
+
+__host__ __device__ inline void arith_plan_pack(uint32_t npos, const uint32_t (&lo)[8], const uint32_t (&rng)[8], const uint32_t (&radix)[8],
+                                                ArithPlan* ap) {
+    ap->enabled = 0;
+    ap->mul24 = 0;
+    ap->keylen = npos;
+#pragma unroll
+    for (int w = 0; w < 2; w++) {
+        uint32_t keep = 0, l = 0, r = 0;
+#pragma unroll
+        for (int i = 0; i < 4; i++) {
+            const int p = 4 * w + i;
+            if ((uint32_t)p < npos) keep |= 0xFFu << (8 * i);
+            l |= lo[p] << (8 * i);
+            r |= (0x7Fu - rng[p]) << (8 * i);
+        }
+        ap->keep[w] = keep;
+        ap->lo[w] = l;
+        ap->rngc[w] = r;
+        ap->wa[w] = radix[4 * w + 1] | 1u << 8;
+        ap->wb[w] = radix[4 * w + 3] << 16 | 1u << 24;
+        ap->ma[w] = radix[4 * w + 2] * radix[4 * w + 3];
+    }
+    const uint64_t s0 = (uint64_t)radix[0] * radix[1] * radix[2] * radix[3];
+    const uint64_t s1 = (uint64_t)radix[4] * radix[5] * radix[6] * radix[7];
+    ap->s1 = (uint32_t)s1;
+    ap->mul24 = s0 <= (1ull << 24) && s1 < (1ull << 24) ? 1u : 0u;
+    ap->enabled = 1;
+}
+
+constexpr int kWpMaxBuckets = 2048;
+constexpr int kWinBits = 14;
+struct DirectPlan {
+    ArithPlan ap;
+    uint32_t states;
+    uint32_t nwin;
+    uint32_t accept;
+};
 
 template <int R, class CW>
 __device__ __forceinline__ void encode_rows_arith(const ArithPlan& ap, const uint64_t (&c0)[R], CW (&code)[R], uint32_t* okmask) {
diff --git a/csvplus_amd/csrc/cph_internal.hpp b/csvplus_amd/csrc/cph_internal.hpp
--- a/csvplus_amd/csrc/cph_internal.hpp
+++ b/csvplus_amd/csrc/cph_internal.hpp
@@ -275,6 +275,8 @@
     uint64_t n_split_respec = 0;
     int hash_load_pct = 50;
     int direct_fused_encode = 1;
+    int direct_spec = 1;
+    uint64_t n_plan_disagree = 0;
     int direct_ranktab = 1;
     int chain_prejoin = 1;
     int split_speculative = 1;
@@ -446,7 +448,9 @@
 Status codec_build(const std::vector<ColStats>& stats, CodecHost* codec);
 bool codec_sample_applies(const cph_ctx* ctx, const DevCol* cols, int32_t ncols, uint64_t n);
 size_t codec_sample_bytes();
-Status codec_sample_launch(cph_ctx* ctx, const DevCol& col, uint64_t n, const void** host_copy);
+struct DirectPlan;
+Status codec_sample_launch(cph_ctx* ctx, const DevCol& col, uint64_t n, const void** host_copy, DirectPlan* plan = nullptr,
+                           DirectPlan* plan_host = nullptr);
 void codec_sample_finish(const DevCol& col, const void* host_copy, std::vector<ColStats>* out);
 bool codec_sample_checked(const CodecHost& codec, const DevCol* cols);
 struct GroupChoice { int t, p0, span; double saved; uint32_t count; uint32_t tab; };
@@ -513,6 +517,9 @@
                                 uint32_t* sorted_out, uint32_t* flag, void* ranktab = nullptr, uint64_t rank_blocks = 0);
 Status direct_sort_windows(cph_ctx* ctx, const uint32_t* codes, uint64_t n, uint64_t states, uint32_t* perm_out, uint32_t* sorted_out,
                            uint32_t* flag, void* ranktab = nullptr, uint64_t rank_blocks = 0);
+uint64_t planned_max_states(uint64_t n);
+Status direct_sort_windows_planned(cph_ctx* ctx, const uint64_t* keys, uint64_t n, const DirectPlan* plan, uint32_t* perm_out, uint32_t* sorted_out,
+                                   uint32_t* flag, void* ranktab, DevBuf* ent, DevBuf* off);
 struct WindowSort {
     Status begin(cph_ctx* ctx, uint64_t n, uint64_t states);
     Status add(cph_ctx* ctx, const uint32_t* codes, uint64_t row0, uint64_t m, uint32_t* flag, const uint64_t* keys = nullptr, const ArithPlan* ap = nullptr);
diff --git a/csvplus_amd/csrc/keycodec.hip b/csvplus_amd/csrc/keycodec.hip
--- a/csvplus_amd/csrc/keycodec.hip
+++ b/csvplus_amd/csrc/keycodec.hip
@@ -1074,7 +1074,8 @@
 constexpr int kFixed8Rows = 8;
 constexpr int kFixed8Blocks = 64;
 __global__ __launch_bounds__(kSplitThreads) void k_sample_fixed8(DevCol col, uint64_t step, uint64_t n, SplitSample* __restrict__ out,
-                                                                SplitSample* __restrict__ host_out) {
+                                                                SplitSample* __restrict__ host_out, DirectPlan* __restrict__ plan,
+                                                                DirectPlan* __restrict__ plan_host, uint64_t table_rows) {
     __shared__ uint32_t s_mask[8 * 8];
     __shared__ uint32_t s_last;
     const uint32_t W = col.fixed_width;
@@ -1117,11 +1118,49 @@
     __syncthreads();
     if (s_last && threadIdx.x < 64) {
         __builtin_amdgcn_fence(__ATOMIC_ACQUIRE, "agent");
-        (&host_out->mask[0][0])[threadIdx.x] = atomicExch(&out->mask[0][0] + threadIdx.x, 0u);
+        const uint32_t bits = atomicExch(&out->mask[0][0] + threadIdx.x, 0u);
+        (&host_out->mask[0][0])[threadIdx.x] = bits;
         if (threadIdx.x == 0) {
             host_out->maxlen = W;
             host_out->minlen_inv = ~W;
             atomicExch(ticket, 0u);
+        }
+        if (plan) {
+            const uint32_t b0 = (threadIdx.x & 7u) * 32u;
+            uint32_t cnt = (uint32_t)__popc(bits);
+            uint32_t first = bits ? b0 + (uint32_t)__builtin_ctz(bits) : 0xFFFFFFFFu;
+            uint32_t last = bits ? b0 + 31u - (uint32_t)__builtin_clz(bits) : 0u;
+#pragma unroll
+            for (int d = 1; d < 8; d <<= 1) {
+                cnt += (uint32_t)__shfl_xor((int)cnt, d);
+                const uint32_t f = (uint32_t)__shfl_xor((int)first, d), l = (uint32_t)__shfl_xor((int)last, d);
+                first = f < first ? f : first;
+                last = l > last ? l : last;
+            }
+            uint32_t lo[8], rng[8], radix[8];
+            bool ok = true;
+            uint64_t states = 1;
+#pragma unroll
+            for (int p = 0; p < 8; p++) {
+                const uint32_t c = (uint32_t)__shfl((int)cnt, 8 * p), f = (uint32_t)__shfl((int)first, 8 * p), l = (uint32_t)__shfl((int)last, 8 * p);
+                const bool okp = c >= 1u && l < 0x80u && l - f + 1u == c && c <= 255u;
+                ok = ok && okp;
+                lo[p] = okp ? f : 0u;
+                rng[p] = okp ? l - f : 0u;
+                radix[p] = okp ? c : 1u;
+                states *= radix[p];
+            }
+            if (threadIdx.x == 0) {
+                DirectPlan dp;
+                arith_plan_pack(8u, lo, rng, radix, &dp.ap);
+                const uint64_t nwin = (states + (1ull << kWinBits) - 1) >> kWinBits;
+                const bool acc = ok && states <= (1ull << 31) && table_rows <= states && states <= 2 * table_rows && nwin <= (uint64_t)kWpMaxBuckets;
+                dp.states = acc ? (uint32_t)states : 0u;
+                dp.nwin = acc ? (uint32_t)nwin : 0u;
+                dp.accept = acc ? 1u : 0u;
+                *plan = dp;
+                *plan_host = dp;
+            }
         }
         __threadfence_system();
     }
@@ -1315,7 +1354,7 @@
            !cols[0].segmented() && n >= (1ull << 20);
 }
 size_t codec_sample_bytes() { return sizeof(SplitSample); }
-Status codec_sample_launch(cph_ctx* ctx, const DevCol& col, uint64_t n, const void** host_copy) {
+Status codec_sample_launch(cph_ctx* ctx, const DevCol& col, uint64_t n, const void** host_copy, DirectPlan* plan, DirectPlan* plan_host) {
     const uint64_t step = n >> 16;
     const uint64_t nsel = (n + step - 1) / step;
     DevBuf& acc = ctx->self_clean[ctx->stream_slot].sample;
@@ -1327,7 +1366,7 @@
     if (nblk > 1024) nblk = 1024;
     if (col.fixed_width <= 8)
         hipLaunchKernelGGL(k_sample_fixed8, dim3((unsigned)std::min<uint64_t>(nblk, (uint64_t)kFixed8Blocks)), dim3(kSplitThreads), 0, ctx->stream, col, step, nsel, acc.as<SplitSample>(),
-                           reinterpret_cast<SplitSample*>(hw));
+                           reinterpret_cast<SplitSample*>(hw), col.fixed_width == 8 ? plan : nullptr, plan_host, n);
     else
         hipLaunchKernelGGL(k_split_count, dim3((unsigned)nblk), dim3(kSplitThreads), 0, ctx->stream, col, step, nsel, acc.as<SplitSample>(),
                            reinterpret_cast<SplitSample*>(hw));
@@ -1669,23 +1708,7 @@
         rng[p] = (uint32_t)(last - first);
         radix[p] = (uint32_t)count;
     }
-    ap->keylen = (uint32_t)cd.npos;
-    for (int w = 0; w < 2; w++) {
-        for (int i = 0; i < 4; i++) {
-            const int p = 4 * w + i;
-            if (p < cd.npos) ap->keep[w] |= 0xFFu << (8 * i);
-            ap->lo[w] |= lo[p] << (8 * i);
-            ap->rngc[w] |= (0x7Fu - rng[p]) << (8 * i);
-        }
-        ap->wa[w] = radix[4 * w + 1] | 1u << 8;
-        ap->wb[w] = radix[4 * w + 3] << 16 | 1u << 24;
-        ap->ma[w] = radix[4 * w + 2] * radix[4 * w + 3];
-    }
-    const uint64_t s0 = (uint64_t)radix[0] * radix[1] * radix[2] * radix[3];
-    const uint64_t s1 = (uint64_t)radix[4] * radix[5] * radix[6] * radix[7];
-    ap->s1 = (uint32_t)s1;
-    ap->mul24 = s0 <= (1ull << 24) && s1 < (1ull << 24) ? 1u : 0u;
-    ap->enabled = 1;
+    arith_plan_pack((uint32_t)cd.npos, lo, rng, radix, ap);
 }
 
 Status codec_upload(cph_ctx* ctx, const CodecHost& cd, DevBuf* dev) {
diff --git a/csvplus_amd/csrc/window_sort.hip b/csvplus_amd/csrc/window_sort.hip
--- a/csvplus_amd/csrc/window_sort.hip
+++ b/csvplus_amd/csrc/window_sort.hip
@@ -10,17 +10,23 @@
 constexpr int kWpItemsOneLevel = 8;
 constexpr int kWpTile = kWpThreads * kWpItems;
 static_assert(kWpThreadsOneLevel * kWpItemsOneLevel == kWpTile, "one tile size");
-constexpr int kWpMaxBuckets = 2048;
-constexpr int kWinBits = 14;
 constexpr uint32_t kWinSlots = 1u << kWinBits;
 constexpr uint32_t kWinEmpty = 0xFFFFFFFFu;
 constexpr int kPlaceThreads = 512;
+
+template <int SRC, int THREADS>
+__host__ __device__ constexpr uint32_t wp_bucket_words(uint32_t nb) {
+    return SRC == 3 ? (nb + 63u) & ~63u : (nb + (uint32_t)THREADS - 1u) & ~((uint32_t)THREADS - 1u);
+}
 
 struct WpArgs {
     const uint64_t* keys;
     ArithPlan ap;
     const uint32_t* codes;
-    const uint64_t* entries;
+    union {
+        const uint64_t* entries;
+        const DirectPlan* plan;
+    };
     const uint32_t* src_count;
     uint64_t n;
     uint32_t src_cap;
@@ -38,9 +44,19 @@
 __global__ __launch_bounds__(THREADS) void k_win_partition(WpArgs a) {
     constexpr bool FROM_CODES = SRC != 0;
     constexpr int TILE = THREADS * ITEMS;
+    ArithPlan ap_dev;
+    uint32_t states_dev = 0;
+    if constexpr (SRC == 3) {
+        const DirectPlan* __restrict__ pl = a.plan;
+        if (pl->accept == 0u) return;
+        ap_dev = pl->ap;
+        states_dev = pl->states;
+    }
+    const ArithPlan& ap = SRC == 3 ? ap_dev : a.ap;
+    const uint32_t states = SRC == 3 ? states_dev : a.states;
     extern __shared__ __attribute__((aligned(16))) uint8_t smem[];
     __shared__ uint32_t s_tmp[THREADS / kWave + 1];
-    const uint32_t nbp = (a.nb + (uint32_t)THREADS - 1u) & ~((uint32_t)THREADS - 1u);
+    const uint32_t nbp = wp_bucket_words<SRC, THREADS>(a.nb);
     uint64_t* s_ent = reinterpret_cast<uint64_t*>(smem);
     uint32_t* s_hist = reinterpret_cast<uint32_t*>(s_ent + TILE);
     uint32_t* s_start = s_hist + nbp;
@@ -60,7 +76,7 @@
     __syncthreads();
     typedef unsigned int u32x4 __attribute__((ext_vector_type(4)));
     uint32_t code[ITEMS], row[ITEMS], rank[ITEMS];
-    if constexpr (SRC == 2) {
+    if constexpr (SRC >= 2) {
         uint64_t c0[ITEMS];
         uint32_t okm = 0;
 #pragma unroll
@@ -84,11 +100,11 @@
             for (int c = 0; c < 4; c++) row[4 * j + c] = a.row_base + (uint32_t)(t0 + i4 + c);
         }
         const uint32_t have = okm;
-        encode_rows_arith<ITEMS, uint32_t>(a.ap, c0, code, &okm);
+        encode_rows_arith<ITEMS, uint32_t>(ap, c0, code, &okm);
         bool bad = false;
 #pragma unroll
         for (int k = 0; k < ITEMS; k++) {
-            const bool ok = ((okm >> k) & 1u) && code[k] < a.states;
+            const bool ok = ((okm >> k) & 1u) && code[k] < states;
             bad |= ((have >> k) & 1u) && !ok;
             code[k] = ok ? code[k] : kWinEmpty;
         }
@@ -136,17 +152,17 @@
     lds_atomics_barrier();
     uint32_t tot;
     {
-        const uint32_t per = nbp / THREADS;
+        const uint32_t per = SRC == 3 ? (nbp + (uint32_t)THREADS - 1u) / THREADS : nbp / THREADS;
         uint32_t h[kWpMaxBuckets / THREADS], sum = 0;
 #pragma unroll
         for (int k = 0; k < kWpMaxBuckets / THREADS; k++) {
-            h[k] = (uint32_t)k < per ? s_hist[t * per + k] : 0u;
+            h[k] = (uint32_t)k < per && (SRC != 3 || t * per + k < nbp) ? s_hist[t * per + k] : 0u;
             sum += h[k];
         }
         uint32_t run = block_exclusive_sum<uint32_t, THREADS>(sum, s_tmp, &tot);
 #pragma unroll
         for (int k = 0; k < kWpMaxBuckets / THREADS; k++) {
-            if ((uint32_t)k < per) {
+            if ((uint32_t)k < per && (SRC != 3 || t * per + k < nbp)) {
                 const uint32_t b = t * per + k;
                 s_start[b] = run;
                 if (h[k]) s_delta[b] = atomicAdd(&a.dst_count[(uint64_t)sb * a.nb + b], h[k]) - run;
@@ -185,8 +201,13 @@
     if (__ballot(over) && lane_id() == 0) *a.flag = 1u;
 }
 
-__global__ __launch_bounds__(1024) void k_win_offsets(const uint32_t* __restrict__ counts, uint32_t nwin, uint32_t* __restrict__ off) {
+__global__ __launch_bounds__(1024) void k_win_offsets(const uint32_t* __restrict__ counts, uint32_t nwin, uint32_t* __restrict__ off,
+                                                     const DirectPlan* __restrict__ plan, uint64_t n) {
     __shared__ uint32_t s_tmp[1024 / kWave + 1];
+    if (plan) {
+        if (plan->accept == 0u || (uint64_t)plan->states == n) return;
+        nwin = plan->nwin;
+    }
     uint32_t carry = 0;
     for (uint32_t base = 0; base < nwin; base += 1024) {
         const uint32_t i = base + threadIdx.x;
@@ -199,16 +220,27 @@
     }
 }
 
+template <bool PLANNED>
 __global__ __launch_bounds__(kPlaceThreads) void k_win_place(const uint64_t* __restrict__ entries, uint32_t* __restrict__ counts,
                                                             const uint32_t* __restrict__ off, uint64_t n, uint32_t* __restrict__ perm,
                                                             uint32_t* __restrict__ sorted, uint32_t* __restrict__ flag,
                                                             uint32_t* __restrict__ clear_also, uint32_t nclear, uint2* __restrict__ ranktab,
-                                                            uint32_t rank_blocks) {
+                                                            uint32_t rank_blocks, const DirectPlan* __restrict__ plan) {
     extern __shared__ __attribute__((aligned(16))) uint8_t smem[];
     __shared__ uint32_t s_wcount[kPlaceThreads / kWave];
     typedef unsigned int u32x4 __attribute__((ext_vector_type(4)));
     uint32_t* win = reinterpret_cast<uint32_t*>(smem);
     const uint32_t g = blockIdx.x, t = threadIdx.x;
+    if constexpr (PLANNED) {
+        if (plan->accept == 0u || g >= plan->nwin) return;
+        const uint32_t states = plan->states;
+        if ((uint64_t)states == n) {
+            off = nullptr;
+            ranktab = nullptr;
+        } else {
+            rank_blocks = (uint32_t)((((uint64_t)states + 31) / 32 + 1) & ~1ull);
+        }
+    }
     const uint32_t craw = counts[g], cnt = craw < kWinSlots ? craw : kWinSlots;
     {
         u32x4 e;
@@ -296,7 +328,7 @@
 
 template <int SRC, int THREADS, int ITEMS>
 static Status win_partition_launch(cph_ctx* ctx, const WpArgs& a, unsigned grid, double bytes) {
-    const uint32_t nbp = (a.nb + (uint32_t)THREADS - 1u) & ~((uint32_t)THREADS - 1u);
+    const uint32_t nbp = wp_bucket_words<SRC, THREADS>(a.nb);
     const size_t lds = (size_t)THREADS * ITEMS * 8 + (size_t)nbp * 12;
     CPH_TRY(kernel_setup(ctx, reinterpret_cast<const void*>(&k_win_partition<SRC, THREADS, ITEMS>), THREADS, lds, nullptr));
     ProfScope ps(ctx, "k_win_partition", bytes);
@@ -352,15 +384,15 @@
     uint32_t* counts = two ? cur2 : cur1;
     if (need_off) {
         ProfScope ps(ctx, "k_win_place", 0);
-        hipLaunchKernelGGL(k_win_offsets, dim3(1), dim3(1024), 0, ctx->stream, counts, (uint32_t)nwin_total, off);
+        hipLaunchKernelGGL(k_win_offsets, dim3(1), dim3(1024), 0, ctx->stream, counts, (uint32_t)nwin_total, off, (const DirectPlan*)nullptr, n);
     }
     {
         const size_t lds = (size_t)kWinSlots * sizeof(uint32_t);
-        CPH_TRY(kernel_setup(ctx, reinterpret_cast<const void*>(&k_win_place), kPlaceThreads, lds, nullptr));
+        CPH_TRY(kernel_setup(ctx, reinterpret_cast<const void*>(&k_win_place<false>), kPlaceThreads, lds, nullptr));
         ProfScope ps(ctx, "k_win_place", 16.0 * (double)n);
-        hipLaunchKernelGGL(k_win_place, dim3((unsigned)nwin_total), dim3(kPlaceThreads), lds, ctx->stream, two ? ent2.as<uint64_t>() : ent1.as<uint64_t>(),
+        hipLaunchKernelGGL(k_win_place<false>, dim3((unsigned)nwin_total), dim3(kPlaceThreads), lds, ctx->stream, two ? ent2.as<uint64_t>() : ent1.as<uint64_t>(),
                            counts, need_off ? off : nullptr, n, perm_out, sorted_out, flag, cur1, two ? (uint32_t)nb1 : 0u,
-                           static_cast<uint2*>(ranktab), (uint32_t)rank_blocks);
+                           static_cast<uint2*>(ranktab), (uint32_t)rank_blocks, (const DirectPlan*)nullptr);
     }
     CPH_HIP_TRY(hipGetLastError());
     finished = true;
@@ -384,6 +416,42 @@
     return ws.finish(ctx, perm_out, sorted_out, flag, ranktab, rank_blocks);
 }
 
+
+uint64_t planned_max_states(uint64_t n) { return std::min<uint64_t>(2 * n, (uint64_t)kWpMaxBuckets << kWinBits); }
+Status direct_sort_windows_planned(cph_ctx* ctx, const uint64_t* keys, uint64_t n, const DirectPlan* plan, uint32_t* perm_out, uint32_t* sorted_out,
+                                   uint32_t* flag, void* ranktab, DevBuf* ent, DevBuf* off) {
+    const uint64_t nb_max = (planned_max_states(n) + kWinSlots - 1) >> kWinBits;
+    CPH_TRY(ent->alloc(&ctx->pool, (nb_max << kWinBits) * sizeof(uint64_t)));
+    CPH_TRY(off->alloc(&ctx->pool, nb_max * sizeof(uint32_t)));
+    DevBuf* words = &ctx->self_clean[ctx->stream_slot].win;
+    CPH_TRY(self_clean_block(ctx, words, nb_max * sizeof(uint32_t)));
+    uint32_t* cur = words->as<uint32_t>();
+    WpArgs a{};
+    a.keys = keys;
+    a.plan = plan;
+    a.n = n;
+    a.tiles_per_src = (uint32_t)((n + kWpTile - 1) / kWpTile);
+    a.shift = (uint32_t)kWinBits;
+    a.nb = (uint32_t)nb_max;
+    a.dst = ent->as<uint64_t>();
+    a.dst_count = cur;
+    a.flag = flag;
+    CPH_TRY((win_partition_launch<3, kWpThreadsOneLevel, kWpItemsOneLevel>(ctx, a, a.tiles_per_src, 16.0 * (double)n)));
+    {
+        ProfScope ps(ctx, "k_win_place", 0);
+        hipLaunchKernelGGL(k_win_offsets, dim3(1), dim3(1024), 0, ctx->stream, cur, (uint32_t)nb_max, off->as<uint32_t>(), plan, n);
+    }
+    {
+        const size_t lds = (size_t)kWinSlots * sizeof(uint32_t);
+        CPH_TRY(kernel_setup(ctx, reinterpret_cast<const void*>(&k_win_place<true>), kPlaceThreads, lds, nullptr));
+        ProfScope ps(ctx, "k_win_place", 16.0 * (double)n);
+        hipLaunchKernelGGL(k_win_place<true>, dim3((unsigned)nb_max), dim3(kPlaceThreads), lds, ctx->stream, ent->as<uint64_t>(), cur, off->as<uint32_t>(), n,
+                           perm_out, sorted_out, flag, cur, 0u, static_cast<uint2*>(ranktab), 0u, plan);
+    }
+    CPH_HIP_TRY(hipGetLastError());
+    return {};
+}
+
 }
 
 namespace cph {
```
